# hila-chefer/Transformer-Explainability

Hardware: NVIDIA H100
Metric: explanations_per_sec (higher is better)
Workload: dtype f32

## Files before the change

### transformer_explainability_b200/csrc/te_bert.cu

```cuda
#include <string.h>

#include <algorithm>

#include "../../include/te_b200.h"
#include "te_engine_util.h"
#include "te_gemm_tc.h"
#include "te_kernels.h"
#include "te_rollout.h"
#include "te_zplus.h"

using namespace te_util;

namespace {

constexpr int kMaxDepth = 64;

struct Dims {
    int B, N, NP, D, H, dh, F, C, L, V, P, T;
    long long M;
    float eps;
};

static bool make_dims(const te_bert_config* c, int B, int S, Dims& d) {
    if (!c || c->layers <= 0 || c->layers > kMaxDepth || c->heads <= 0 || c->hidden % c->heads != 0 || c->hidden % 8 != 0 ||
// ... 187 lines not shown
    TE_TRY(check_ws(cfg, batch, seq, workspace, workspace_bytes, d, ws));
    if (!weights || !input_ids || !attention_mask) { te_set_last_error("te_bert_forward: null pointer"); return TE_ERR_ARG; }
    Select sel;
    TE_TRY(decode_flags(sel, "te_bert_forward", flags, derived, 0, false));
    cudaStream_t st = reinterpret_cast<cudaStream_t>(stream);
    const F16Forward f16 = f16_forward(sel, d.M, d.D, d.F, ws.tD[1], ws.tD[2], ws.tF[1], ws.tD[3]);
    auto layernorm = [&](const float* x, const float* g, const float* b, float* y, float* mean, float* rstd) {
        return f16.on ? te_launch_layernorm_split(x, g, b, y, mean, rstd, d.M, d.D, d.eps, f16.qkv.split, f16.qkv.scale, st)
                      : te_launch_layernorm(x, g, b, y, mean, rstd, d.M, d.D, d.eps, st);
    };
    Weights w;
    bind_weights(cfg, weights, w);
    const float scale = 1.0f / sqrtf((float)d.dh);

    TE_TRY(te_launch_bert_embed(input_ids, w.word, w.pos, w.type, ws.tD[0], d.B, d.N, d.D, d.V, st));
    TE_TRY(layernorm(ws.tD[0], w.elnw, w.elnb, ws.layer[0].h, nullptr, nullptr));
    TE_TRY(te_launch_bert_mask(attention_mask, ws.maskadd, (long long)d.B * d.N, st));

    for (int l = 0; l < d.L; ++l) {
        LayerAct& a = ws.layer[l];
        const LayerW& lw = w.layer[l];
        float* h_next = (l + 1 < d.L) ? ws.layer[l + 1].h : ws.h_last;
        const DerivedW tw = bind_derived(d, sel.lbase, l);
        TE_TRY(linear_fwd_tc(tw.qkv, a.h, d.D, lw.qkvw, lw.qkvb, a.qkv, nullptr, nullptr, d.M, d.D, 3 * d.D, TE_EPI_BIAS, st,
                             &f16.qkv));
        TE_TRY(attn_nn(sel.atc, d.B, d.H, d.N, d.NP, d.dh, a.qkv, 3 * d.D, a.qkv + d.D, 3 * d.D, a.P, nullptr, scale,
                       TE_EPI_STORE, st));
        TE_TRY(te_launch_softmax_masked(a.P, (long long)d.B * d.H * d.N, d.N, d.NP, ws.maskadd, (long long)d.H * d.N, st));
        TE_TRY(attn_nk(sel.atc, d.B, d.H, d.N, d.NP, d.dh, a.P, 0, a.qkv + 2 * d.D, 3 * d.D, a.ctx, d.D, nullptr, 1.f,
                       TE_EPI_STORE, st));
        TE_TRY(linear_fwd_tc(tw.o, a.ctx, d.D, lw.ow, lw.ob, a.d1, a.s1, a.h, d.M, d.D, d.D, TE_EPI_BIAS_ADD, st, &f16.proj));
        TE_TRY(layernorm(a.s1, lw.ln1w, lw.ln1b, a.ao, a.mean1, a.rstd1));
        TE_TRY(linear_fwd_tc(tw.w1, a.ao, d.D, lw.w1, lw.b1, a.hpre, a.g, nullptr, d.M, d.D, d.F, TE_EPI_BIAS_GELU, st,
                             &f16.fc1));
        TE_TRY(linear_fwd_tc(tw.w2, a.g, d.F, lw.w2, lw.b2, a.d2, a.s2, a.ao, d.M, d.F, d.D, TE_EPI_BIAS_ADD, st, &f16.fc2));
        TE_TRY(layernorm(a.s2, lw.ln2w, lw.ln2b, h_next, a.mean2, a.rstd2));
    }
    TE_TRY(linear_fwd(ws.h_last, d.N * d.D, w.poolw, w.poolb, ws.pd, nullptr, nullptr, d.B, d.D, d.D, TE_EPI_BIAS, st));
    TE_TRY(te_launch_tanh(ws.pd, ws.pooled, (long long)d.B * d.D, st));
    TE_TRY(linear_fwd(ws.pooled, d.D, w.clsw, w.clsb, ws.logits, nullptr, nullptr, d.B, d.D, d.C, TE_EPI_BIAS, st));
    if (logits && cudaMemcpyAsync(logits, ws.logits, sizeof(float) * d.B * d.C, cudaMemcpyDeviceToDevice, st) != cudaSuccess) {
        te_set_last_error("te_bert_forward: logits copy failed");
        return TE_ERR_CUDA;
    }
    return TE_OK;
}

extern "C" int te_bert_attribute(const te_bert_config* cfg, const float* weights, const float* derived, int batch, int seq,
                                 int* index, int start_layer, float alpha, unsigned flags, float* maps, void* workspace,
                                 long long workspace_bytes, void* stream) {
    Dims d; Workspace ws;
    TE_TRY(check_ws(cfg, batch, seq, workspace, workspace_bytes, d, ws));
    if (!isfinite(alpha)) { te_set_last_error("te_bert_attribute: alpha must be finite"); return TE_ERR_ARG; }
    TE_TRY(te_util::check_grad_rollout("te_bert_attribute", flags, alpha));
    const bool grad_rollout = (flags & TE_FLAG_ATTN_GRAD_ROLLOUT) != 0;
    if (!weights || !index || (!maps && !(flags & TE_FLAG_GRADIENTS_ONLY))) { te_set_last_error("te_bert_attribute: null pointer"); return TE_ERR_ARG; }
    if (start_layer < 0 || start_layer >= d.L) { te_set_last_error("te_bert_attribute: start_layer out of range"); return TE_ERR_ARG; }
    Select sel;
    TE_TRY(decode_flags(sel, "te_bert_attribute", flags, derived, start_layer, !grad_rollout, {ws.tF[1], ws.nF[1]},
                        {ws.t3D[1], d.M * 3LL * d.D}, d.M, std::max(3 * d.D, d.F)));
    cudaStream_t st = reinterpret_cast<cudaStream_t>(stream);
    Weights w;
    bind_weights(cfg, weights, w);
    const float scale = 1.0f / sqrtf((float)d.dh);
    const long long MD = d.M * d.D, DD = (long long)d.D * d.D;

    TE_TRY(te_launch_argmax(ws.logits, index, d.B, d.C, 1, st));
    TE_TRY(te_launch_onehot(index, ws.seed, d.B, d.C, 1.0f, st));

    float* dxa = ws.tD[0]; float* dsx = ws.tD[1]; float* dctx = ws.tD[2]; float* dxn = ws.tD[3];
    float* dF = ws.tF[0]; float* dqkv = ws.t3D[0]; float* dS = ws.tA[0];
    TE_TRY(linear_bwd(ws.seed, w.clsw, ws.dpool, nullptr, d.B, d.D, d.C, TE_EPI_STORE, st));
    TE_TRY(te_launch_tanh_bwd(ws.dpool, ws.pooled, ws.dpd, (long long)d.B * d.D, st));
    TE_TRY(linear_bwd(ws.dpd, w.poolw, ws.dfirst, nullptr, d.B, d.D, d.D, TE_EPI_STORE, st));
    TE_TRY(te_launch_fill(dxa, 0.f, MD, st));
    if (cudaMemcpy2DAsync(dxa, sizeof(float) * d.N * d.D, ws.dfirst, sizeof(float) * d.D, sizeof(float) * d.D, d.B,
                          cudaMemcpyDeviceToDevice, st) != cudaSuccess) {
        te_set_last_error("te_bert_attribute: scatter of the pooled-token gradient failed");
        return TE_ERR_CUDA;
    }
    for (int l = d.L - 1; l >= start_layer; --l) {
        LayerAct& a = ws.layer[l];
        const LayerW& lw = w.layer[l];
        TE_TRY(te_launch_layernorm_bwd(dxa, a.s2, lw.ln2w, a.mean2, a.rstd2, nullptr, dsx, d.M, d.D, st));
        const DerivedW tw = bind_derived(d, sel.lbase, l);
        TE_TRY(linear_bwd_tc(tw.w2, dsx, lw.w2, dF, a.hpre, d.M, d.F, d.D, TE_EPI_GELU_BWD, st, sel.btf, &sel.bfs));
        TE_TRY(linear_bwd_tc(tw.w1, dF, lw.w1, dxn, nullptr, d.M, d.D, d.F, TE_EPI_STORE, st, sel.btf, &sel.bfs));
        TE_TRY(te_launch_add2(dxn, dsx, dxn, MD, st));
        TE_TRY(te_launch_layernorm_bwd(dxn, a.s1, lw.ln1w, a.mean1, a.rstd1, nullptr, dsx, d.M, d.D, st));
        TE_TRY(linear_bwd_tc(tw.o, dsx, lw.ow, dctx, nullptr, d.M, d.D, d.D, TE_EPI_STORE, st, sel.btf, &sel.bfs));
        const bool last = (l == start_layer);
        TE_TRY(attn_block_bwd(sel, d.B, d.H, d.N, d.NP, d.dh, a.qkv, a.P, dctx, a.G, dS, dqkv, scale, last, st));
        if (last) break;
        TE_TRY(linear_bwd_tc(tw.qkv, dqkv, lw.qkvw, dxn, nullptr, d.M, d.D, 3 * d.D, TE_EPI_STORE, st, sel.btf, &sel.bfs));
        TE_TRY(te_launch_add2(dxn, dsx, dxa, MD, st));
    }

    if (flags & TE_FLAG_GRADIENTS_ONLY) return TE_OK;
    const long long layer_stride = d.L > 1 ? (long long)(ws.layer[1].G - ws.layer[0].G) : 0;
    if (grad_rollout) {
        TE_TRY(te_rollout_layers(ws.layer[0].G, ws.layer[0].P, layer_stride, d.L, d.B, d.H, d.N, d.NP, d.NP, start_layer,
                                 0, flags, ws.mats, ws.joint[0], ws.joint[1], nullptr, maps, 0,
                                 0, st));
        if (cudaMemset2DAsync(maps, sizeof(float) * d.N, 0, sizeof(float), d.B, st) != cudaSuccess) {
            te_set_last_error("te_bert_attribute: clearing element 0 of the maps failed");
            return TE_ERR_CUDA;
        }
        return TE_OK;
    }

    float* R = ws.tD[0]; float* R1 = ws.tD[1]; float* R2 = ws.tD[2]; float* R3 = ws.tD[3];
    float* RF = ws.tF[0]; float* SF = ws.tF[1]; float* S = ws.t3D[0]; float* Rqkv = ws.t3D[1];
    double* addp = sel.lrp ? nullptr : ws.addpart;
    TE_TRY(te_linear_rule_relprop(sel.lrp, ws.pooled, d.D, w.clsw, nullptr, ws.seed, d.C, ws.rpool, ws.shead, d.B, d.D, d.C, st,
                                  nullptr, 0, nullptr, sel.zv, 0, nullptr, alpha));
    TE_TRY(te_linear_rule_relprop(sel.lrp, ws.h_last, (long long)d.N * d.D, w.poolw, nullptr, ws.rpool, d.D, ws.rfirst, ws.shead,
                                  d.B, d.D, d.D, st, nullptr, 0, nullptr, sel.zv, 0, nullptr, alpha));
    TE_TRY(te_launch_index_select_relprop(ws.h_last, ws.rfirst, nullptr, R, d.B, d.N, d.D, st));

    for (int l = d.L - 1; l >= sel.low; --l) {
        LayerAct& a = ws.layer[l];
        const LayerW& lw = w.layer[l];
        const DerivedW dw = bind_derived(d, sel.dbase, l);
        const bool top = (l == d.L - 1) && te_engine_cls_rows();
        const long long zr = top ? d.B : d.M;
        const long long sD = top ? (long long)d.N * d.D : d.D, sF = top ? (long long)d.N * d.F : d.F;
        TE_TRY(te_launch_add_relprop(a.d2, a.ao, R, R1, R2, addp, d.B, (long long)d.N * d.D, st));
        TE_TRY(te_linear_rule_relprop(sel.lrp, a.g, sF, lw.w2, dw.w2, R1, sD, RF, S, zr, d.F, d.D, st, a.d2, sD, lw.b2, sel.zv, sF,
                                      SF, alpha));
        TE_TRY(te_linear_rule_relprop(sel.lrp, a.ao, sD, lw.w1, dw.w1, RF, sF, R1, SF, zr, d.D, d.F, st, a.hpre, sF, lw.b1, sel.zv,
                                      sD, S, alpha));
        TE_TRY(te_launch_clone_relprop(a.ao, R1, R2, nullptr, R, MD, st));
        TE_TRY(te_launch_add_relprop(a.d1, a.h, R, R1, R2, addp, d.B, (long long)d.N * d.D, st));
        if (top) TE_TRY(te_launch_fill(R3, 0.f, MD, st));
        TE_TRY(te_linear_rule_relprop(sel.lrp, a.ctx, sD, lw.ow, dw.o, R1, sD, R3, S, zr, d.D, d.D, st, a.d1, sD, lw.ob, sel.zv, sD,
                                      S + MD, alpha));
        const bool last = (l == sel.low && !(flags & TE_FLAG_RELPROP_TO_INPUT));
        TE_TRY(attn_relprop_pv(sel, d.B, d.H, d.N, d.NP, d.dh, a.qkv, a.P, R3, a.ctx, S, a.cam, Rqkv, last, st));
        if (last) break;
        TE_TRY(attn_nn(sel.atc, d.B, d.H, d.N, d.NP, d.dh, a.qkv, 3 * d.D, a.qkv + d.D, 3 * d.D, ws.tA[0], nullptr, scale,
                       TE_EPI_STORE, st));
        TE_TRY(te_launch_add_relprop_keymask(ws.tA[0], ws.maskadd, a.cam, ws.tA[1], addp, d.B, d.H, d.N, d.NP, st));
        TE_TRY(attn_relprop_qk(sel, d.B, d.H, d.N, d.NP, d.dh, a.qkv, ws.tA[1], ws.tA[0], Rqkv, st));
        TE_TRY(te_linear_rule_relprop(sel.lrp, a.h, d.D, lw.qkvw, dw.q, Rqkv, 3 * d.D, R, S, d.M, d.D, d.D, st, a.qkv, 3 * d.D,
                                      lw.qkvb, sel.zv, 0, S + MD, alpha));
        TE_TRY(te_linear_rule_relprop(sel.lrp, a.h, d.D, lw.qkvw + DD, dw.k, Rqkv + d.D, 3 * d.D, R1, S, d.M, d.D, d.D, st,
                                      a.qkv + d.D, 3 * d.D, lw.qkvb + d.D, sel.zv, 0, S + MD, alpha));
        TE_TRY(te_linear_rule_relprop(sel.lrp, a.h, d.D, lw.qkvw + 2 * DD, dw.v, Rqkv + 2 * d.D, 3 * d.D, R3, S, d.M, d.D, d.D, st,
                                      a.qkv + 2 * d.D, 3 * d.D, lw.qkvb + 2 * d.D, sel.zv, 0, S + MD, alpha));
        TE_TRY(te_launch_clone_relprop(a.h, R, R1, R3, SF, MD, st));
        TE_TRY(te_launch_clone_relprop(a.h, SF, R2, nullptr, R, MD, st));
    }

    TE_TRY(te_rollout_layers(ws.layer[0].G, ws.layer[0].cam, layer_stride, d.L, d.B, d.H, d.N, d.NP, d.NP, start_layer,
                             1, flags, ws.mats, ws.joint[0], ws.joint[1], nullptr, maps, 0,
                             1, st));
    return TE_OK;
}

extern "C" int te_bert_explain(const te_bert_config* cfg, const float* weights, const float* derived,
                               const long long* input_ids, const long long* attention_mask, int batch, int seq,
                               int* index, int start_layer, unsigned flags, float* maps, float* logits, void* workspace,
                               long long workspace_bytes, void* stream) {
    TE_TRY(te_bert_forward(cfg, weights, derived, input_ids, attention_mask, batch, seq, flags, logits, workspace,
                           workspace_bytes, stream));
    return te_bert_attribute(cfg, weights, derived, batch, seq, index, start_layer, 1.f, flags, maps, workspace, workspace_bytes,
                             stream);
}

extern "C" int te_bert_tensor(const te_bert_config* cfg, int batch, int seq, void* workspace, const char* name, int layer,
                              float** ptr, long long dims[4], long long strides[4]) {
    Dims d; Workspace ws;
    if (!workspace || !name || !ptr) return TE_ERR_ARG;
    if (batch <= 0 || !make_dims(cfg, batch, seq, d)) return TE_ERR_ARG;
    carve(d, reinterpret_cast<char*>(workspace), ws);
    const std::string n(name);
    const View set{ptr, dims, strides};
    if (n == "logits") return set(ws.logits, d.B, d.C, 1, 1, d.C, 1, 1, 1);
    if (n == "relevance_in") return set(ws.tD[0], d.B, d.N, d.D, 1, (long long)d.N * d.D, d.D, 1, 1);
    if (n.rfind("tmp_d", 0) == 0 && n.size() == 6 && n[5] >= '0' && n[5] <= '3')
        return set(ws.tD[n[5] - '0'], d.B, d.N, d.D, 1, (long long)d.N * d.D, d.D, 1, 1);
    if (n.rfind("tmp_f", 0) == 0 && n.size() == 6 && n[5] >= '0' && n[5] <= '1')
        return set(ws.tF[n[5] - '0'], d.B, d.N, d.F, 1, (long long)d.N * d.F, d.F, 1, 1);
    if (n.rfind("tmp_3d", 0) == 0 && n.size() == 7 && n[6] >= '0' && n[6] <= '1')
        return set(ws.t3D[n[6] - '0'], d.B, d.N, 3LL * d.D, 1, (long long)d.N * 3 * d.D, 3LL * d.D, 1, 1);
    const long long ND = (long long)d.N * d.D, NF = (long long)d.N * d.F;
    if (n == "h_last") return set(ws.h_last, d.B, d.N, d.D, 1, ND, d.D, 1, 1);
    if (n == "pooled") return set(ws.pooled, d.B, d.D, 1, 1, d.D, 1, 1, 1);
    if (layer < 0 || layer >= d.L) { te_set_last_error("te_bert_tensor: layer out of range"); return TE_ERR_ARG; }
    LayerAct& a = ws.layer[layer];
    const long long hs = (long long)d.N * d.NP, bs = hs * d.H;
    if (n == "attn") return set(a.P, d.B, d.H, d.N, d.N, bs, hs, d.NP, 1);
    if (n == "attn_grad") return set(a.G, d.B, d.H, d.N, d.N, bs, hs, d.NP, 1);
    if (n == "attn_cam") return set(a.cam, d.B, d.H, d.N, d.N, bs, hs, d.NP, 1);
    if (n == "hidden") return set(a.h, d.B, d.N, d.D, 1, (long long)d.N * d.D, d.D, 1, 1);
    if (n == "qkv") return set(a.qkv, d.B, d.N, 3LL * d.D, 1, 3 * ND, 3LL * d.D, 1, 1);
    float* rowD = n == "ctx" ? a.ctx : n == "d1" ? a.d1 : n == "s1" ? a.s1 : n == "ao" ? a.ao : n == "d2" ? a.d2
                : n == "s2" ? a.s2 : nullptr;
    if (rowD) return set(rowD, d.B, d.N, d.D, 1, ND, d.D, 1, 1);
    float* rowF = n == "hpre" ? a.hpre : n == "g" ? a.g : nullptr;
    if (rowF) return set(rowF, d.B, d.N, d.F, 1, NF, d.F, 1, 1);
    float* row1 = n == "mean1" ? a.mean1 : n == "rstd1" ? a.rstd1 : n == "mean2" ? a.mean2 : n == "rstd2" ? a.rstd2 : nullptr;
    if (row1) return set(row1, d.B, d.N, 1, 1, d.N, 1, 1, 1);
    te_set_last_error("te_bert_tensor: unknown tensor name");
    return TE_ERR_ARG;
}
```

### transformer_explainability_b200/csrc/te_elementwise.cu

```cuda
#include "te_kernels.h"

namespace {

constexpr int kThreads = 256;

__global__ void im2col_kernel(const float* __restrict__ img, float* __restrict__ patches, int B, int C, int H,
                              int W, int P) {
    const int gw = W / P, gh = H / P, pq = P / 4;
    const long long total = (long long)B * gh * gw * C * P * pq;
    for (long long t = blockIdx.x * (long long)blockDim.x + threadIdx.x; t < total;
         t += (long long)gridDim.x * blockDim.x) {
        long long r = t;
        const int q = (int)(r % pq); r /= pq;
        const int iy = (int)(r % P); r /= P;
        const int c = (int)(r % C); r /= C;
        const int px = (int)(r % gw); r /= gw;
        const int py = (int)(r % gh); r /= gh;
        const int b = (int)r;
        const float4 v = *reinterpret_cast<const float4*>(
            img + (((long long)b * C + c) * H + (py * P + iy)) * W + px * P + q * 4);
        const long long row = ((long long)b * gh + py) * gw + px;
        *reinterpret_cast<float4*>(patches + row * ((long long)C * P * P) + (c * P + iy) * P + q * 4) = v;
    }
}
// ... 37 lines not shown
    const float var = te_warp_sum(q) / (float)D;
    rstd = 1.0f / sqrtf(var + eps);
}

template <bool SPLIT>
__global__ void layernorm_kernel(const float* __restrict__ x, const float* __restrict__ w,
                                 const float* __restrict__ b, float* __restrict__ y, float* __restrict__ mean_o,
                                 float* __restrict__ rstd_o, long long rows, int D, float eps, __half* __restrict__ hi,
                                 __half* __restrict__ lo, float* __restrict__ scale) {
    const int lane = threadIdx.x & 31;
    const long long row = blockIdx.x * (long long)(blockDim.x >> 5) + (threadIdx.x >> 5);
    if (row >= rows) return;
    const float* xr = x + row * D;
    float mean, rstd;
    row_stats(xr, D, lane, eps, mean, rstd);
    float* yr = y + row * D;
    const int nblk = (D + 127) / 128;
    for (int base = 0; base < D; base += 128) {
        const int i = base + lane * 4;
        float4 o = make_float4(0.f, 0.f, 0.f, 0.f);
        if (i < D) {
            const float4 v = *reinterpret_cast<const float4*>(xr + i);
            const float4 ww = *reinterpret_cast<const float4*>(w + i);
            const float4 bb = *reinterpret_cast<const float4*>(b + i);
            o.x = (v.x - mean) * rstd * ww.x + bb.x;
            o.y = (v.y - mean) * rstd * ww.y + bb.y;
            o.z = (v.z - mean) * rstd * ww.z + bb.z;
            o.w = (v.w - mean) * rstd * ww.w + bb.w;
            *reinterpret_cast<float4*>(yr + i) = o;
        }
        if (SPLIT) {
            float s, si;
            te_f16_block_scale(te_warp_max(te_absmax4(o)), s, si);
            if (i < D) {
                uint2 h, l;
                te_f16_split4(o, s, h, l);
                *reinterpret_cast<uint2*>(hi + row * D + i) = h;
                *reinterpret_cast<uint2*>(lo + row * D + i) = l;
            }
            if (lane == 0) scale[row * nblk + base / 128] = si;
        }
    }
    if (lane == 0) {
        if (mean_o) mean_o[row] = mean;
        if (rstd_o) rstd_o[row] = rstd;
    }
}

__device__ __forceinline__ void ln_bwd_row(const float* __restrict__ dyr, const float* __restrict__ xr,
                                           const float* __restrict__ w, const float* __restrict__ dresr,
                                           float* __restrict__ dxr, int D, int lane, float mean, float rstd) {
    float s1 = 0.f, s2 = 0.f;
    for (int i = lane * 4; i < D; i += 128) {
        const float4 dy = *reinterpret_cast<const float4*>(dyr + i);
        const float4 xv = *reinterpret_cast<const float4*>(xr + i);
        const float4 ww = *reinterpret_cast<const float4*>(w + i);
        const float g0 = dy.x * ww.x, g1 = dy.y * ww.y, g2 = dy.z * ww.z, g3 = dy.w * ww.w;
        s1 += (g0 + g1) + (g2 + g3);
        s2 += (g0 * ((xv.x - mean) * rstd) + g1 * ((xv.y - mean) * rstd)) +
              (g2 * ((xv.z - mean) * rstd) + g3 * ((xv.w - mean) * rstd));
    }
    const float c1 = te_warp_sum(s1) / (float)D;
    const float c2 = te_warp_sum(s2) / (float)D;
    for (int i = lane * 4; i < D; i += 128) {
        const float4 dy = *reinterpret_cast<const float4*>(dyr + i);
        const float4 xv = *reinterpret_cast<const float4*>(xr + i);
        const float4 ww = *reinterpret_cast<const float4*>(w + i);
        float4 o;
        o.x = rstd * (dy.x * ww.x - c1 - (xv.x - mean) * rstd * c2);
        o.y = rstd * (dy.y * ww.y - c1 - (xv.y - mean) * rstd * c2);
        o.z = rstd * (dy.z * ww.z - c1 - (xv.z - mean) * rstd * c2);
        o.w = rstd * (dy.w * ww.w - c1 - (xv.w - mean) * rstd * c2);
        if (dresr) {
            const float4 r = *reinterpret_cast<const float4*>(dresr + i);
            o.x += r.x; o.y += r.y; o.z += r.z; o.w += r.w;
        }
        *reinterpret_cast<float4*>(dxr + i) = o;
    }
}

__global__ void layernorm_bwd_kernel(const float* __restrict__ dy, const float* __restrict__ x,
                                     const float* __restrict__ w, const float* __restrict__ mean,
                                     const float* __restrict__ rstd, const float* __restrict__ dres,
                                     float* __restrict__ dx, long long rows, int D) {
    const int lane = threadIdx.x & 31;
    const long long row = blockIdx.x * (long long)(blockDim.x >> 5) + (threadIdx.x >> 5);
    if (row >= rows) return;
    ln_bwd_row(dy + row * D, x + row * D, w, dres ? dres + row * D : nullptr, dx + row * D, D, lane, mean[row],
               rstd[row]);
}

__global__ void layernorm_bwd_strided_kernel(const float* __restrict__ dy, long long dy_stride,
                                             const float* __restrict__ x, long long x_stride,
                                             const float* __restrict__ w, float eps, float* __restrict__ dx,
                                             long long dx_stride, int rows, int D) {
    const int lane = threadIdx.x & 31;
    const int row = blockIdx.x * (blockDim.x >> 5) + (threadIdx.x >> 5);
    if (row >= rows) return;
    const float* xr = x + row * x_stride;
    float mean, rstd;
    row_stats(xr, D, lane, eps, mean, rstd);
    ln_bwd_row(dy + row * dy_stride, xr, w, nullptr, dx + row * dx_stride, D, lane, mean, rstd);
}

__global__ void softmax_kernel(float* __restrict__ s, long long rows, int N, int ld,
                               const float* __restrict__ keymask, long long rows_per_batch) {
    const int lane = threadIdx.x & 31;
    const long long row = blockIdx.x * (long long)(blockDim.x >> 5) + (threadIdx.x >> 5);
    if (row >= rows) return;
    float* r = s + row * ld;
    if (keymask) {
        const float* mk = keymask + (row / rows_per_batch) * N;
        for (int j = lane; j < N; j += 32) r[j] = r[j] + mk[j];
    }
    float m = -INFINITY;
    for (int j = lane; j < N; j += 32) m = fmaxf(m, r[j]);
    m = te_warp_max(m);
    float sum = 0.f;
    for (int j = lane; j < N; j += 32) {
        const float e = expf(r[j] - m);
        r[j] = e;
        sum += e;
    }
    sum = te_warp_sum(sum);
    for (int j = lane; j < ld; j += 32) r[j] = (j < N) ? r[j] / sum : 0.f;
}

__global__ void softmax_bwd_kernel(const float* __restrict__ p, const float* __restrict__ dp,
                                   float* __restrict__ ds, long long rows, int N, int ld, float scale) {
    const int lane = threadIdx.x & 31;
    const long long row = blockIdx.x * (long long)(blockDim.x >> 5) + (threadIdx.x >> 5);
    if (row >= rows) return;
    const float* pr = p + row * ld;
    const float* gr = dp + row * ld;
    float dot = 0.f;
    for (int j = lane; j < N; j += 32) dot = fmaf(pr[j], gr[j], dot);
    dot = te_warp_sum(dot);
    float* o = ds + row * ld;
    for (int j = lane; j < ld; j += 32) o[j] = (j < N) ? pr[j] * (gr[j] - dot) * scale : 0.f;
}

__global__ void argmax_kernel(const float* __restrict__ logits, int* __restrict__ index, int B, int C,
                              int only_negative) {
    const int lane = threadIdx.x & 31;
    const int b = blockIdx.x * (blockDim.x >> 5) + (threadIdx.x >> 5);
    if (b >= B) return;
    const float* r = logits + (long long)b * C;
    float best = -INFINITY;
    int bi = 0x7fffffff;
    for (int j = lane; j < C; j += 32) {
        const float v = r[j];
        if (v > best || (v == best && j < bi)) { best = v; bi = j; }
    }
#pragma unroll
    for (int o = 16; o > 0; o >>= 1) {
        const float ov = __shfl_xor_sync(0xffffffffu, best, o);
        const int oi = __shfl_xor_sync(0xffffffffu, bi, o);
        if (ov > best || (ov == best && oi < bi)) { best = ov; bi = oi; }
    }
    if (lane == 0 && (!only_negative || index[b] < 0)) index[b] = (bi == 0x7fffffff) ? 0 : bi;
}

__global__ void onehot_kernel(const int* __restrict__ index, float* __restrict__ seed, int B, int C, float value) {
    const long long total = (long long)B * C;
    for (long long t = blockIdx.x * (long long)blockDim.x + threadIdx.x; t < total;
         t += (long long)gridDim.x * blockDim.x) {
        const int b = (int)(t / C), c = (int)(t % C);
        seed[t] = (index[b] == c) ? value : 0.f;
    }
}

__global__ void sd_kernel(const float* a, const float* b, float* out,
                          long long n4) {
    for (long long t = blockIdx.x * (long long)blockDim.x + threadIdx.x; t < n4;
         t += (long long)gridDim.x * blockDim.x) {
        const float4 va = reinterpret_cast<const float4*>(a)[t];
        const float4 vb = reinterpret_cast<const float4*>(b)[t];
        reinterpret_cast<float4*>(out)[t] =
            make_float4(te_sd(va.x, vb.x), te_sd(va.y, vb.y), te_sd(va.z, vb.z), te_sd(va.w, vb.w));
    }
}

__global__ void clone_relprop_kernel(const float* __restrict__ x, const float* __restrict__ r1,
                                     const float* __restrict__ r2, const float* __restrict__ r3,
                                     float* __restrict__ out, long long n4) {
    for (long long t = blockIdx.x * (long long)blockDim.x + threadIdx.x; t < n4;
         t += (long long)gridDim.x * blockDim.x) {
        const float4 xv = reinterpret_cast<const float4*>(x)[t];
        const float4 a = reinterpret_cast<const float4*>(r1)[t];
        const float4 b = reinterpret_cast<const float4*>(r2)[t];
        float4 c = make_float4(te_sd(a.x, xv.x) + te_sd(b.x, xv.x), te_sd(a.y, xv.y) + te_sd(b.y, xv.y),
                               te_sd(a.z, xv.z) + te_sd(b.z, xv.z), te_sd(a.w, xv.w) + te_sd(b.w, xv.w));
        if (r3) {
            const float4 d = reinterpret_cast<const float4*>(r3)[t];
            c.x += te_sd(d.x, xv.x); c.y += te_sd(d.y, xv.y); c.z += te_sd(d.z, xv.z); c.w += te_sd(d.w, xv.w);
        }
        reinterpret_cast<float4*>(out)[t] = make_float4(xv.x * c.x, xv.y * c.y, xv.z * c.z, xv.w * c.w);
    }
}

__global__ void add_reduce_kernel(const float* __restrict__ x1, const float* __restrict__ x2,
                                  const float* __restrict__ r, double* __restrict__ partial, long long per4,
                                  long long x2s4) {
    const int b = blockIdx.y, sp = blockIdx.x;
    const long long chunk = (per4 + TE_ADD_SPLIT - 1) / TE_ADD_SPLIT;
    const long long lo = sp * chunk, hi = min(per4, lo + chunk);
    const float4* p1 = reinterpret_cast<const float4*>(x1) + b * per4;
    const float4* p2 = reinterpret_cast<const float4*>(x2) + b * x2s4;
    const float4* pr = reinterpret_cast<const float4*>(r) + b * per4;
    double sa = 0.0, sb = 0.0, sr = 0.0;
    for (long long t = lo + threadIdx.x; t < hi; t += blockDim.x) {
        const float4 a = p1[t], c = p2[t], rr = pr[t];
        const float s0 = te_sd(rr.x, a.x + c.x), s1 = te_sd(rr.y, a.y + c.y);
        const float s2 = te_sd(rr.z, a.z + c.z), s3 = te_sd(rr.w, a.w + c.w);
        sa += ((double)(a.x * s0) + (double)(a.y * s1)) + ((double)(a.z * s2) + (double)(a.w * s3));
        sb += ((double)(c.x * s0) + (double)(c.y * s1)) + ((double)(c.z * s2) + (double)(c.w * s3));
        sr += ((double)rr.x + (double)rr.y) + ((double)rr.z + (double)rr.w);
    }
    __shared__ double red[3][kThreads / 32];
    sa = te_warp_sum(sa); sb = te_warp_sum(sb); sr = te_warp_sum(sr);
    const int lane = threadIdx.x & 31, wid = threadIdx.x >> 5;
    if (lane == 0) { red[0][wid] = sa; red[1][wid] = sb; red[2][wid] = sr; }
    __syncthreads();
    if (threadIdx.x == 0) {
        double ta = 0, tb = 0, tr = 0;
        for (int i = 0; i < kThreads / 32; ++i) { ta += red[0][i]; tb += red[1][i]; tr += red[2][i]; }
        double* o = partial + ((long long)b * TE_ADD_SPLIT + sp) * 3;
        o[0] = ta; o[1] = tb; o[2] = tr;
    }
}

__global__ void add_scale_kernel(const float* __restrict__ x1, const float* __restrict__ x2,
                                 const float* __restrict__ r, float* __restrict__ r1, float* __restrict__ r2,
                                 const double* __restrict__ partial, long long per4, long long x2s4) {
    const int b = blockIdx.y;
    __shared__ float fa_s, fb_s;
    if (threadIdx.x == 0 && partial == nullptr) { fa_s = 1.f; fb_s = 1.f; }
    if (threadIdx.x == 0 && partial != nullptr) {
        double A = 0, Bs = 0, rho = 0;
        const double* q = partial + (long long)b * TE_ADD_SPLIT * 3;
        for (int i = 0; i < TE_ADD_SPLIT; ++i) { A += q[i * 3]; Bs += q[i * 3 + 1]; rho += q[i * 3 + 2]; }
        const double den = fabs(A) + fabs(Bs);
        const double a_fact = te_sd(fabs(A), den) * rho;
        const double b_fact = te_sd(fabs(Bs), den) * rho;
        fa_s = (float)te_sd(a_fact, A);
        fb_s = (float)te_sd(b_fact, Bs);
    }
    __syncthreads();
    const float fa = fa_s, fb = fb_s;
    const float4* p1 = reinterpret_cast<const float4*>(x1) + b * per4;
    const float4* p2 = reinterpret_cast<const float4*>(x2) + b * x2s4;
    const float4* pr = reinterpret_cast<const float4*>(r) + b * per4;
    float4* o1 = reinterpret_cast<float4*>(r1) + b * per4;
    float4* o2 = r2 ? reinterpret_cast<float4*>(r2) + b * per4 : nullptr;
    for (long long t = blockIdx.x * (long long)blockDim.x + threadIdx.x; t < per4;
         t += (long long)gridDim.x * blockDim.x) {
        const float4 a = p1[t], c = p2[t], rr = pr[t];
        const float s0 = te_sd(rr.x, a.x + c.x), s1 = te_sd(rr.y, a.y + c.y);
        const float s2 = te_sd(rr.z, a.z + c.z), s3 = te_sd(rr.w, a.w + c.w);
        o1[t] = make_float4(a.x * s0 * fa, a.y * s1 * fa, a.z * s2 * fa, a.w * s3 * fa);
        if (o2) o2[t] = make_float4(c.x * s0 * fb, c.y * s1 * fb, c.z * s2 * fb, c.w * s3 * fb);
    }
}

__global__ void index_select_relprop_kernel(const float* __restrict__ x, const float* __restrict__ r0,
                                            const float* __restrict__ r1, float* __restrict__ out, int B, int N,
                                            int D) {
    const long long total = (long long)B * N * D;
    for (long long t = blockIdx.x * (long long)blockDim.x + threadIdx.x; t < total;
         t += (long long)gridDim.x * blockDim.x) {
        const int d = (int)(t % D);
        const long long rt = t / D;
        const int tok = (int)(rt % N);
        const int b = (int)(rt / N);
        float v = 0.f;
        if (tok == 0) v = x[t] * te_sd(r0[(long long)b * D + d], x[t]);
        else if (tok == 1 && r1 != nullptr) v = x[t] * te_sd(r1[(long long)b * D + d], x[t]);
        out[t] = v;
    }
}

__global__ void aggregate_kernel(const float* __restrict__ G, const float* __restrict__ cam,
                                 float* __restrict__ M, int B, int H, int N, int ld_in, int ld, int add_eye,
                                 int normalize, float* __restrict__ diag) {
    const int lane = threadIdx.x & 31;
    const long long row = blockIdx.x * (long long)(blockDim.x >> 5) + (threadIdx.x >> 5);
    if (row >= (long long)B * N) return;
    const int b = (int)(row / N), i = (int)(row % N);
    float* out = M + row * ld;
    float rs = 0.f;
    for (int j = lane; j < ld; j += 32) {
        float v = 0.f;
        if (j < N) {
            float s = 0.f;
            for (int h = 0; h < H; ++h) {
                const long long o = (((long long)b * H + h) * N + i) * ld_in + j;
                s += fmaxf(G[o] * cam[o], 0.f);
            }
            v = s / (float)H;
            if (add_eye && j == i) v += 1.0f;
        }
        out[j] = v;
        rs += v;
    }
    if (normalize) {
        rs = te_warp_sum(rs);
        if (diag != nullptr) rs += 1.0f;
        __syncwarp();
        for (int j = lane; j < N; j += 32) out[j] = out[j] / rs;
        if (diag != nullptr && lane == 0) diag[row] = 1.0f / rs;
    }
}

__global__ void aggregate_vec_kernel(const float* __restrict__ G, const float* __restrict__ cam, float* __restrict__ M,
                                     int B, int H, int N, int ld_in, int ld, int add_eye, int normalize,
                                     float* __restrict__ diag) {
    const int lane = threadIdx.x & 31;
    const long long row = blockIdx.x * (long long)(blockDim.x >> 5) + (threadIdx.x >> 5);
    if (row >= (long long)B * N) return;
    const int b = (int)(row / N), i = (int)(row % N);
    float* out = M + row * ld;
    float rs = 0.f;
    for (int j4 = lane; j4 * 4 < ld; j4 += 32) {
        const int j = j4 * 4;
        float4 s = make_float4(0.f, 0.f, 0.f, 0.f);
        if (j < N && j < ld_in) {
#pragma unroll 4
            for (int h = 0; h < H; ++h) {
                const long long o = (((long long)b * H + h) * N + i) * ld_in + j;
                const float4 g = __ldcs(reinterpret_cast<const float4*>(G + o));
                const float4 c = __ldcs(reinterpret_cast<const float4*>(cam + o));
                s.x += fmaxf(g.x * c.x, 0.f); s.y += fmaxf(g.y * c.y, 0.f);
                s.z += fmaxf(g.z * c.z, 0.f); s.w += fmaxf(g.w * c.w, 0.f);
            }
        }
        float v[4] = {s.x / (float)H, s.y / (float)H, s.z / (float)H, s.w / (float)H};
#pragma unroll
        for (int u = 0; u < 4; ++u) {
// ... 133 lines not shown
    }
}

__global__ void prep_mats_kernel(const float* __restrict__ in, float* __restrict__ out, long long rows, int N,
                                 int ld_in, int ld_out, int normalize) {
    const int lane = threadIdx.x & 31;
    const long long row = blockIdx.x * (long long)(blockDim.x >> 5) + (threadIdx.x >> 5);
    if (row >= rows) return;
    const int i = (int)(row % N);
    const float* r = in + row * ld_in;
    float* o = out + row * ld_out;
    float rs = 0.f;
    for (int j = lane; j < ld_out; j += 32) {
        float v = 0.f;
        if (j < N) v = r[j] + ((j == i) ? 1.0f : 0.0f);
        o[j] = v;
        rs += v;
    }
    if (normalize) {
        rs = te_warp_sum(rs);
        __syncwarp();
        for (int j = lane; j < N; j += 32) o[j] = o[j] / rs;
    }
}

__global__ void extract_row_kernel(const float* __restrict__ joint, float* __restrict__ out, int B, int N, int ld,
                                   int first, int bert_fix) {
    const int lane = threadIdx.x & 31;
    const int b = blockIdx.x * (blockDim.x >> 5) + (threadIdx.x >> 5);
    if (b >= B) return;
    const float* r = joint + (long long)b * N * ld;
    float mn = INFINITY;
    if (bert_fix) {
        for (int j = lane; j < N; j += 32) mn = fminf(mn, r[j]);
#pragma unroll
        for (int o = 16; o > 0; o >>= 1) mn = fminf(mn, __shfl_xor_sync(0xffffffffu, mn, o));
    }
    float* o = out + (long long)b * (N - first);
    for (int j = first + lane; j < N; j += 32) o[j - first] = (bert_fix && j == 0) ? mn : r[j];
}

__global__ void average2_kernel(const float* __restrict__ a, const float* __restrict__ b, float* __restrict__ out,
                                long long n) {
    for (long long t = blockIdx.x * (long long)blockDim.x + threadIdx.x; t < n;
         t += (long long)gridDim.x * blockDim.x) out[t] = (a[t] + b[t]) / 2.0f;
}

__global__ void bert_embed_kernel(const long long* __restrict__ ids, const float* __restrict__ word,
                                  const float* __restrict__ pos, const float* __restrict__ type0,
                                  float* __restrict__ out, int B, int S, int D, int vocab) {
    const int d4 = D / 4;
    const long long total = (long long)B * S * d4;
    for (long long t = blockIdx.x * (long long)blockDim.x + threadIdx.x; t < total;
         t += (long long)gridDim.x * blockDim.x) {
        const int q = (int)(t % d4);
        const long long rt = t / d4;
        const int s = (int)(rt % S);
        const long long id = ids[rt];
        if (id < 0 || id >= vocab) {
            const float qn = __int_as_float(0x7fc00000);
            *reinterpret_cast<float4*>(out + rt * D + q * 4) = make_float4(qn, qn, qn, qn);
            continue;
        }
        const float4 w = *reinterpret_cast<const float4*>(word + id * D + q * 4);
        const float4 p = *reinterpret_cast<const float4*>(pos + (long long)s * D + q * 4);
        const float4 ty = *reinterpret_cast<const float4*>(type0 + q * 4);
        *reinterpret_cast<float4*>(out + rt * D + q * 4) =
            make_float4((ty.x + p.x) + w.x, (ty.y + p.y) + w.y, (ty.z + p.z) + w.z, (ty.w + p.w) + w.w);
    }
}
__global__ void bert_mask_kernel(const long long* __restrict__ mask, float* __restrict__ out, long long n) {
    for (long long t = blockIdx.x * (long long)blockDim.x + threadIdx.x; t < n; t += (long long)gridDim.x * blockDim.x)
        out[t] = (1.0f - (float)mask[t]) * -10000.0f;
}
__global__ void tanh_kernel(const float* __restrict__ x, float* __restrict__ y, long long n) {
    for (long long t = blockIdx.x * (long long)blockDim.x + threadIdx.x; t < n; t += (long long)gridDim.x * blockDim.x)
        y[t] = tanhf(x[t]);
}
__global__ void tanh_bwd_kernel(const float* __restrict__ dy, const float* __restrict__ y, float* __restrict__ dx,
                                long long n) {
    for (long long t = blockIdx.x * (long long)blockDim.x + threadIdx.x; t < n; t += (long long)gridDim.x * blockDim.x)
        dx[t] = dy[t] * (1.0f - y[t] * y[t]);
}
__global__ void add2_kernel(const float* a, const float* b, float* out, long long n4) {
    for (long long t = blockIdx.x * (long long)blockDim.x + threadIdx.x; t < n4;
         t += (long long)gridDim.x * blockDim.x) {
        const float4 u = reinterpret_cast<const float4*>(a)[t], v = reinterpret_cast<const float4*>(b)[t];
        reinterpret_cast<float4*>(out)[t] = make_float4(u.x + v.x, u.y + v.y, u.z + v.z, u.w + v.w);
    }
}

__global__ void add_keymask_reduce_kernel(const float* __restrict__ x1, const float* __restrict__ mk,
                                          const float* __restrict__ r, double* __restrict__ partial, int HN, int N,
                                          int ld) {
    const int b = blockIdx.y, sp = blockIdx.x;
    const int lane = threadIdx.x & 31, wid = threadIdx.x >> 5, nw = blockDim.x >> 5;
    const float* m = mk + (long long)b * N;
    double sa = 0.0, sb = 0.0, sr = 0.0;
    for (int row = sp * nw + wid; row < HN; row += TE_ADD_SPLIT * nw) {
        const float* xr = x1 + ((long long)b * HN + row) * ld;
        const float* rr = r + ((long long)b * HN + row) * ld;
        for (int j = lane; j < N; j += 32) {
            const float a = xr[j], c = m[j], rv = rr[j];
            const float s = te_sd(rv, a + c);
            sa += (double)(a * s); sb += (double)(c * s); sr += (double)rv;
        }
    }
    __shared__ double red[3][kThreads / 32];
    sa = te_warp_sum(sa); sb = te_warp_sum(sb); sr = te_warp_sum(sr);
    if (lane == 0) { red[0][wid] = sa; red[1][wid] = sb; red[2][wid] = sr; }
    __syncthreads();
    if (threadIdx.x == 0) {
        double ta = 0, tb = 0, tr = 0;
        for (int i = 0; i < nw; ++i) { ta += red[0][i]; tb += red[1][i]; tr += red[2][i]; }
        double* o = partial + ((long long)b * TE_ADD_SPLIT + sp) * 3;
        o[0] = ta; o[1] = tb; o[2] = tr;
    }
}
__global__ void add_keymask_scale_kernel(const float* __restrict__ x1, const float* __restrict__ mk,
                                         const float* __restrict__ r, float* __restrict__ r1,
                                         const double* __restrict__ partial, int HN, int N, int ld) {
    const int b = blockIdx.y;
    __shared__ float fa_s;
    if (threadIdx.x == 0 && partial == nullptr) fa_s = 1.f;
    else if (threadIdx.x == 0) {
        double A = 0, Bs = 0, rho = 0;
        const double* q = partial + (long long)b * TE_ADD_SPLIT * 3;
        for (int i = 0; i < TE_ADD_SPLIT; ++i) { A += q[i * 3]; Bs += q[i * 3 + 1]; rho += q[i * 3 + 2]; }
        const double den = fabs(A) + fabs(Bs);
        fa_s = (float)te_sd(te_sd(fabs(A), den) * rho, A);
    }
    __syncthreads();
    const float fa = fa_s;
    const int lane = threadIdx.x & 31, wid = threadIdx.x >> 5, nw = blockDim.x >> 5;
    const float* m = mk + (long long)b * N;
    for (int row = blockIdx.x * nw + wid; row < HN; row += gridDim.x * nw) {
        const float* xr = x1 + ((long long)b * HN + row) * ld;
        const float* rr = r + ((long long)b * HN + row) * ld;
        float* o = r1 + ((long long)b * HN + row) * ld;
        for (int j = lane; j < ld; j += 32) {
            float v = 0.f;
            if (j < N) { const float a = xr[j]; v = a * te_sd(rr[j], a + m[j]) * fa; }
            o[j] = v;
        }
    }
}

__global__ void fill_kernel(float* __restrict__ p, float v, long long n) {
    for (long long t = blockIdx.x * (long long)blockDim.x + threadIdx.x; t < n;
         t += (long long)gridDim.x * blockDim.x) p[t] = v;
}

inline int flat_grid(long long work) {
    long long g = (work + kThreads - 1) / kThreads;
    const long long cap = 132LL * 16;
    return (int)(g < 1 ? 1 : (g > cap ? cap : g));
}
inline int warp_rows_grid(long long rows) { return (int)((rows + (kThreads / 32) - 1) / (kThreads / 32)); }

}

#define TE_REQ(c, msg) do { if (!(c)) { te_set_last_error(msg); return TE_ERR_ARG; } } while (0)

int te_launch_im2col(const float* img, float* patches, int B, int C, int H, int W, int P, cudaStream_t st) {
    TE_REQ(P % 4 == 0 && W % P == 0 && H % P == 0, "im2col: patch must divide the image and be a multiple of 4");
    const long long total = (long long)B * (H / P) * (W / P) * C * P * (P / 4);
    im2col_kernel<<<flat_grid(total), kThreads, 0, st>>>(img, patches, B, C, H, W, P);
    TE_CUDA_CHECK_LAUNCH();
    return TE_OK;
}
int te_launch_assemble_tokens(const float* patch_out, const float* cls, const float* dist, const float* pos,
                              float* x, int B, int N, int D, int n_prefix, cudaStream_t st) {
    TE_REQ(D % 4 == 0, "assemble: D % 4 != 0");
    assemble_tokens_kernel<<<flat_grid((long long)B * N * (D / 4)), kThreads, 0, st>>>(patch_out, cls, dist, pos, x,
                                                                                     B, N, D, n_prefix);
    TE_CUDA_CHECK_LAUNCH();
    return TE_OK;
}
int te_launch_layernorm(const float* x, const float* w, const float* b, float* y, float* mean, float* rstd,
                        long long rows, int D, float eps, cudaStream_t st) {
    TE_REQ(D % 4 == 0, "layernorm: D % 4 != 0");
    if (rows <= 0) return TE_OK;
    layernorm_kernel<false><<<warp_rows_grid(rows), kThreads, 0, st>>>(x, w, b, y, mean, rstd, rows, D, eps, nullptr, nullptr,
                                                                       nullptr);
    TE_CUDA_CHECK_LAUNCH();
    return TE_OK;
}
int te_launch_layernorm_split(const float* x, const float* w, const float* b, float* y, float* mean, float* rstd,
                              long long rows, int D, float eps, float* split, float* scale, cudaStream_t st) {
    TE_REQ(D % 4 == 0, "layernorm: D % 4 != 0");
    TE_REQ(split && scale, "layernorm_split: null split buffers");
    if (rows <= 0) return TE_OK;
    __half* hi = reinterpret_cast<__half*>(split);
    layernorm_kernel<true><<<warp_rows_grid(rows), kThreads, 0, st>>>(x, w, b, y, mean, rstd, rows, D, eps, hi, hi + rows * D, scale);
    TE_CUDA_CHECK_LAUNCH();
    return TE_OK;
}
int te_launch_layernorm_bwd(const float* dy, const float* x, const float* w, const float* mean, const float* rstd,
                            const float* dres, float* dx, long long rows, int D, cudaStream_t st) {
    TE_REQ(D % 4 == 0, "layernorm_bwd: D % 4 != 0");
    if (rows <= 0) return TE_OK;
    layernorm_bwd_kernel<<<warp_rows_grid(rows), kThreads, 0, st>>>(dy, x, w, mean, rstd, dres, dx, rows, D);
    TE_CUDA_CHECK_LAUNCH();
    return TE_OK;
}
int te_launch_layernorm_bwd_strided(const float* dy, long long dy_stride, const float* x, long long x_stride,
                                    const float* w, float eps, float* dx, long long dx_stride, int rows, int D,
                                    cudaStream_t st) {
    TE_REQ(D % 4 == 0 && dy_stride % 4 == 0 && x_stride % 4 == 0 && dx_stride % 4 == 0, "layernorm_bwd_strided: align");
    if (rows <= 0) return TE_OK;
    layernorm_bwd_strided_kernel<<<warp_rows_grid(rows), kThreads, 0, st>>>(dy, dy_stride, x, x_stride, w, eps, dx,
                                                                          dx_stride, rows, D);
    TE_CUDA_CHECK_LAUNCH();
    return TE_OK;
}
int te_launch_softmax(float* s, long long rows, int N, int ld, cudaStream_t st) {
    return te_launch_softmax_masked(s, rows, N, ld, nullptr, 1, st);
}
int te_launch_softmax_masked(float* s, long long rows, int N, int ld, const float* keymask, long long rows_per_batch,
                             cudaStream_t st) {
    if (rows <= 0) return TE_OK;
    softmax_kernel<<<warp_rows_grid(rows), kThreads, 0, st>>>(s, rows, N, ld, keymask, rows_per_batch);
    TE_CUDA_CHECK_LAUNCH();
    return TE_OK;
}
int te_launch_softmax_bwd(const float* p, const float* dp, float* ds, long long rows, int N, int ld, float scale,
                          cudaStream_t st) {
    if (rows <= 0) return TE_OK;
    softmax_bwd_kernel<<<warp_rows_grid(rows), kThreads, 0, st>>>(p, dp, ds, rows, N, ld, scale);
    TE_CUDA_CHECK_LAUNCH();
    return TE_OK;
}
int te_launch_argmax(const float* logits, int* index, int B, int C, int only_negative, cudaStream_t st) {
    argmax_kernel<<<warp_rows_grid(B), kThreads, 0, st>>>(logits, index, B, C, only_negative);
    TE_CUDA_CHECK_LAUNCH();
    return TE_OK;
}
int te_launch_onehot(const int* index, float* seed, int B, int C, float value, cudaStream_t st) {
    onehot_kernel<<<flat_grid((long long)B * C), kThreads, 0, st>>>(index, seed, B, C, value);
    TE_CUDA_CHECK_LAUNCH();
    return TE_OK;
}
int te_launch_sd(const float* a, const float* b, float* out, long long n, cudaStream_t st) {
    TE_REQ(n % 4 == 0, "sd: n % 4 != 0");
    sd_kernel<<<flat_grid(n / 4), kThreads, 0, st>>>(a, b, out, n / 4);
    TE_CUDA_CHECK_LAUNCH();
    return TE_OK;
}
int te_launch_clone_relprop(const float* x, const float* r1, const float* r2, const float* r3, float* out,
                            long long n, cudaStream_t st) {
    TE_REQ(n % 4 == 0, "clone_relprop: n % 4 != 0");
    clone_relprop_kernel<<<flat_grid(n / 4), kThreads, 0, st>>>(x, r1, r2, r3, out, n / 4);
    TE_CUDA_CHECK_LAUNCH();
    return TE_OK;
}
int te_launch_add_relprop_strided(const float* x1, const float* x2, long long x2_sample_stride, const float* r, float* r1,
                                  float* r2, double* partial, int B, long long per_sample, cudaStream_t st) {
    TE_REQ(per_sample % 4 == 0 && x2_sample_stride % 4 == 0, "add_relprop: per-sample size % 4 != 0");
    TE_REQ(B <= 65535, "add_relprop: batch too large for one launch");
    const long long per4 = per_sample / 4, x2s4 = x2_sample_stride / 4;
    if (partial) {
        add_reduce_kernel<<<dim3(TE_ADD_SPLIT, B), kThreads, 0, st>>>(x1, x2, r, partial, per4, x2s4);
        TE_CUDA_CHECK_LAUNCH();
    }
    int gx = (int)((per4 + kThreads - 1) / kThreads);
    gx = gx > 64 ? 64 : (gx < 1 ? 1 : gx);
    add_scale_kernel<<<dim3(gx, B), kThreads, 0, st>>>(x1, x2, r, r1, r2, partial, per4, x2s4);
    TE_CUDA_CHECK_LAUNCH();
    return TE_OK;
}
int te_launch_add_relprop(const float* x1, const float* x2, const float* r, float* r1, float* r2, double* partial,
                          int B, long long per_sample, cudaStream_t st) {
    return te_launch_add_relprop_strided(x1, x2, per_sample, r, r1, r2, partial, B, per_sample, st);
}
int te_launch_index_select_relprop(const float* x, const float* r_tok0, const float* r_tok1, float* out, int B,
                                   int N, int D, cudaStream_t st) {
    index_select_relprop_kernel<<<flat_grid((long long)B * N * D), kThreads, 0, st>>>(x, r_tok0, r_tok1, out, B, N, D);
    TE_CUDA_CHECK_LAUNCH();
    return TE_OK;
}
int te_launch_aggregate(const float* G, const float* cam, float* M, int B, int H, int N, int ld_in, int ld_out,
                        int add_eye, int normalize, cudaStream_t st, float* diag) {
    const bool vec = ld_in % 4 == 0 && ld_out % 4 == 0 && ld_in >= ((N + 3) & ~3) &&
                     ((reinterpret_cast<uintptr_t>(G) | reinterpret_cast<uintptr_t>(cam) | reinterpret_cast<uintptr_t>(M)) & 15u) == 0;
    if (vec)
        aggregate_vec_kernel<<<warp_rows_grid((long long)B * N), kThreads, 0, st>>>(G, cam, M, B, H, N, ld_in, ld_out,
                                                                                  add_eye, normalize, diag);
    else
        aggregate_kernel<<<warp_rows_grid((long long)B * N), kThreads, 0, st>>>(G, cam, M, B, H, N, ld_in, ld_out, add_eye,
                                                                              normalize, diag);
    TE_CUDA_CHECK_LAUNCH();
    return TE_OK;
}
int te_launch_aggregate_layers(const float* G0, const float* cam0, long long in_layer_stride, float* M0, long long m_layer_stride,
                               int B, int H, int N, int ld_in, int ld_out, int first_layer, int num_layers, int normalize,
                               cudaStream_t st, float* diag0) {
    const bool vec = ld_in % 4 == 0 && ld_out % 4 == 0 && ld_in >= ((N + 3) & ~3) && in_layer_stride % 4 == 0 &&
                     m_layer_stride % 4 == 0 &&
                     ((reinterpret_cast<uintptr_t>(G0) | reinterpret_cast<uintptr_t>(cam0) | reinterpret_cast<uintptr_t>(M0)) & 15u) == 0;
    TE_REQ(vec && num_layers >= 1 && num_layers <= 65535, "aggregate_layers: unsupported layout");
    dim3 grid(warp_rows_grid((long long)B * N), num_layers);
    aggregate_layers_vec_kernel<<<grid, kThreads, 0, st>>>(G0, cam0, in_layer_stride, M0, m_layer_stride, B, H, N, ld_in, ld_out,
                                                          first_layer, normalize, diag0);
    TE_CUDA_CHECK_LAUNCH();
    return TE_OK;
}
int te_launch_relevance_heatmap(const float* maps, float* out, int B, int g, int scale, cudaStream_t st) {
    TE_REQ(B > 0 && g > 0 && scale > 0, "relevance_heatmap: bad shape");
    relevance_heatmap_kernel<<<B, kThreads, 0, st>>>(maps, out, g, scale);
    TE_CUDA_CHECK_LAUNCH();
    return TE_OK;
}
int te_launch_head_reduce(const float* a, const float* g, const float* hw, float* out, int B, int H, int N, int ld,
                          int mode, cudaStream_t st) {
    head_reduce_kernel<<<warp_rows_grid((long long)B * N), kThreads, 0, st>>>(a, g, hw, out, B, H, N, ld, mode);
    TE_CUDA_CHECK_LAUNCH();
    return TE_OK;
}
int te_launch_head_region_mean(const float* g, float* out, int BH, int N, int ld, int r0, int r1, int c0, int c1,
                               cudaStream_t st) {
    TE_REQ(BH > 0 && r0 >= 0 && r1 > r0 && r1 <= N && c0 >= 0 && c1 > c0 && c1 <= N, "head_region_mean: bad region");
    head_region_mean_kernel<<<BH, kThreads, 0, st>>>(g, out, N, ld, r0, r1, c0, c1);
    TE_CUDA_CHECK_LAUNCH();
    return TE_OK;
}
int te_launch_prep_mats(const float* in, float* out, long long rows, int N, int ld_in, int ld_out, int normalize,
                        cudaStream_t st) {
    if (rows <= 0) return TE_OK;
    prep_mats_kernel<<<warp_rows_grid(rows), kThreads, 0, st>>>(in, out, rows, N, ld_in, ld_out, normalize);
    TE_CUDA_CHECK_LAUNCH();
    return TE_OK;
}
int te_launch_extract_row(const float* joint, float* out, int B, int N, int ld, int first, int bert_fix,
                          cudaStream_t st) {
    extract_row_kernel<<<warp_rows_grid(B), kThreads, 0, st>>>(joint, out, B, N, ld, first, bert_fix);
    TE_CUDA_CHECK_LAUNCH();
    return TE_OK;
}
int te_launch_average2(const float* a, const float* b, float* out, long long n, cudaStream_t st) {
    average2_kernel<<<flat_grid(n), kThreads, 0, st>>>(a, b, out, n);
    TE_CUDA_CHECK_LAUNCH();
    return TE_OK;
}
int te_launch_bert_embed(const long long* ids, const float* word, const float* pos, const float* type0, float* out,
                         int B, int S, int D, int vocab, cudaStream_t st) {
    TE_REQ(D % 4 == 0, "bert_embed: D % 4 != 0");
    bert_embed_kernel<<<flat_grid((long long)B * S * (D / 4)), kThreads, 0, st>>>(ids, word, pos, type0, out, B, S, D, vocab);
    TE_CUDA_CHECK_LAUNCH();
    return TE_OK;
}
int te_launch_bert_mask(const long long* mask, float* out, long long n, cudaStream_t st) {
    bert_mask_kernel<<<flat_grid(n), kThreads, 0, st>>>(mask, out, n);
    TE_CUDA_CHECK_LAUNCH();
    return TE_OK;
}
int te_launch_tanh(const float* x, float* y, long long n, cudaStream_t st) {
    tanh_kernel<<<flat_grid(n), kThreads, 0, st>>>(x, y, n);
    TE_CUDA_CHECK_LAUNCH();
    return TE_OK;
}
int te_launch_tanh_bwd(const float* dy, const float* y, float* dx, long long n, cudaStream_t st) {
    tanh_bwd_kernel<<<flat_grid(n), kThreads, 0, st>>>(dy, y, dx, n);
    TE_CUDA_CHECK_LAUNCH();
    return TE_OK;
}
int te_launch_add2(const float* a, const float* b, float* out, long long n, cudaStream_t st) {
    TE_REQ(n % 4 == 0, "add2: n % 4 != 0");
    add2_kernel<<<flat_grid(n / 4), kThreads, 0, st>>>(a, b, out, n / 4);
    TE_CUDA_CHECK_LAUNCH();
    return TE_OK;
}
int te_launch_add_relprop_keymask(const float* x1, const float* keymask, const float* r, float* r1, double* partial,
                                  int B, int H, int N, int ld, cudaStream_t st) {
    TE_REQ(B <= 65535, "add_relprop_keymask: batch too large for one launch");
    if (partial) {
        add_keymask_reduce_kernel<<<dim3(TE_ADD_SPLIT, B), kThreads, 0, st>>>(x1, keymask, r, partial, H * N, N, ld);
        TE_CUDA_CHECK_LAUNCH();
    }
    int gx = (H * N + 7) / 8;
    gx = gx > 64 ? 64 : gx;
    add_keymask_scale_kernel<<<dim3(gx, B), kThreads, 0, st>>>(x1, keymask, r, r1, partial, H * N, N, ld);
    TE_CUDA_CHECK_LAUNCH();
    return TE_OK;
}
int te_launch_fill(float* p, float v, long long n, cudaStream_t st) {
    if (n <= 0) return TE_OK;
    fill_kernel<<<flat_grid(n), kThreads, 0, st>>>(p, v, n);
    TE_CUDA_CHECK_LAUNCH();
    return TE_OK;
}
```

### transformer_explainability_b200/csrc/te_engine_util.h

```cpp
#pragma once
#include <string.h>
#include <string>
#include <vector>

#include "../../include/te_b200.h"
#include "te_gemm.cuh"
#include "te_gemm_tc.h"
#include "te_kernels.h"
#include "te_zplus.h"

bool te_engine_cls_rows();
void te_engine_set_cls_rows(int on);
bool te_engine_gelu_split();
void te_engine_set_gelu_split(int on);

namespace te_util {

static inline TeGemm gemm0() {
    TeGemm p;
    memset(&p, 0, sizeof(p));
    p.nb1 = 1; p.nb2 = 1; p.alpha = 1.f;
    return p;
}

static inline int linear_fwd(const float* x, int lda, const float* w, const float* bias, float* y, float* y2,
                             const float* e0, long long M, int in, int out, int epi, cudaStream_t st) {
    TeGemm p = gemm0();
    p.A = x; p.lda = lda; p.B = w; p.ldb = in; p.C = y; p.ldc = out; p.C2 = y2; p.ldc2 = out; p.E0 = e0; p.lde0 = out;
    p.bias = bias; p.M = (int)M; p.N = out; p.K = in;
    return te_gemm_launch(p, TE_L_K, TE_L_K, TE_XF_NONE, epi, st);
}
static inline int linear_bwd(const float* dy, const float* w, float* dx, const float* e0, long long M, int in, int out,
                             int epi, cudaStream_t st) {
    TeGemm p = gemm0();
    p.A = dy; p.lda = out; p.B = w; p.ldb = in; p.C = dx; p.ldc = in; p.E0 = e0; p.lde0 = in;
    p.M = (int)M; p.N = in; p.K = out;
    return te_gemm_launch(p, TE_L_K, TE_L_MN, TE_XF_NONE, epi, st);
}

static inline int no_fallback(const char* msg) {
    te_set_last_error(msg);
    return TE_ERR_UNSUPPORTED;
}

struct F16Split { float* split; float* scale; bool ready; float* split_out; float* scale_out; };
static inline int linear_fwd_tc(const float* dw, const float* x, int lda, const float* w, const float* bias, float* y,
                                float* y2, const float* e0, long long M, int in, int out, int epi, cudaStream_t st,
                                const F16Split* fs = nullptr) {
    const bool f16 = dw && fs && fs->split;
    if (f16 && epi != TE_EPI_GELU_BWD && te_tc_fwd16_supported(M, in, out, lda))
        return te_tc_linear_fwd16(fs->ready ? nullptr : x, lda, fs->split, fs->scale, dw, in, out, bias, y, y2, e0, M, epi, st,
                                  epi == TE_EPI_BIAS_GELU ? fs->split_out : nullptr, epi == TE_EPI_BIAS_GELU ? fs->scale_out : nullptr);
    if (dw && te_tc_gemm3x_supported(M, in, out, lda))
        return te_tc_linear_fwd(x, lda, dw, in, out, bias, y, y2, e0, M, epi, st);
    return linear_fwd(x, lda, w, bias, y, y2, e0, M, in, out, epi, st);
}
static inline int linear_bwd_tc(const float* dw, const float* dy, const float* w, float* dx, const float* e0, long long M,
                                int in, int out, int epi, cudaStream_t st, bool tf32 = false, const F16Split* fs = nullptr) {
    const bool f16 = dw && fs && fs->split, single_epi = epi == TE_EPI_STORE || epi == TE_EPI_GELU_BWD;
    if (f16 && single_epi && te_tc_fwd16_supported(M, out, in, out))
        return te_tc_linear_bwd16(fs->ready ? nullptr : dy, out, fs->split, fs->scale, dw, in, out, dx, e0, M, epi, st);
    if (dw && tf32 && single_epi && te_tc_gemm3x_supported(M, out, in, out))
        return te_tc_linear_bwd_tf32(dy, out, dw, in, out, dx, e0, M, epi, st);
    if (dw && te_tc_gemm3x_supported(M, out, in, out))
        return te_tc_linear_bwd(dy, dw, in, out, dx, e0, M, epi, st);
    return linear_bwd(dy, w, dx, e0, M, in, out, epi, st);
}

struct HeadOp { const float* ptr; int ld; long long s1, s2; };
static inline HeadOp head_rows(const float* base, int ld, int N, int dh) {
    return {base, ld, (long long)N * ld, (long long)dh};
}
static inline HeadOp attn_map(const float* base, int H, int N, int NP) {
    return {base, NP, (long long)H * N * NP, (long long)N * NP};
}
static inline int head_gemm(int B, int H, HeadOp A, int alay, HeadOp Bm, int blay, HeadOp C, HeadOp E, int M, int N,
                            int K, float alpha, int epi, cudaStream_t st) {
    TeGemm p = gemm0();
    p.A = A.ptr; p.lda = A.ld; p.sA1 = A.s1; p.sA2 = A.s2;
    p.B = Bm.ptr; p.ldb = Bm.ld; p.sB1 = Bm.s1; p.sB2 = Bm.s2;
    p.C = const_cast<float*>(C.ptr); p.ldc = C.ld; p.sC1 = C.s1; p.sC2 = C.s2;
    p.E0 = E.ptr; p.lde0 = E.ld; p.sE1 = E.s1; p.sE2 = E.s2;
    p.M = M; p.N = N; p.K = K; p.nb1 = B; p.nb2 = H; p.alpha = alpha;
    return te_gemm_launch(p, alay, blay, TE_XF_NONE, epi, st);
}

static inline int attn_nn(bool tc, int B, int H, int N, int NP, int dh, const float* A, int lda, const float* Bm, int ldb,
                          float* out, const float* E, float alpha, int epi, cudaStream_t st, bool tf32 = false) {
    if (tc && te_tc_attn_supported(N, dh, lda, ldb, NP)) {
        const int e = (epi == TE_EPI_STORE) ? TE_TC_ATTN_STORE : (epi == TE_EPI_MUL) ? TE_TC_ATTN_MUL : TE_TC_ATTN_SD;
        return te_tc_attn_nn(A, lda, Bm, ldb, B, H, N, dh, out, NP, E, alpha, e, st, tf32 && N <= 256 && epi != TE_EPI_SD);
    }
    const HeadOp none = {nullptr, 0, 0, 0};
    return head_gemm(B, H, head_rows(A, lda, N, dh), TE_L_K, head_rows(Bm, ldb, N, dh), TE_L_K, attn_map(out, H, N, NP),
                     E ? attn_map(E, H, N, NP) : none, N, N, dh, alpha, epi, st);
}

static inline int attn_probs(bool tc, int B, int H, int N, int NP, int dh, const float* Q, int ldq, const float* K, int ldk,
                             float* P, float alpha, cudaStream_t st) {
    if (tc && N <= 256 && te_tc_attn_supported(N, dh, ldq, ldk, NP))
        return te_tc_attn_nn(Q, ldq, K, ldk, B, H, N, dh, P, NP, nullptr, alpha, TE_TC_ATTN_SOFTMAX, st);
    TE_TRY(attn_nn(tc, B, H, N, NP, dh, Q, ldq, K, ldk, P, nullptr, alpha, TE_EPI_STORE, st));
    return te_launch_softmax(P, (long long)B * H * N, N, NP, st);
}

static inline int attn_nk(bool tc, int B, int H, int N, int NP, int dh, const float* map, int amn, const float* X, int ldx,
                          float* out, int ld_out, const float* E, float alpha, int epi, cudaStream_t st, bool tf32 = false) {
    if (tc && te_tc_attn_nk_supported(N, dh, NP, ldx, ld_out)) {
        const int e = (epi == TE_EPI_STORE) ? TE_TC_ATTN_STORE : TE_TC_ATTN_MUL;
        if (epi == TE_EPI_STORE || epi == TE_EPI_MUL)
            return te_tc_attn_nk(map, NP, amn, X, ldx, B, H, N, out, ld_out, E, alpha, e, st, tf32);
    }
    const HeadOp none = {nullptr, 0, 0, 0};
    return head_gemm(B, H, attn_map(map, H, N, NP), amn ? TE_L_MN : TE_L_K, head_rows(X, ldx, N, dh), TE_L_MN,
                     head_rows(out, ld_out, N, dh), E ? head_rows(E, ld_out, N, dh) : none, N, dh, N, alpha, epi, st);
}

struct Select {
    const float* lbase;
    const float* dbase;
    bool atc;
    bool btf;
    bool rtf;
    bool f16;
    F16Split bfs;
    bool lrp;
    ZplusVariant zv;
    int low;
};
struct Lent { float* ptr; long long floats; };
static inline long long bwd_split_floats(long long rows, int out) { return rows * out / 2; }
static inline long long bwd_scale_floats(long long rows, int out) { return rows * ((out + 127) / 128); }

static inline int decode_flags(Select& s, const char* fn, unsigned flags, const float* derived, int start_layer, bool zplus,
                               Lent bwd_split = {nullptr, 0}, Lent bwd_scale = {nullptr, 0}, long long rows = 0,
                               int widest_out = 0) {
    const bool lrp = (flags & TE_FLAG_RULES_LRP) != 0;
    const unsigned rule_tc = lrp ? (flags & TE_FLAG_RULES_LRP_TC) : (flags & TE_FLAG_ZPLUS_TENSOR_CORES);
    if (((flags & (TE_FLAG_LINEAR_TENSOR_CORES | (zplus ? TE_FLAG_ZPLUS_TENSOR_CORES : 0u))) || (zplus && rule_tc)) && !derived) {
        te_set_last_error((std::string(fn) + ": tensor-core flags need the derived weight buffer").c_str());
        return TE_ERR_ARG;
    }
    s.lbase = (flags & TE_FLAG_LINEAR_TENSOR_CORES) ? derived : nullptr;
    s.dbase = rule_tc ? derived : nullptr;
    s.atc = (flags & TE_FLAG_ATTN_TENSOR_CORES) != 0;
    s.btf = (flags & TE_FLAG_BACKWARD_TF32) != 0;
    s.rtf = (flags & TE_FLAG_RELPROP_TF32) != 0;
    s.f16 = s.lbase && (flags & TE_FLAG_LINEAR_F16_SPLIT);
    const bool bf16 = s.lbase && (flags & TE_FLAG_BACKWARD_F16) && bwd_split.ptr;
    if (bf16 && (bwd_split.floats < bwd_split_floats(rows, widest_out) || bwd_scale.floats < bwd_scale_floats(rows, widest_out))) {
        te_set_last_error((std::string(fn) + ": the region lent for the fp16 split of the backward gradients is too small").c_str());
        return TE_ERR_WORKSPACE;
    }
    s.bfs = {bf16 ? bwd_split.ptr : nullptr, bwd_scale.ptr, false, nullptr, nullptr};
    s.lrp = lrp;
    s.zv = te_zplus_from_flags(flags);
    s.low = (flags & (TE_FLAG_KEEP_ALL_CAMS | TE_FLAG_RELPROP_TO_INPUT)) ? 0 : start_layer;
    return TE_OK;
}

static inline int check_grad_rollout(const char* fn, unsigned flags, float alpha) {
    if (!(flags & TE_FLAG_ATTN_GRAD_ROLLOUT)) return TE_OK;
    const char* clash = (flags & TE_FLAG_GRADIENTS_ONLY) ? "TE_FLAG_GRADIENTS_ONLY"
                      : (flags & TE_FLAG_KEEP_ALL_CAMS) ? "TE_FLAG_KEEP_ALL_CAMS"
                      : (flags & TE_FLAG_RELPROP_TO_INPUT) ? "TE_FLAG_RELPROP_TO_INPUT" : nullptr;
    if (clash) {
        te_set_last_error((std::string(fn) + ": TE_FLAG_ATTN_GRAD_ROLLOUT does not combine with " + clash).c_str());
        return TE_ERR_ARG;
    }
    if (alpha != 1.f) {
        te_set_last_error((std::string(fn) + ": TE_FLAG_ATTN_GRAD_ROLLOUT runs no relprop, alpha must be 1").c_str());
        return TE_ERR_ARG;
    }
    return TE_OK;
}

struct F16Forward { bool on; F16Split qkv, proj, fc1, fc2; };
static inline F16Forward f16_forward(const Select& s, long long M, int D, int F, float* a, float* a_scale, float* b,
                                     float* b_scale) {
    F16Forward f = {};
    f.on = s.f16 && F >= D && te_tc_fwd16_supported(M, D, 3 * D, D) && te_tc_fwd16_supported(M, D, D, D) &&
           te_tc_fwd16_supported(M, D, F, D) && te_tc_fwd16_supported(M, F, D, F);
    if (!f.on) return f;
    const bool gsf = te_engine_gelu_split();
    f.qkv = {a, a_scale, true, nullptr, nullptr};
    f.proj = {a, a_scale, false, nullptr, nullptr};
    f.fc1 = {a, a_scale, true, gsf ? b : nullptr, gsf ? b_scale : nullptr};
    f.fc2 = {b, b_scale, gsf, nullptr, nullptr};
    return f;
}

static inline int attn_block_bwd(const Select& s, int B, int H, int N, int NP, int dh, const float* qkv, const float* P,
                                 const float* dctx, float* G, float* dS, float* dqkv, float scale, bool g_only, cudaStream_t st) {
    const int D = H * dh;
    TE_TRY(attn_nn(s.atc, B, H, N, NP, dh, dctx, D, qkv + 2 * D, 3 * D, G, nullptr, 1.f, TE_EPI_STORE, st, s.btf));
    if (g_only) return TE_OK;
    TE_TRY(attn_nk(s.atc, B, H, N, NP, dh, P, 1, dctx, D, dqkv + 2 * D, 3 * D, nullptr, 1.f, TE_EPI_STORE, st, s.btf));
    TE_TRY(te_launch_softmax_bwd(P, G, dS, (long long)B * H * N, N, NP, scale, st));
    TE_TRY(attn_nk(s.atc, B, H, N, NP, dh, dS, 0, qkv + D, 3 * D, dqkv, 3 * D, nullptr, 1.f, TE_EPI_STORE, st, s.btf));
    return attn_nk(s.atc, B, H, N, NP, dh, dS, 1, qkv, 3 * D, dqkv + D, 3 * D, nullptr, 1.f, TE_EPI_STORE, st, s.btf);
}

static inline int attn_relprop_pv(const Select& s, int B, int H, int N, int NP, int dh, const float* qkv, const float* P,
                                  const float* Rctx, const float* ctx, float* S, float* cam, float* Rqkv, bool cam_only,
                                  cudaStream_t st) {
    const int D = H * dh;
    TE_TRY(te_launch_sd(Rctx, ctx, S, (long long)B * N * D, st));
    TE_TRY(attn_nn(s.atc, B, H, N, NP, dh, S, D, qkv + 2 * D, 3 * D, cam, P, 0.5f, TE_EPI_MUL, st, s.rtf));
    if (cam_only) return TE_OK;
    return attn_nk(s.atc, B, H, N, NP, dh, P, 1, S, D, Rqkv + 2 * D, 3 * D, qkv + 2 * D, 0.5f, TE_EPI_MUL, st, s.rtf);
}
static inline int attn_relprop_qk(const Select& s, int B, int H, int N, int NP, int dh, const float* qkv, const float* E,
                                  float* S1, float* Rqkv, cudaStream_t st) {
    const int D = H * dh;
    TE_TRY(attn_nn(s.atc, B, H, N, NP, dh, qkv, 3 * D, qkv + D, 3 * D, S1, E, 1.f, TE_EPI_SD, st));
    TE_TRY(attn_nk(s.atc, B, H, N, NP, dh, S1, 0, qkv + D, 3 * D, Rqkv, 3 * D, qkv, 0.5f, TE_EPI_MUL, st, s.rtf));
    return attn_nk(s.atc, B, H, N, NP, dh, S1, 1, qkv, 3 * D, Rqkv + D, 3 * D, qkv + D, 0.5f, TE_EPI_MUL, st, s.rtf);
}

struct Bump {
    char* base;
    long long off = 0;
    float* operator()(long long nfloat) {
        float* p = base ? reinterpret_cast<float*>(base + off) : nullptr;
        off += ((nfloat * 4 + 255) / 256) * 256;
        return p;
    }
};

template <class MakeDims, class Carve>
static inline int check_ws(const char* eng, int batch, void* workspace, long long bytes, MakeDims make_dims, Carve carve) {
    const std::string e(eng);
    if (batch <= 0 || !workspace) { te_set_last_error((e + ": batch <= 0 or null workspace").c_str()); return TE_ERR_ARG; }
    if (!make_dims()) return TE_ERR_ARG;
    if (((uintptr_t)workspace & 255u) != 0) { te_set_last_error((e + ": workspace must be 256-byte aligned").c_str()); return TE_ERR_ARG; }
    if (carve() > bytes) { te_set_last_error((e + ": workspace too small").c_str()); return TE_ERR_WORKSPACE; }
    return TE_OK;
}

struct View {
    float** ptr; long long* dims; long long* strides;
    int operator()(float* p, long long d0, long long d1, long long d2, long long d3, long long s0, long long s1, long long s2,
                   long long s3) const {
        *ptr = p; dims[0] = d0; dims[1] = d1; dims[2] = d2; dims[3] = d3;
        strides[0] = s0; strides[1] = s1; strides[2] = s2; strides[3] = s3;
        return TE_OK;
    }
};

struct WEntry { std::string name; long long numel; long long offset; };
using WTable = std::vector<WEntry>;
static inline int wt_count(const WTable& t) { return t.empty() ? TE_ERR_ARG : (int)t.size() - 1; }
static inline bool wt_has(const WTable& t, int i) { return i >= 0 && i + 1 < (int)t.size(); }
static inline const char* wt_name(const WTable& t, int i) {
    static thread_local std::string s;
    if (!wt_has(t, i)) return nullptr;
    s = t[i].name;
    return s.c_str();
}
static inline long long wt_numel(const WTable& t, int i) { return wt_has(t, i) ? t[i].numel : TE_ERR_ARG; }
static inline long long wt_offset(const WTable& t, int i) { return wt_has(t, i) ? t[i].offset : TE_ERR_ARG; }
static inline long long wt_total(const WTable& t) { return t.empty() ? TE_ERR_ARG : t.back().offset; }

}
```

### transformer_explainability_b200/csrc/te_gemm_tc.h

```cpp
#pragma once
#include <cuda_bf16.h>
#include <type_traits>

#include "te_common.cuh"
#include "te_zplus.h"

bool te_tc_zplus_supported(long long rows, int in_features, int out_features, long long ldx);

template <class F>
struct TeDerived {
    template <class T> using P = std::conditional_t<std::is_const<F>::value, const T*, T*>;
    F *wp, *wn, *wpt, *wnt;
    F *wh, *wl, *wth, *wtl;
    F* wabs;
    P<__nv_bfloat16> bf_wpt, bf_wnt;
    F* gap;
    P<__nv_bfloat16> bf_wabs;
    P<__half> h_w, l_w;
    F* s_w;
    P<__half> h_wt;
    F* s_wt;
    P<__half> h_wpt, h_wnt;
    F *s_wpt, *s_wnt;
    static constexpr long long floats(int in_features, int out_features) { return 16LL * in_features * out_features; }
    __host__ __device__ TeDerived(F* d, int in_features, int out_features) {
        const long long n = (long long)in_features * out_features;
        wp = d; wn = d + n; wpt = d + 2 * n; wnt = d + 3 * n;
        wh = d + 4 * n; wl = d + 5 * n; wth = d + 6 * n; wtl = d + 7 * n;
        wabs = d + 8 * n;
        bf_wpt = reinterpret_cast<P<__nv_bfloat16>>(d + 9 * n); bf_wnt = bf_wpt + n;
        gap = d + 10 * n;
        bf_wabs = reinterpret_cast<P<__nv_bfloat16>>(d + 11 * n);
        h_w = reinterpret_cast<P<__half>>(d + 11 * n + n / 2); l_w = reinterpret_cast<P<__half>>(d + 12 * n); s_w = d + 12 * n + n / 2;
        h_wt = reinterpret_cast<P<__half>>(d + 13 * n); s_wt = d + 13 * n + n / 2;
        h_wpt = reinterpret_cast<P<__half>>(d + 14 * n); h_wnt = reinterpret_cast<P<__half>>(d + 14 * n + n / 2);
        s_wpt = d + 15 * n; s_wnt = d + 15 * n + in_features;
    }
};
long long te_tc_derived_floats(int in_features, int out_features);
int te_tc_prepare_weights(const float* w, float* derived, int in_features, int out_features, cudaStream_t st);
int te_tc_zplus_linear_relprop(const float* x, long long ldx, const float* derived, const float* r, long long ldr,
                               float* out, float* s_scratch, long long rows, int in_features, int out_features, cudaStream_t st,
                               const float* y, long long ldy, const float* bias, ZplusVariant zv, long long ld_out,
                               float* xabs, float alpha = 1.f);
int te_tc_lrp_linear_relprop(const float* x, long long ldx, const float* derived, const float* r, long long ldr, float* out,
                             long long ld_out, float* s_scratch, long long rows, int in_features, int out_features,
                             cudaStream_t st, float alpha = 1.f);

enum { TE_TC_EPI_STORE = 0, TE_TC_EPI_BIAS = 1, TE_TC_EPI_BIAS_GELU = 2, TE_TC_EPI_BIAS_ADD = 3, TE_TC_EPI_GELU_BWD = 4 };
bool te_tc_gemm3x_supported(long long rows, int K, int N, long long lda);
int te_tc_linear_fwd(const float* x, long long ldx, const float* derived, int in_features, int out_features,
                     const float* bias, float* y, float* y2, const float* e0, long long rows, int epi, cudaStream_t st);
int te_tc_linear_bwd(const float* dy, const float* derived, int in_features, int out_features, float* dx, const float* e0,
                     long long rows, int epi, cudaStream_t st);

bool te_tc_fwd16_supported(long long rows, int K, int N, long long lda);
int te_tc_rowsplit_f16(const float* x, long long ldx, long long rows, int cols, void* hi, void* lo, float* scale_inv,
                       cudaStream_t st);
int te_tc_blocksplit_f16(const float* x, long long ldx, long long rows, int cols, float* split, float* scale_inv, cudaStream_t st,
                         bool hi_only = false);
int te_tc_linear_fwd16(const float* x, long long ldx, float* split, float* scale, const float* derived, int in_features,
                       int out_features, const float* bias, float* y, float* y2, const float* e0, long long rows, int epi,
                       cudaStream_t st, float* split_out = nullptr, float* scale_out = nullptr);
int te_tc_linear_bwd16(const float* dy, long long lddy, float* split, float* scale, const float* derived, int in_features,
                       int out_features, float* dx, const float* e0, long long rows, int epi, cudaStream_t st);
int te_tc_zplus_r16(const float* s, float* split, float* scale, const float* derived, const float* x, long long ldx, float* out,
                    long long ld_out, long long rows, int in_features, int out_features, cudaStream_t st, bool inh = false);

enum { TE_TC_ATTN_STORE = 0, TE_TC_ATTN_MUL = 1, TE_TC_ATTN_SD = 2, TE_TC_ATTN_SOFTMAX = 3 };
bool te_tc_attn_supported(int N, int dh, long long lda, long long ldb, int ld_out);
int te_tc_attn_nn(const float* A, long long lda, const float* B, long long ldb, int batch, int H, int N, int dh,
                  float* out, int ld_out, const float* E, float alpha, int epi, cudaStream_t st, bool single_pass = false);

bool te_tc_attn_nk_supported(int N, int dh, int NP, long long ldx, long long ld_out);
int te_tc_attn_nk(const float* map, int NP, int amn, const float* X, long long ldx, int batch, int H, int N, float* out,
                  int ld_out, const float* E, float alpha, int epi, cudaStream_t st, bool single_pass = false);

bool te_tc_bmm_nk_supported(int N, int ld);
int te_tc_bmm_nk_resid(const float* A, const float* J, const float* rowscale, float* out, int batch, int N, int ld,
                       cudaStream_t st);

int te_tc_zplus_s1(const float* x, long long ldx, float* xabs, const float* derived, const float* r, long long ldr,
                   const float* y, long long ldy, const float* bias, float* s_out, long long rows, int in_features,
                   int out_features, cudaStream_t st, bool bf16 = false, float* s16 = nullptr, float* s16_scale = nullptr,
                   float s_scale = 1.f, bool inh = false);
int te_tc_zplus_r(const float* s, const float* derived, const float* x, long long ldx, float* out, long long ld_out,
                  long long rows, int in_features, int out_features, cudaStream_t st, bool inh = false);
int te_tc_linear_bwd_tf32(const float* dy, long long lddy, const float* derived, int in_features, int out_features, float* dx,
                          const float* e0, long long rows, int epi, cudaStream_t st);
```

### transformer_explainability_b200/csrc/te_kernels.h

```cpp
#pragma once
#include "te_common.cuh"
#include "te_gemm.cuh"

int te_launch_im2col(const float* img, float* patches, int B, int C, int H, int W, int P, cudaStream_t st);
int te_launch_assemble_tokens(const float* patch_out, const float* cls, const float* dist, const float* pos,
                              float* x, int B, int N, int D, int n_prefix, cudaStream_t st);
int te_launch_layernorm(const float* x, const float* w, const float* b, float* y, float* mean, float* rstd,
                        long long rows, int D, float eps, cudaStream_t st);
int te_launch_layernorm_split(const float* x, const float* w, const float* b, float* y, float* mean, float* rstd,
                              long long rows, int D, float eps, float* split, float* scale, cudaStream_t st);
int te_launch_layernorm_bwd(const float* dy, const float* x, const float* w, const float* mean, const float* rstd,
                            const float* dres, float* dx, long long rows, int D, cudaStream_t st);
int te_launch_layernorm_bwd_strided(const float* dy, long long dy_stride, const float* x, long long x_stride,
                                    const float* w, float eps, float* dx, long long dx_stride, int rows, int D,
                                    cudaStream_t st);
int te_launch_softmax(float* s, long long rows, int N, int ld, cudaStream_t st);
int te_launch_softmax_bwd(const float* p, const float* dp, float* ds, long long rows, int N, int ld, float scale,
                          cudaStream_t st);
int te_launch_argmax(const float* logits, int* index, int B, int C, int only_negative, cudaStream_t st);
int te_launch_average2(const float* a, const float* b, float* out, long long n, cudaStream_t st);
int te_launch_onehot(const int* index, float* seed, int B, int C, float value, cudaStream_t st);
int te_launch_sd(const float* a, const float* b, float* out, long long n, cudaStream_t st);
int te_launch_clone_relprop(const float* x, const float* r1, const float* r2, const float* r3, float* out,
                            long long n, cudaStream_t st);
#define TE_ADD_SPLIT 16
int te_launch_add_relprop(const float* x1, const float* x2, const float* r, float* r1, float* r2, double* partial,
                          int B, long long per_sample, cudaStream_t st);
int te_launch_add_relprop_strided(const float* x1, const float* x2, long long x2_sample_stride, const float* r, float* r1,
                                  float* r2, double* partial, int B, long long per_sample, cudaStream_t st);
long long te_patch_relprop_scratch_floats(int B, int C, int img, int P, int D);
int te_patch_relprop_run(const float* images, const float* weight, const float* r, long long r_sample_stride, int B,
                         int C, int img, int P, int D, float* scratch, float* r_pixels, float* r_sum, cudaStream_t st);
int te_launch_index_select_relprop(const float* x, const float* r_tok0, const float* r_tok1, float* out, int B,
                                   int N, int D, cudaStream_t st);
int te_launch_aggregate(const float* G, const float* cam, float* M, int B, int H, int N, int ld_in, int ld_out,
                        int add_eye, int normalize, cudaStream_t st, float* diag = nullptr);
int te_launch_aggregate_layers(const float* G0, const float* cam0, long long in_layer_stride, float* M0, long long m_layer_stride,
                               int B, int H, int N, int ld_in, int ld_out, int first_layer, int num_layers, int normalize,
                               cudaStream_t st, float* diag0 = nullptr);
int te_launch_relevance_heatmap(const float* maps, float* out, int B, int g, int scale, cudaStream_t st);
int te_launch_head_reduce(const float* a, const float* g, const float* hw, float* out, int B, int H, int N, int ld,
                          int mode, cudaStream_t st);
int te_launch_head_region_mean(const float* g, float* out, int BH, int N, int ld, int r0, int r1, int c0, int c1,
                               cudaStream_t st);
int te_launch_prep_mats(const float* in, float* out, long long rows, int N, int ld_in, int ld_out, int normalize,
                        cudaStream_t st);
int te_launch_extract_row(const float* joint, float* out, int B, int N, int ld, int first, int bert_fix,
                          cudaStream_t st);
int te_launch_fill(float* p, float v, long long n, cudaStream_t st);
int te_launch_softmax_masked(float* s, long long rows, int N, int ld, const float* keymask, long long rows_per_batch,
                             cudaStream_t st);
int te_launch_bert_embed(const long long* ids, const float* word, const float* pos, const float* type0, float* out,
                         int B, int S, int D, int vocab, cudaStream_t st);
int te_launch_bert_mask(const long long* mask, float* out, long long n, cudaStream_t st);
int te_launch_tanh(const float* x, float* y, long long n, cudaStream_t st);
int te_launch_tanh_bwd(const float* dy, const float* y, float* dx, long long n, cudaStream_t st);
int te_launch_add2(const float* a, const float* b, float* out, long long n, cudaStream_t st);
int te_launch_add_relprop_keymask(const float* x1, const float* keymask, const float* r, float* r1, double* partial,
                                  int B, int H, int N, int ld, cudaStream_t st);
```

### transformer_explainability_b200/csrc/te_rollout_fused.cu

```cuda
#include <cooperative_groups.h>

#include "te_rollout_fused.h"

namespace cg = cooperative_groups;

namespace {

constexpr int kThreads = 256;
constexpr int kWarps = kThreads / 32;
constexpr int kHeadGroup = 6;

template <int NCHUNK>
__global__ void __launch_bounds__(kThreads, 2)
rollout_row_kernel(const float* __restrict__ G0, const float* __restrict__ cam0, long long layer_stride, int L, int H,
                   int N, int ld, int start, int normalize, int first, int bert_fix, float* __restrict__ out) {
    constexpr int NPAD = NCHUNK * 128;
    cg::cluster_group cluster = cg::this_cluster();
    const int K = (int)cluster.num_blocks();
    const int crank = (int)cluster.block_rank();
    const int b = blockIdx.x / K;
    const int warp = threadIdx.x >> 5, lane = threadIdx.x & 31;

    __shared__ __align__(16) float r[NPAD];
    __shared__ __align__(16) float part[NPAD];
    __shared__ __align__(16) float wacc[kWarps][NPAD];

    for (int j = threadIdx.x; j < NPAD; j += kThreads) r[j] = (j == 0) ? 1.f : 0.f;
    __syncthreads();

    const float invH = 1.0f / (float)H;
    for (int l = L - 1; l >= start; --l) {
        const float* Gl = G0 + l * layer_stride + (long long)b * H * N * ld;
        const float* Cl = cam0 + l * layer_stride + (long long)b * H * N * ld;
        float acc[NCHUNK][4];
#pragma unroll
        for (int c = 0; c < NCHUNK; ++c) { acc[c][0] = acc[c][1] = acc[c][2] = acc[c][3] = 0.f; }

        for (int i = crank + K * warp; i < N; i += K * kWarps) {
            float m[NCHUNK][4];
#pragma unroll
            for (int c = 0; c < NCHUNK; ++c) { m[c][0] = m[c][1] = m[c][2] = m[c][3] = 0.f; }
            for (int h0 = 0; h0 < H; h0 += kHeadGroup) {
#pragma unroll
                for (int c = 0; c < NCHUNK; ++c) {
                    const int col = c * 128 + lane * 4;
                    float4 g[kHeadGroup], q[kHeadGroup];
#pragma unroll
                    for (int hh = 0; hh < kHeadGroup; ++hh) {
                        g[hh] = make_float4(0.f, 0.f, 0.f, 0.f);
                        q[hh] = g[hh];
                        if (h0 + hh < H && col < ld) {
                            const long long o = ((long long)(h0 + hh) * N + i) * ld + col;
                            g[hh] = __ldcs(reinterpret_cast<const float4*>(Gl + o));
                            q[hh] = __ldcs(reinterpret_cast<const float4*>(Cl + o));
                        }
                    }
#pragma unroll
                    for (int hh = 0; hh < kHeadGroup; ++hh) {
                        m[c][0] += fmaxf(g[hh].x * q[hh].x, 0.f);
                        m[c][1] += fmaxf(g[hh].y * q[hh].y, 0.f);
                        m[c][2] += fmaxf(g[hh].z * q[hh].z, 0.f);
                        m[c][3] += fmaxf(g[hh].w * q[hh].w, 0.f);
                    }
                }
            }
            float rs = 0.f;
#pragma unroll
            for (int c = 0; c < NCHUNK; ++c)
#pragma unroll
                for (int e = 0; e < 4; ++e) {
                    const int col = c * 128 + lane * 4 + e;
                    m[c][e] = (col < N) ? m[c][e] * invH : 0.f;
                    rs += m[c][e];
                }
            float wgt = r[i];
            if (normalize) {
                rs = te_warp_sum(rs) + 1.0f;
                wgt = wgt / rs;
            }
#pragma unroll
            for (int c = 0; c < NCHUNK; ++c)
#pragma unroll
                for (int e = 0; e < 4; ++e) {
                    const int col = c * 128 + lane * 4 + e;
                    acc[c][e] = fmaf(wgt, m[c][e] + ((col == i) ? 1.0f : 0.0f), acc[c][e]);
                }
        }
#pragma unroll
        for (int c = 0; c < NCHUNK; ++c)
            *reinterpret_cast<float4*>(&wacc[warp][c * 128 + lane * 4]) = make_float4(acc[c][0], acc[c][1], acc[c][2], acc[c][3]);
        __syncthreads();
        for (int j = threadIdx.x; j < NPAD; j += kThreads) {
            float s = 0.f;
#pragma unroll
            for (int w = 0; w < kWarps; ++w) s += wacc[w][j];
            part[j] = s;
        }
        cluster.sync();
        for (int j = threadIdx.x; j < NPAD; j += kThreads) {
            float s = 0.f;
            for (int k = 0; k < K; ++k) s += cluster.map_shared_rank(part, k)[j];
            r[j] = s;
        }
        cluster.sync();
    }
    if (crank == 0) {
        __shared__ float mn_s;
        if (bert_fix) {
            if (warp == 0) {
                float mn = INFINITY;
                for (int j = lane; j < N; j += 32) mn = fminf(mn, r[j]);
#pragma unroll
                for (int o = 16; o > 0; o >>= 1) mn = fminf(mn, __shfl_xor_sync(0xffffffffu, mn, o));
                if (lane == 0) mn_s = mn;
            }
            __syncthreads();
        }
        float* o = out + (long long)b * (N - first);
        for (int j = first + threadIdx.x; j < N; j += kThreads) o[j - first] = (bert_fix && j == 0) ? mn_s : r[j];
    }
}
// ... 44 lines not shown
```

### transformer_explainability_b200/csrc/te_tc_wgmma.cu

```cuda
#include <cuda.h>
#include <cuda_bf16.h>
#include <cuda_fp16.h>
#include <cuda_runtime.h>
#include <string.h>
#include <algorithm>
#include <string>
#include <type_traits>
#include <utility>

#include "te_gemm_tc.h"
#include "te_wgmma.cuh"

namespace {

constexpr int BM = 128, NTHREADS = 256;

__device__ __forceinline__ uint32_t smem_u32(const void* p) { return (uint32_t)__cvta_generic_to_shared(p); }
__device__ __forceinline__ void fence_proxy_async() { asm volatile("fence.proxy.async.shared::cta;" ::: "memory"); }
__device__ __forceinline__ void wg_fence() { asm volatile("wgmma.fence.sync.aligned;" ::: "memory"); }
__device__ __forceinline__ void wg_commit() { asm volatile("wgmma.commit_group.sync.aligned;" ::: "memory"); }
__device__ __forceinline__ void wg_wait0() { asm volatile("wgmma.wait_group.sync.aligned 0;" ::: "memory"); }
__device__ __forceinline__ void wg_wait1() { asm volatile("wgmma.wait_group.sync.aligned 1;" ::: "memory"); }

__device__ __forceinline__ void mbar_init(uint32_t bar, uint32_t count) {
// ... 721 lines not shown
        return i == 0 ? TmaTile{a, (long long)batch * N, H * dh, lda, BM} : TmaTile{b, (long long)batch * N, H * dh, ldb, BN};
    }
    __device__ void produce(const TmaArgs& ta, uint32_t st, uint32_t bar, int kb, int m0, int n0, int bh) const {
        const int s = bh / H, k = (bh % H) * dh + kb * 32;
        mbar_expect_tx(bar, TILE128 + BN * 128);
        tma_load(st + L::a(0), &ta.map[0], k, s * N + m0, bar);
        tma_load(st + L::b(0), &ta.map[1], k, s * N + n0, bar);
    }
    __device__ void fix(uint8_t* st, int wg, int tid) const {
        fix_tf32<SP>(st + L::a(0), st + L::a(1), 64 * wg, 64, tid & 127, 128);
        fix_tf32<SP>(st + L::b(0), st + L::b(1), 0, BN, tid, 256);
    }
    __device__ void epilogue(float (&acc)[1][BN / 2], int m0, int n0, int bh, int tid, const uint8_t*) const {
        const int ncols = (N + 3) & ~3;
        if constexpr (EPI == AT_SOFTMAX) {
            float mx[2] = {-INFINITY, -INFINITY};
#pragma unroll
            for (int j = 0; j < BN / 2; ++j)
                if (n0 + frag_col(tid, j) < N) mx[(j >> 1) & 1] = fmaxf(mx[(j >> 1) & 1], alpha * acc[0][j]);
            float sum[2] = {0.f, 0.f}, m2[2];
#pragma unroll
            for (int h = 0; h < 2; ++h) {
                mx[h] = fmaxf(mx[h], __shfl_xor_sync(0xffffffffu, mx[h], 1));
                mx[h] = fmaxf(mx[h], __shfl_xor_sync(0xffffffffu, mx[h], 2));
                m2[h] = -mx[h] * 1.4426950408889634f;
            }
            const float a2 = alpha * 1.4426950408889634f;
#pragma unroll
            for (int j = 0; j < BN / 2; ++j) {
                const float e = (n0 + frag_col(tid, j) < N) ? ex2_approx(fmaf(a2, acc[0][j], m2[(j >> 1) & 1])) : 0.f;
                acc[0][j] = e;
                sum[(j >> 1) & 1] += e;
            }
#pragma unroll
            for (int h = 0; h < 2; ++h) {
                sum[h] += __shfl_xor_sync(0xffffffffu, sum[h], 1);
                sum[h] += __shfl_xor_sync(0xffffffffu, sum[h], 2);
                sum[h] = 1.0f / sum[h];
            }
#pragma unroll
            for (int j = 0; j < BN / 2; j += 2) {
                const int r = m0 + frag_row(tid, j), col = n0 + frag_col(tid, j);
                if (r >= N || col >= ncols) continue;
                const float inv = sum[(j >> 1) & 1];
                *reinterpret_cast<float2*>(out + ((long long)bh * N + r) * ld_out + col) = make_float2(acc[0][j] * inv, acc[0][j + 1] * inv);
            }
        } else {
        float2 ef[BN / 4];
#pragma unroll
        for (int j = 0; j < BN / 2; j += 2) {
            const int r = m0 + frag_row(tid, j), col = n0 + frag_col(tid, j);
            ef[j / 2] = (EPI != AT_STORE && r < N && col < ncols)
                            ? *reinterpret_cast<const float2*>(E + ((long long)bh * N + r) * ld_out + col) : make_float2(0.f, 0.f);
        }
#pragma unroll
        for (int j = 0; j < BN / 2; j += 2) {
            const int r = m0 + frag_row(tid, j), col = n0 + frag_col(tid, j);
            if (r >= N || col >= ncols) continue;
            const long long off = ((long long)bh * N + r) * ld_out + col;
            const float2 e = ef[j / 2];
            float v[2] = {alpha * acc[0][j], alpha * acc[0][j + 1]};
            const float ee[2] = {e.x, e.y};
#pragma unroll
            for (int u = 0; u < 2; ++u) {
                if (EPI == AT_MUL) v[u] *= ee[u];
                else if (EPI == AT_SD) v[u] = te_sd_fast(ee[u], v[u]);
                if (col + u >= N) v[u] = 0.f;
            }
            *reinterpret_cast<float2*>(out + off) = make_float2(v[0], v[1]);
        }
        }
    }
};

template <int AMN, int EPI, bool SP, int BN_>
struct NkProb : NoScale {
    static constexpr int BN = BN_, CHUNK = SP ? 0 : 4, FMT = OP_TF32;
    using PRODS = std::conditional_t<SP, One, Split3>;
    static constexpr int LAND_A = AMN ? BM * 128 : 0, LAND_X = BN * 128;
    using L = Stage<PRODS, BN, LAND_A + LAND_X>;
    static constexpr bool TMA = true;
    static constexpr int FIX = FIX_AB, EPI_MAPS = 0;
    int N, H, NP, ld_out, n_out, n_pad, a_shared, batch;
    const float* map; const float* X; long long ldx;
    const float* rowscale; const float* E; float* out; float alpha;
    __device__ int kblocks() const { return (N + 31) / 32; }
    static constexpr int NMAPS = 2;
    TmaTile tile(int i) const {
        if (i == 0) return TmaTile{map, N, N, NP, AMN ? 32 : BM, (long long)batch * (a_shared ? 1 : H), (long long)N * NP};
        return TmaTile{X, N, n_pad, ldx, 32, batch, (long long)N * ldx};
    }
    __device__ void produce(const TmaArgs& ta, uint32_t st, uint32_t bar, int kb, int m0, int, int bh) const {
        const int s = bh / H, h = bh % H, za = a_shared ? s : bh;
        mbar_expect_tx(bar, (AMN ? LAND_A : TILE128) + LAND_X);
        if (AMN == 0) tma_load3(st + L::a(0), &ta.map[0], kb * 32, m0, za, bar);
#pragma unroll
        for (int j = 0; j < LAND_A / 4096; ++j) tma_load3(st + L::land() + j * 4096, &ta.map[0], m0 + 32 * j, kb * 32, za, bar);
#pragma unroll
        for (int j = 0; j < LAND_X / 4096; ++j)
            tma_load3(st + L::land() + LAND_A + j * 4096, &ta.map[1], h * BN + 32 * j, kb * 32, s, bar);
    }
    __device__ void fix(uint8_t* st, int wg, int tid) const {
        if (AMN) transpose_rows(st + L::land(), 64 * wg, 64, tid & 127, 128, put_tf32<SP>(st + L::a(0), st + L::a(1)));
        else fix_tf32<SP>(st + L::a(0), st + L::a(1), 64 * wg, 64, tid & 127, 128);
        transpose_rows(st + L::land() + LAND_A, 0, BN, tid, 256, put_tf32<SP>(st + L::b(0), st + L::b(1)));
    }
    __device__ void epilogue(float (&acc)[1][BN / 2], int m0, int, int bh, int tid, const uint8_t*) const {
        const int s = bh / H, h = bh % H;
        float2 ef[BN / 4];
#pragma unroll
        for (int j = 0; j < BN / 2; j += 2) {
            const int m = m0 + frag_row(tid, j), gcol = h * BN + frag_col(tid, j);
            ef[j / 2] = (EPI != AT_STORE && m < N && gcol < n_pad)
                            ? *reinterpret_cast<const float2*>(E + ((long long)s * N + m) * ld_out + gcol) : make_float2(0.f, 0.f);
        }
#pragma unroll
        for (int j = 0; j < BN / 2; j += 2) {
            const int m = m0 + frag_row(tid, j), gcol = h * BN + frag_col(tid, j);
            if (m >= N || gcol >= n_pad) continue;
            const long long off = ((long long)s * N + m) * ld_out + gcol;
            float v[2] = {alpha * acc[0][j], alpha * acc[0][j + 1]};
            const float2 e = ef[j / 2];
            if (EPI == AT_MUL) {
                v[0] *= e.x; v[1] *= e.y;
            } else if (EPI == AT_RESID) {
                const float rsc = rowscale ? rowscale[(long long)s * N + m] : 1.f;
                v[0] += rsc * e.x; v[1] += rsc * e.y;
            }
            if (gcol >= n_out) v[0] = 0.f;
            if (gcol + 1 >= n_out) v[1] = 0.f;
            *reinterpret_cast<float2*>(out + off) = make_float2(v[0], v[1]);
        }
    }
};

inline bool a16(const void* p) { return ((uintptr_t)p & 15u) == 0; }

int sm_count() {
    static int sms[64];
    int dev = 0;
    cudaGetDevice(&dev);
    int& n = sms[dev & 63];
    if (n == 0 && cudaDeviceGetAttribute(&n, cudaDevAttrMultiProcessorCount, dev) != cudaSuccess) n = 1;
    return n;
}

using EncodeTiled = CUresult (*)(CUtensorMap*, CUtensorMapDataType, cuuint32_t, void*, const cuuint64_t*, const cuuint64_t*,
                                 const cuuint32_t*, const cuuint32_t*, CUtensorMapInterleave, CUtensorMapSwizzle,
                                 CUtensorMapL2promotion, CUtensorMapFloatOOBfill);
EncodeTiled encode_tiled() {
    static const EncodeTiled fn = [] {
        void* f = nullptr;
        cudaDriverEntryPointQueryResult q;
        if (cudaGetDriverEntryPoint("cuTensorMapEncodeTiled", &f, cudaEnableDefault, &q) != cudaSuccess ||
            q != cudaDriverEntryPointSuccess)
            return (EncodeTiled) nullptr;
        return (EncodeTiled)f;
    }();
    return fn;
}
bool encode_tile(CUtensorMap* map, const TmaTile& t, int esize) {
    const EncodeTiled fn = encode_tiled();
    const int rank = t.count > 0 ? 3 : 2;
    if (!fn || ((uintptr_t)t.base & 15u) || (t.ld * esize) % 16 != 0 || (t.cstride * esize) % 16 != 0 || t.rows < 1 || t.cols < 1)
        return false;
    const cuuint64_t dims[3] = {(cuuint64_t)t.cols, (cuuint64_t)t.rows, (cuuint64_t)t.count};
    const cuuint64_t strides[2] = {(cuuint64_t)(t.ld * esize), (cuuint64_t)(t.cstride * esize)};
    const cuuint32_t box[3] = {(cuuint32_t)(128 / esize), (cuuint32_t)t.box_rows, 1}, estr[3] = {1, 1, 1};
    return fn(map, esize == 4 ? CU_TENSOR_MAP_DATA_TYPE_FLOAT32 : CU_TENSOR_MAP_DATA_TYPE_UINT16, rank, const_cast<void*>(t.base),
// ... 79 lines not shown
        }
    }
}

__global__ void __launch_bounds__(256) blocksplit_f16_kernel(const float* __restrict__ x, long long ldx, long long rows, int cols,
                                                             __half* __restrict__ hi, __half* __restrict__ lo,
                                                             float* __restrict__ inv) {
    const int lane = threadIdx.x & 31;
    const long long wpb = blockDim.x >> 5;
    const int nblk = (cols + 127) / 128;
    for (long long row = blockIdx.x * wpb + (threadIdx.x >> 5); row < rows; row += (long long)gridDim.x * wpb) {
        const float* xr = x + row * ldx;
#pragma unroll 2
        for (int base = 0; base < cols; base += 128) {
            const int i = base + lane * 4;
            float4 v = make_float4(0.f, 0.f, 0.f, 0.f);
            if (i < cols) v = *reinterpret_cast<const float4*>(xr + i);
            float s, si;
            te_f16_block_scale(te_warp_max(te_absmax4(v)), s, si);
            if (i < cols) {
                uint2 h, l;
                te_f16_split4(v, s, h, l);
                *reinterpret_cast<uint2*>(hi + row * cols + i) = h;
                if (lo) *reinterpret_cast<uint2*>(lo + row * cols + i) = l;
            }
            if (lane == 0) inv[row * nblk + base / 128] = si;
        }
    }
}
__global__ void __launch_bounds__(256) rowsplit_f16_kernel(const float* __restrict__ x, long long ldx, long long rows, int cols4,
                                                           __half* __restrict__ hi, __half* __restrict__ lo,
                                                           float* __restrict__ inv) {
    const int lane = threadIdx.x & 31;
    const long long wpb = blockDim.x >> 5;
    for (long long row = blockIdx.x * wpb + (threadIdx.x >> 5); row < rows; row += (long long)gridDim.x * wpb) {
        const float4* xr = reinterpret_cast<const float4*>(x + row * ldx);
        float m = 0.f;
#pragma unroll 4
        for (int c = lane; c < cols4; c += 32) m = fmaxf(m, te_absmax4(xr[c]));
        float s, si;
        te_f16_block_scale(te_warp_max(m), s, si);
        uint2* hr = reinterpret_cast<uint2*>(hi + row * (long long)cols4 * 4);
        uint2* lr = reinterpret_cast<uint2*>(lo + row * (long long)cols4 * 4);
#pragma unroll 4
        for (int c = lane; c < cols4; c += 32) {
            uint2 h, l;
            te_f16_split4(xr[c], s, h, l);
            hr[c] = h;
            if (lo) lr[c] = l;
        }
        if (lane == 0) inv[row] = si;
    }
}
__global__ void abs_bf16_kernel(const float* __restrict__ x, long long ldx, __nv_bfloat16* __restrict__ out, long long rows, int cols4) {
    const long long total = rows * cols4;
    for (long long t = blockIdx.x * (long long)blockDim.x + threadIdx.x; t < total; t += (long long)gridDim.x * blockDim.x) {
        const long long r = t / cols4;
        const int c = (int)(t - r * cols4);
        const float4 v = *reinterpret_cast<const float4*>(x + r * ldx + 4 * c);
        const __nv_bfloat162 a = __floats2bfloat162_rn(fabsf(v.x), fabsf(v.y)), b = __floats2bfloat162_rn(fabsf(v.z), fabsf(v.w));
        uint2 pk;
        pk.x = *reinterpret_cast<const uint32_t*>(&a);
        pk.y = *reinterpret_cast<const uint32_t*>(&b);
        *reinterpret_cast<uint2*>(out + t * 4) = pk;
    }
}
unsigned stride_blocks(long long work, int per_block) {
    long long b = (work + per_block - 1) / per_block;
    const long long cap = (long long)sm_count() * 16;
    if (b > cap) b = cap;
    return (unsigned)(b < 1 ? 1 : b);
}

template <int EPI, int FORM>
int lin_launch(const LinArgs& args, cudaStream_t st) {
    using P = LinProb<EPI, FORM>;
    P p;
    static_cast<LinArgs&>(p) = args;
    return launch(p, dim3(mtiles(args.o.M), (args.o.N + P::BN - 1) / P::BN), st);
}
template <int FORM, bool FWD>
int linear(int K, const void* a, const void* a_lo, long long lda, const void* b, const void* b_lo, const float* rs,
           const float* cs, long long rows, int N, const float* bias, const float* e0, float* y, float* y2, int epi,
           const char* who, cudaStream_t st) {
    LinArgs g;
    g.K = K; g.a = a; g.a_lo = a_lo; g.lda = lda; g.b = b; g.b_lo = b_lo; g.rs = rs; g.rs_ld = (K + 127) / 128; g.cs = cs;
    g.o.M = (int)rows; g.o.N = N; g.o.bias = bias; g.o.E = e0; g.o.lde = N; g.o.C = y; g.o.ldc = N; g.o.C2 = y2; g.o.ldc2 = N;
    switch (epi) {
        case TE_TC_EPI_STORE: return lin_launch<TE_TC_EPI_STORE, FORM>(g, st);
        case TE_TC_EPI_BIAS: if constexpr (FWD) return lin_launch<TE_TC_EPI_BIAS, FORM>(g, st); break;
        case TE_TC_EPI_BIAS_GELU: if constexpr (FWD) return lin_launch<TE_TC_EPI_BIAS_GELU, FORM>(g, st); break;
        case TE_TC_EPI_BIAS_ADD: if constexpr (FWD) return lin_launch<TE_TC_EPI_BIAS_ADD, FORM>(g, st); break;
        case TE_TC_EPI_GELU_BWD: if constexpr (!FWD) return lin_launch<TE_TC_EPI_GELU_BWD, FORM>(g, st); break;
    }
    te_set_last_error((std::string(who) + ": unsupported epilogue").c_str());
    return TE_ERR_UNSUPPORTED;
}

template <bool SINGLE, bool BF, int OUT>
int zs(const float* x, long long ldx, const void* xabs, const void* wa, const void* wb, const float* r, long long ldr,
       const float* y, long long ldy, const float* bias, void* out, float* hs, long long rows, int in_features, int out_features,
       cudaStream_t st, float s_scale, bool inh) {
    ZsProb<SINGLE, BF, OUT> p;
    p.M = (int)rows; p.N = out_features; p.K = in_features;
    p.x = x; p.ldx = ldx; p.xabs = xabs; p.wa = wa; p.wb = wb;
    p.r = r; p.ldr = ldr; p.y = y; p.ldy = ldy; p.bias = bias;
    p.out = out; p.ldo = out_features; p.hs = hs;
    p.sscale = s_scale; p.zsign = inh ? -1.f : 1.f;
    return launch(p, dim3(mtiles(p.M), p.N / 128), st);
}

}

long long te_tc_derived_floats(int in_features, int out_features) { return TeDerived<float>::floats(in_features, out_features); }

int te_tc_prepare_weights(const float* w, float* derived, int in_features, int out_features, cudaStream_t st) {
    dim3 grid((in_features + 31) / 32, (out_features + 31) / 32), block(32, 8);
    prepare_weights_kernel<<<grid, block, 0, st>>>(w, derived, out_features, in_features);
    TE_CUDA_CHECK_LAUNCH();
    const TeDerived<float> dv(derived, in_features, out_features);
    if (in_features % 8 == 0 && in_features >= 8 && a16(w))
        TE_TRY(te_tc_rowsplit_f16(w, in_features, out_features, in_features, dv.h_w, dv.l_w, dv.s_w, st));
    if (out_features % 8 == 0 && in_features >= 2) {
        TE_TRY(te_tc_rowsplit_f16(dv.wth, out_features, in_features, out_features, dv.h_wt, nullptr, dv.s_wt, st));
        TE_TRY(te_tc_rowsplit_f16(dv.wpt, out_features, in_features, out_features, dv.h_wpt, nullptr, dv.s_wpt, st));
        TE_TRY(te_tc_rowsplit_f16(dv.wnt, out_features, in_features, out_features, dv.h_wnt, nullptr, dv.s_wnt, st));
    }
    return TE_OK;
}

int te_tc_rowsplit_f16(const float* x, long long ldx, long long rows, int cols, void* hi, void* lo, float* scale_inv,
                       cudaStream_t st) {
    if (cols % 4 != 0 || ldx % 4 != 0 || !a16(x) || ((uintptr_t)hi & 7u) || (lo && ((uintptr_t)lo & 7u))) {
        te_set_last_error("te_tc_rowsplit_f16: alignment");
        return TE_ERR_ARG;
    }
    rowsplit_f16_kernel<<<stride_blocks(rows, 8), 256, 0, st>>>(x, ldx, rows, cols / 4, reinterpret_cast<__half*>(hi),
                                                                reinterpret_cast<__half*>(lo), scale_inv);
    TE_CUDA_CHECK_LAUNCH();
    return TE_OK;
}

int te_tc_blocksplit_f16(const float* x, long long ldx, long long rows, int cols, float* split, float* scale_inv, cudaStream_t st,
                         bool hi_only) {
    if (cols % 4 != 0 || ldx % 4 != 0 || !a16(x) || !a16(split) || !scale_inv) {
        te_set_last_error("te_tc_blocksplit_f16: alignment");
        return TE_ERR_ARG;
    }
    __half* hi = reinterpret_cast<__half*>(split);
    blocksplit_f16_kernel<<<stride_blocks(rows, 8), 256, 0, st>>>(x, ldx, rows, cols, hi, hi_only ? nullptr : hi + rows * cols,
                                                                  scale_inv);
    TE_CUDA_CHECK_LAUNCH();
    return TE_OK;
}

bool te_tc_zplus_supported(long long rows, int in_features, int out_features, long long ldx) {
    return rows > 0 && rows < (1LL << 31) && in_features % 128 == 0 && out_features % 128 == 0 && ldx % 4 == 0;
}
int te_tc_zplus_s1(const float* x, long long ldx, float* xabs, const float* derived, const float* r, long long ldr,
                   const float* y, long long ldy, const float* bias, float* s_out, long long rows, int in_features,
                   int out_features, cudaStream_t st, bool bf16, float* s16, float* s16_scale, float s_scale, bool inh) {
    const TeDerived<const float> dv(derived, in_features, out_features);
    if (ldx % 4 != 0 || !a16(x) || !a16(r) || !a16(y) || ldr % 4 != 0 || ldy % 4 != 0) {
        te_set_last_error("te_tc_zplus_s1: alignment");
        return TE_ERR_ARG;
    }
    void* o = s16 ? (void*)s16 : (void*)s_out;
    auto run = [&](auto zs_fn, const void* wa) {
        return zs_fn(x, ldx, xabs, wa, nullptr, r, ldr, y, ldy, bias, o, s16_scale, rows, in_features, out_features, st, s_scale,
                     inh);
// ... 58 lines not shown
        return single ? zs_fn(x, ldx, nullptr, dv.wabs, nullptr, r, ldr, y, ldy, bias, s_scratch, nullptr, rows,
                              in_features, out_features, st, s_scale, inh)
                      : zs_fn(x, ldx, nullptr, inh ? dv.wn : dv.wp, inh ? dv.wp : dv.wn, r, ldr, nullptr, 0, nullptr, s_scratch,
                              nullptr, rows, in_features, out_features, st, s_scale, inh);
    };
    if (single) TE_TRY(rb ? run(zs<true, false, ZO_BF16>) : run(zs<true, false, ZO_F32>));
    else TE_TRY(rb ? run(zs<false, false, ZO_BF16>) : run(zs<false, false, ZO_F32>));
    if (rb) {
        ZrProb<1> p;
        memset(&p, 0, sizeof(p));
        p.M = (int)rows; p.N = in_features; p.K = out_features;
        p.s = s_scratch; p.wp = inh ? dv.bf_wnt : dv.bf_wpt; p.wn = inh ? dv.bf_wpt : dv.bf_wnt;
        p.x = x; p.ldx = ldx; p.out = out; p.ldo = ld_out; p.accum = inh;
        return launch(p, dim3(mtiles(rows), in_features / 128), st);
    }
    return te_tc_zplus_r(s_scratch, derived, x, ldx, out, ld_out, rows, in_features, out_features, st, inh);
}
}

int te_tc_zplus_linear_relprop(const float* x, long long ldx, const float* derived, const float* r, long long ldr,
                               float* out, float* s_scratch, long long rows, int in_features, int out_features, cudaStream_t st,
                               const float* y, long long ldy, const float* bias, ZplusVariant zv, long long ld_out, float* xabs,
                               float alpha) {
    if (ld_out == 0) ld_out = in_features;
    if (!a16(x) || !a16(derived) || !a16(r) || !a16(out) || !a16(s_scratch)) {
        te_set_last_error("te_gemm_tc: operands must be 16-byte aligned");
        return TE_ERR_ARG;
    }
    const float beta = alpha - 1.f;
    TE_TRY(zplus_half(x, ldx, derived, r, ldr, out, s_scratch, rows, in_features, out_features, st, y, ldy, bias, zv, ld_out, xabs,
                      alpha, false));
    if (beta == 0.f) return TE_OK;
    return zplus_half(x, ldx, derived, r, ldr, out, s_scratch, rows, in_features, out_features, st, y, ldy, bias, zv, ld_out, xabs,
                      -beta, true);
}

namespace {
template <bool NEG>
int lrp_half(const float* x, long long ldx, const float* w, const float* wt, const float* r, long long ldr, float* out,
             long long ld_out, float* s, long long rows, int in_features, int out_features, cudaStream_t st, float s_scale,
             bool accum) {
    LrpSProb<NEG> ps;
    ps.M = (int)rows; ps.N = out_features; ps.K = in_features;
    ps.x = x; ps.ldx = ldx; ps.w = w; ps.r = r; ps.ldr = ldr; ps.out = s; ps.sscale = s_scale;
    TE_TRY(launch(ps, dim3(mtiles(rows), out_features / 128), st));
    LrpRProb<NEG> pr;
    pr.M = (int)rows; pr.N = in_features; pr.K = out_features;
    pr.s = s; pr.wt = wt; pr.x = x; pr.ldx = ldx; pr.out = out; pr.ldo = ld_out; pr.accum = accum;
    return launch(pr, dim3(mtiles(rows), in_features / 128), st);
}
}

int te_tc_lrp_linear_relprop(const float* x, long long ldx, const float* derived, const float* r, long long ldr, float* out,
                             long long ld_out, float* s_scratch, long long rows, int in_features, int out_features,
                             cudaStream_t st, float alpha) {
    if (!a16(x) || !a16(derived) || !a16(r) || !a16(out) || !a16(s_scratch) || ldx % 4 != 0 || ldr % 4 != 0 || ld_out % 4 != 0) {
        te_set_last_error("te_tc_lrp_linear_relprop: operands must be 16-byte aligned");
        return TE_ERR_ARG;
    }
    const TeDerived<const float> dv(derived, in_features, out_features);
    const float beta = alpha - 1.f;
    TE_TRY(lrp_half<false>(x, ldx, dv.wp, dv.wpt, r, ldr, out, ld_out, s_scratch, rows, in_features, out_features, st, alpha, false));
    TE_TRY(lrp_half<true>(x, ldx, dv.wn, dv.wnt, r, ldr, out, ld_out, s_scratch, rows, in_features, out_features, st, alpha, true));
    if (beta == 0.f) return TE_OK;
    TE_TRY(lrp_half<false>(x, ldx, dv.wn, dv.wnt, r, ldr, out, ld_out, s_scratch, rows, in_features, out_features, st, -beta, true));
    return lrp_half<true>(x, ldx, dv.wp, dv.wpt, r, ldr, out, ld_out, s_scratch, rows, in_features, out_features, st, -beta, true);
}

bool te_tc_gemm3x_supported(long long rows, int K, int N, long long lda) {
    return rows > 0 && rows < (1LL << 31) && K % 32 == 0 && N % 128 == 0 && lda % 4 == 0;
}

int te_tc_linear_fwd(const float* x, long long ldx, const float* derived, int in_features, int out_features, const float* bias,
                     float* y, float* y2, const float* e0, long long rows, int epi, cudaStream_t st) {
    if (!a16(x) || !a16(derived) || !a16(y) || (y2 && !a16(y2)) || (e0 && !a16(e0)) || (bias && !a16(bias))) {
        te_set_last_error("te_tc_linear_fwd: operands must be 16-byte aligned");
        return TE_ERR_ARG;
    }
    const TeDerived<const float> dv(derived, in_features, out_features);
    return linear<LIN_3XTF32, true>(in_features, x, nullptr, ldx, dv.wh, dv.wl, nullptr, nullptr, rows, out_features, bias, e0, y,
                                    y2, epi, "te_tc_linear_fwd", st);
}

int te_tc_linear_bwd(const float* dy, const float* derived, int in_features, int out_features, float* dx, const float* e0,
                     long long rows, int epi, cudaStream_t st) {
    if (!a16(dy) || !a16(derived) || !a16(dx) || (e0 && !a16(e0))) {
        te_set_last_error("te_tc_linear_bwd: operands must be 16-byte aligned");
        return TE_ERR_ARG;
    }
    const TeDerived<const float> dv(derived, in_features, out_features);
    return linear<LIN_3XTF32, false>(out_features, dy, nullptr, out_features, dv.wth, dv.wtl, nullptr, nullptr, rows, in_features,
                                     nullptr, e0, dx, nullptr, epi, "te_tc_linear_bwd", st);
}

int te_tc_linear_bwd_tf32(const float* dy, long long lddy, const float* derived, int in_features, int out_features, float* dx,
                          const float* e0, long long rows, int epi, cudaStream_t st) {
    if (!a16(dy) || lddy % 4 != 0 || !a16(derived) || !a16(dx) || (e0 && !a16(e0))) {
        te_set_last_error("te_tc_linear_bwd_tf32: operands must be 16-byte aligned");
        return TE_ERR_ARG;
    }
    const TeDerived<const float> dv(derived, in_features, out_features);
    return linear<LIN_TF32, false>(out_features, dy, nullptr, lddy, dv.wth, nullptr, nullptr, nullptr, rows, in_features, nullptr,
                                   e0, dx, nullptr, epi, "te_tc_linear_bwd_tf32", st);
}

bool te_tc_fwd16_supported(long long rows, int K, int N, long long lda) {
    return rows > 0 && rows < (1LL << 31) && K % 64 == 0 && N % 128 == 0 && lda % 4 == 0;
}

int te_tc_linear_fwd16(const float* x, long long ldx, float* split, float* scale, const float* derived, int in_features,
                       int out_features, const float* bias, float* y, float* y2, const float* e0, long long rows, int epi,
                       cudaStream_t st, float* split_out, float* scale_out) {
    if (!a16(split) || !scale || !a16(derived) || !a16(y) || (y2 && !a16(y2)) || (e0 && !a16(e0)) || (bias && !a16(bias)) ||
        (split_out && (!a16(split_out) || !scale_out || !y2 || epi != TE_TC_EPI_BIAS_GELU))) {
        te_set_last_error("te_tc_linear_fwd16: bad operands");
        return TE_ERR_ARG;
    }
    const __half* ah = reinterpret_cast<const __half*>(split);
    const __half* al = ah + rows * in_features;
    if (x) TE_TRY(te_tc_blocksplit_f16(x, ldx, rows, in_features, split, scale, st));
    const TeDerived<const float> dv(derived, in_features, out_features);
    TE_TRY((linear<LIN_F16X3, true>(in_features, ah, al, in_features, dv.h_w, dv.l_w, scale, dv.s_w, rows, out_features, bias, e0,
                                    y, y2, epi, "te_tc_linear_fwd16", st)));
    if (split_out) return te_tc_blocksplit_f16(y2, out_features, rows, out_features, split_out, scale_out, st);
    return TE_OK;
}

int te_tc_linear_bwd16(const float* dy, long long lddy, float* split, float* scale, const float* derived, int in_features,
                       int out_features, float* dx, const float* e0, long long rows, int epi, cudaStream_t st) {
    if (!a16(split) || !scale || !a16(derived) || !a16(dx) || (e0 && !a16(e0))) {
        te_set_last_error("te_tc_linear_bwd16: bad operands");
        return TE_ERR_ARG;
    }
    if (dy) TE_TRY(te_tc_blocksplit_f16(dy, lddy, rows, out_features, split, scale, st, true));
    const TeDerived<const float> dv(derived, in_features, out_features);
    return linear<LIN_F16, false>(out_features, split, nullptr, out_features, dv.h_wt, nullptr, scale, dv.s_wt, rows, in_features,
                                  nullptr, e0, dx, nullptr, epi, "te_tc_linear_bwd16", st);
}

bool te_tc_attn_supported(int N, int dh, long long lda, long long ldb, int ld_out) {
    return N >= 1 && (dh == 32 || dh == 64) && lda % 4 == 0 && ldb % 4 == 0 && ld_out % 4 == 0;
}
bool te_tc_attn_nk_supported(int N, int dh, int NP, long long ldx, long long ld_out) {
    return N >= 1 && dh == 64 && NP % 4 == 0 && ldx % 4 == 0 && ld_out % 4 == 0;
}
bool te_tc_bmm_nk_supported(int N, int ld) { return N >= 1 && ld % 4 == 0 && ld >= N; }

namespace {
template <int EPI, bool SP, int BN>
int nn(const float* A, long long lda, const float* B, long long ldb, int batch, int H, int N, int dh, float* out, int ld_out,
       const float* E, float alpha, cudaStream_t st) {
    NnProb<EPI, SP, BN> p;
    p.N = N; p.H = H; p.dh = dh; p.ld_out = ld_out; p.batch = batch;
    p.a = A; p.lda = lda; p.b = B; p.ldb = ldb; p.E = E; p.out = out; p.alpha = alpha;
    return launch(p, dim3(mtiles(N), (unsigned)((N + BN - 1) / BN), (unsigned)(batch * H)), st);
}
template <int AMN, int EPI, bool SP, int BN>
int nk(const float* map, int NP, const float* X, long long ldx, int batch, int H, int N, float* out, int ld_out, int n_out,
       int n_pad, int a_shared, const float* rowscale, const float* E, float alpha, cudaStream_t st) {
    NkProb<AMN, EPI, SP, BN> p;
    p.N = N; p.H = H; p.NP = NP; p.ld_out = ld_out; p.n_out = n_out; p.n_pad = n_pad; p.a_shared = a_shared; p.batch = batch;
    p.map = map; p.X = X; p.ldx = ldx; p.rowscale = rowscale; p.E = E; p.out = out; p.alpha = alpha;
    return launch(p, dim3(mtiles(N), 1, (unsigned)(batch * H)), st);
}
}

int te_tc_attn_nn(const float* A, long long lda, const float* B, long long ldb, int batch, int H, int N, int dh,
                  float* out, int ld_out, const float* E, float alpha, int epi, cudaStream_t st, bool single_pass) {
#define TE_NN(EPI, SP, BN) nn<EPI, SP, BN>(A, lda, B, ldb, batch, H, N, dh, out, ld_out, E, alpha, st)
    if (single_pass && epi == TE_TC_ATTN_STORE) return TE_NN(AT_STORE, true, 128);
    if (single_pass && epi == TE_TC_ATTN_MUL) return TE_NN(AT_MUL, true, 128);
    switch (epi) {
        case TE_TC_ATTN_STORE: return TE_NN(AT_STORE, false, 128);
        case TE_TC_ATTN_MUL: return TE_NN(AT_MUL, false, 128);
        case TE_TC_ATTN_SD: return TE_NN(AT_SD, false, 128);
        case TE_TC_ATTN_SOFTMAX:
            if (N > 256) break;
            return TE_NN(AT_SOFTMAX, false, 256);
    }
#undef TE_NN
    te_set_last_error("te_gemm_tc: unsupported attention epilogue");
    return TE_ERR_UNSUPPORTED;
}

int te_tc_attn_nk(const float* map, int NP, int amn, const float* X, long long ldx, int batch, int H, int N, float* out,
                  int ld_out, const float* E, float alpha, int epi, cudaStream_t st, bool single_pass) {
#define TE_NK(AMN, EPI, SP) nk<AMN, EPI, SP, 64>(map, NP, X, ldx, batch, H, N, out, ld_out, H * 64, H * 64, 0, nullptr, E, alpha, st)
    if (epi == TE_TC_ATTN_STORE) {
        if (single_pass) return amn ? TE_NK(1, AT_STORE, true) : TE_NK(0, AT_STORE, true);
        return amn ? TE_NK(1, AT_STORE, false) : TE_NK(0, AT_STORE, false);
    }
    if (epi == TE_TC_ATTN_MUL) {
        if (single_pass) return amn ? TE_NK(1, AT_MUL, true) : TE_NK(0, AT_MUL, true);
        return amn ? TE_NK(1, AT_MUL, false) : TE_NK(0, AT_MUL, false);
    }
#undef TE_NK
    te_set_last_error("te_gemm_tc: unsupported attention nk epilogue");
    return TE_ERR_UNSUPPORTED;
}

int te_tc_bmm_nk_resid(const float* A, const float* J, const float* rowscale, float* out, int batch, int N, int ld,
                       cudaStream_t st) {
    return nk<0, AT_RESID, false, 128>(A, ld, J, ld, batch, (ld + 127) / 128, N, out, ld, N, ld, 1, rowscale, J, 1.f, st);
}
```

### transformer_explainability_b200/csrc/te_vit.cu

```cuda
#include <string.h>

#include <algorithm>

#include "../../include/te_b200.h"
#include "te_engine_util.h"
#include "te_kernels.h"
#include "te_rollout.h"
#include "te_zplus.h"
#include "te_gemm_tc.h"

namespace {

constexpr int kMaxDepth = 64;

struct Dims {
    int B, N, NP, D, H, dh, F, C, L, P, img, Cin, npatch, prefix, KP;
    long long M;
};

static bool make_dims(const te_vit_config* c, int B, Dims& d) {
    if (!c || c->depth <= 0 || c->depth > kMaxDepth || c->heads <= 0 || c->dim % c->heads != 0 || c->dim % 4 != 0 ||
        c->mlp_dim % 4 != 0 || c->patch_size % 4 != 0 || c->img_size % c->patch_size != 0 || c->num_classes <= 0) {
        te_set_last_error("te_vit: invalid config");
        return false;
// ... 209 lines not shown
                                      TE_EPI_BIAS_GELU, st, &f16.fc1));
        TE_TRY(te_util::linear_fwd_tc(lw.fc2, a.g, d.F, bw.fc2w, bw.fc2b, a.mlp_out, x_next, a.x_mid, d.M, d.F, d.D,
                                      TE_EPI_BIAS_ADD, st, &f16.fc2));
    }
    TE_TRY(te_launch_layernorm(ws.x_last, w.normw, w.normb, ws.xf, nullptr, nullptr, d.M, d.D, cfg->eps_final, st));
    TE_TRY(linear_fwd(ws.xf, d.N * d.D, w.headw, w.headb, ws.logits, nullptr, nullptr, d.B, d.D, d.C, TE_EPI_BIAS, st));
    if (cfg->distilled) {
        TE_TRY(linear_fwd(ws.xf + d.D, d.N * d.D, w.headdw, w.headdb, ws.logits2, nullptr, nullptr, d.B, d.D, d.C,
                          TE_EPI_BIAS, st));
        TE_TRY(te_launch_average2(ws.logits, ws.logits2, ws.logits, (long long)d.B * d.C, st));
    }
    if (logits) {
        if (cudaMemcpyAsync(logits, ws.logits, sizeof(float) * d.B * d.C, cudaMemcpyDeviceToDevice, st) != cudaSuccess) {
            te_set_last_error("te_vit_forward: logits copy failed");
            return TE_ERR_CUDA;
        }
    }
    return TE_OK;
}

extern "C" long long te_vit_derived_total(const te_vit_config* cfg) {
    Dims d;
    if (!make_dims(cfg, 1, d)) return TE_ERR_ARG;
    return (long long)d.L * derived_block_floats(d);
}

extern "C" int te_vit_prepare_derived(const te_vit_config* cfg, const float* weights, float* derived, void* stream) {
    Dims d;
    if (!make_dims(cfg, 1, d)) return TE_ERR_ARG;
    if (!weights || !derived) { te_set_last_error("te_vit_prepare_derived: null pointer"); return TE_ERR_ARG; }
    cudaStream_t st = reinterpret_cast<cudaStream_t>(stream);
    Weights w;
    bind_weights(cfg, weights, w);
    for (int l = 0; l < d.L; ++l) {
        const DerivedW dw = bind_derived(d, derived, l);
        TE_TRY(te_tc_prepare_weights(w.blk[l].qkvw, const_cast<float*>(dw.qkv), d.D, 3 * d.D, st));
        TE_TRY(te_tc_prepare_weights(w.blk[l].projw, const_cast<float*>(dw.proj), d.D, d.D, st));
        TE_TRY(te_tc_prepare_weights(w.blk[l].fc1w, const_cast<float*>(dw.fc1), d.D, d.F, st));
        TE_TRY(te_tc_prepare_weights(w.blk[l].fc2w, const_cast<float*>(dw.fc2), d.F, d.D, st));
    }
    return TE_OK;
}

extern "C" int te_vit_attribute(const te_vit_config* cfg, const float* weights, const float* derived, int batch, int* index,
                                int start_layer, float alpha, unsigned flags, float* maps, void* workspace,
                                long long workspace_bytes, void* stream) {
    Dims d; Workspace ws;
    TE_TRY(check_ws(cfg, batch, workspace, workspace_bytes, d, ws));
    if (!isfinite(alpha)) { te_set_last_error("te_vit_attribute: alpha must be finite"); return TE_ERR_ARG; }
    TE_TRY(te_util::check_grad_rollout("te_vit_attribute", flags, alpha));
    const bool grad_rollout = (flags & TE_FLAG_ATTN_GRAD_ROLLOUT) != 0;
    if (!weights || !index || (!maps && !(flags & TE_FLAG_GRADIENTS_ONLY))) { te_set_last_error("te_vit_attribute: null pointer"); return TE_ERR_ARG; }
    if (start_layer < 0 || start_layer >= d.L) { te_set_last_error("te_vit_attribute: start_layer out of range"); return TE_ERR_ARG; }
    cudaStream_t st = reinterpret_cast<cudaStream_t>(stream);
    Weights w;
    bind_weights(cfg, weights, w);
    const float scale = 1.0f / sqrtf((float)d.dh);
    const long long MD = d.M * d.D, M3D = d.M * 3LL * d.D;
    te_util::Select sel;
    TE_TRY(te_util::decode_flags(sel, "te_vit_attribute", flags, derived, start_layer, !grad_rollout, {ws.tF[1], ws.nF[1]},
                                 {ws.t3D[1], M3D}, d.M, std::max(3 * d.D, d.F)));

    TE_TRY(te_launch_argmax(ws.logits, index, d.B, d.C, 1, st));
    const float seedv = cfg->distilled ? 0.5f : 1.0f;
    TE_TRY(te_launch_onehot(index, ws.seed, d.B, d.C, seedv, st));

    float* dxa = ws.tD[0]; float* dxb = ws.tD[1]; float* dctx = ws.tD[2]; float* dxn = ws.tD[3];
    float* dF = ws.tF[0]; float* dqkv = ws.t3D[0]; float* dS = ws.tA;
    TE_TRY(te_launch_fill(dxa, 0.f, MD, st));
    {
        TE_TRY(linear_bwd(ws.seed, w.headw, ws.dpool, nullptr, d.B, d.D, d.C, TE_EPI_STORE, st));
        TE_TRY(te_launch_layernorm_bwd_strided(ws.dpool, d.D, ws.x_last, (long long)d.N * d.D, w.normw, cfg->eps_final,
                                               dxa, (long long)d.N * d.D, d.B, d.D, st));
        if (cfg->distilled) {
            TE_TRY(linear_bwd(ws.seed, w.headdw, ws.dpool, nullptr, d.B, d.D, d.C, TE_EPI_STORE, st));
            TE_TRY(te_launch_layernorm_bwd_strided(ws.dpool, d.D, ws.x_last + d.D, (long long)d.N * d.D, w.normw,
                                                   cfg->eps_final, dxa + d.D, (long long)d.N * d.D, d.B, d.D, st));
        }
    }
    for (int l = d.L - 1; l >= start_layer; --l) {
        LayerAct& a = ws.layer[l];
        const BlockW& bw = w.blk[l];
        const DerivedW lw = bind_derived(d, sel.lbase, l);
        TE_TRY(te_util::linear_bwd_tc(lw.fc2, dxa, bw.fc2w, dF, a.h, d.M, d.F, d.D, TE_EPI_GELU_BWD, st, sel.btf, &sel.bfs));
        TE_TRY(te_util::linear_bwd_tc(lw.fc1, dF, bw.fc1w, dxn, nullptr, d.M, d.D, d.F, TE_EPI_STORE, st, sel.btf, &sel.bfs));
        TE_TRY(te_launch_layernorm_bwd(dxn, a.x_mid, bw.n2w, a.mean2, a.rstd2, dxa, dxb, d.M, d.D, st));
        TE_TRY(te_util::linear_bwd_tc(lw.proj, dxb, bw.projw, dctx, nullptr, d.M, d.D, d.D, TE_EPI_STORE, st, sel.btf, &sel.bfs));
        const bool last = (l == start_layer);
        TE_TRY(te_util::attn_block_bwd(sel, d.B, d.H, d.N, d.NP, d.dh, a.qkv, a.P, dctx, a.G, dS, dqkv, scale, last, st));
        if (last) break;
        TE_TRY(te_util::linear_bwd_tc(lw.qkv, dqkv, bw.qkvw, dxn, nullptr, d.M, d.D, 3 * d.D, TE_EPI_STORE, st, sel.btf, &sel.bfs));
        TE_TRY(te_launch_layernorm_bwd(dxn, a.x_in, bw.n1w, a.mean1, a.rstd1, dxb, dxa, d.M, d.D, st));
    }

    if (flags & TE_FLAG_GRADIENTS_ONLY) return TE_OK;
    const long long layer_stride = d.L > 1 ? (long long)(ws.layer[1].G - ws.layer[0].G) : 0;
    if (grad_rollout)
        return te_rollout_layers(ws.layer[0].G, ws.layer[0].P, layer_stride, d.L, d.B, d.H, d.N, d.NP, d.NP, start_layer,
                                 0, flags, ws.mats, ws.joint[0], ws.joint[1], nullptr, maps, d.prefix,
                                 0, st);

    float* R = ws.tD[0]; float* R1 = ws.tD[1]; float* R2 = ws.tD[2]; float* R3 = ws.tD[3];
    float* RF = ws.tF[0]; float* SF = ws.tF[1]; float* S = ws.t3D[0]; float* Rqkv = ws.t3D[1]; float* S1 = ws.tA;
    auto addrule = [&](const float* x1, const float* x2, const float* r, float* r1, float* r2) -> int {
        return te_launch_add_relprop(x1, x2, r, r1, r2, sel.lrp ? nullptr : ws.addpart, d.B, (long long)d.N * d.D, st);
    };
    TE_TRY(te_linear_rule_relprop(sel.lrp, ws.xf, (long long)d.N * d.D, w.headw, nullptr, ws.seed, d.C, ws.rhead0, ws.shead, d.B,
                                  d.D, d.C, st, nullptr, 0, nullptr, sel.zv, 0, nullptr, alpha));
    if (cfg->distilled)
        TE_TRY(te_linear_rule_relprop(sel.lrp, ws.xf + d.D, (long long)d.N * d.D, w.headdw, nullptr, ws.seed, d.C, ws.rhead1,
                                      ws.shead, d.B, d.D, d.C, st, nullptr, 0, nullptr, sel.zv, 0, nullptr, alpha));
    TE_TRY(te_launch_index_select_relprop(ws.xf, ws.rhead0, cfg->distilled ? ws.rhead1 : nullptr, R, d.B, d.N, d.D, st));

    for (int l = d.L - 1; l >= sel.low; --l) {
        LayerAct& a = ws.layer[l];
        const BlockW& bw = w.blk[l];
        const DerivedW dw = bind_derived(d, sel.dbase, l);
        const bool top = (l == d.L - 1) && !cfg->distilled && !sel.lrp && te_engine_cls_rows();
        const long long zr = top ? d.B : d.M;
        const long long sD = top ? (long long)d.N * d.D : d.D, sF = top ? (long long)d.N * d.F : d.F;
        TE_TRY(addrule(a.x_mid, a.mlp_out, R, R1, R2));
        TE_TRY(te_linear_rule_relprop(sel.lrp, a.g, sF, bw.fc2w, dw.fc2, R2, sD, RF, S, zr, d.F, d.D, st, a.mlp_out, sD, bw.fc2b,
                                      sel.zv, sF, SF, alpha));
        TE_TRY(te_linear_rule_relprop(sel.lrp, a.xn2, sD, bw.fc1w, dw.fc1, RF, sF, R2, SF, zr, d.D, d.F, st, a.h, sF, bw.fc1b,
                                      sel.zv, sD, S, alpha));
        TE_TRY(te_launch_clone_relprop(a.x_mid, R1, R2, nullptr, R, MD, st));
        TE_TRY(addrule(a.x_in, a.attn_out, R, R1, R2));
        if (top) TE_TRY(te_launch_fill(R3, 0.f, MD, st));
        TE_TRY(te_linear_rule_relprop(sel.lrp, a.ctx, sD, bw.projw, dw.proj, R2, sD, R3, S, zr, d.D, d.D, st, a.attn_out, sD,
                                      bw.projb, sel.zv, sD, S + MD, alpha));
        const bool last = (l == sel.low && !(flags & TE_FLAG_RELPROP_TO_INPUT));
        TE_TRY(te_util::attn_relprop_pv(sel, d.B, d.H, d.N, d.NP, d.dh, a.qkv, a.P, R3, a.ctx, S, a.cam, Rqkv, last, st));
        if (last) break;
        TE_TRY(te_util::attn_relprop_qk(sel, d.B, d.H, d.N, d.NP, d.dh, a.qkv, a.cam, S1, Rqkv, st));
        TE_TRY(te_linear_rule_relprop(sel.lrp, a.xn1, d.D, bw.qkvw, dw.qkv, Rqkv, 3 * d.D, R2, S, d.M, d.D, 3 * d.D, st, a.qkv,
                                      3 * d.D, bw.qkvb, sel.zv, 0, RF, alpha));
        TE_TRY(te_launch_clone_relprop(a.x_in, R1, R2, nullptr, R, MD, st));
    }

    TE_TRY(te_rollout_layers(ws.layer[0].G, ws.layer[0].cam, layer_stride, d.L, d.B, d.H, d.N, d.NP, d.NP,
                             start_layer, 0, flags, ws.mats, ws.joint[0], ws.joint[1], nullptr, maps,
                             d.prefix, 0, st));
    return TE_OK;
}

extern "C" int te_vit_relprop_pixels(const te_vit_config* cfg, const float* weights, const float* images, int batch,
                                     unsigned flags, float* pixel_maps, float* pixel_relevance, void* workspace,
                                     long long workspace_bytes, void* stream) {
    Dims d; Workspace ws;
    TE_TRY(check_ws(cfg, batch, workspace, workspace_bytes, d, ws));
    if (!weights || !images || (!pixel_maps && !pixel_relevance)) { te_set_last_error("te_vit_relprop_pixels: null pointer"); return TE_ERR_ARG; }
    cudaStream_t st = reinterpret_cast<cudaStream_t>(stream);
    Weights w;
    bind_weights(cfg, weights, w);
    float* R = ws.tD[0];
    float* tokens = ws.tD[1];
    float* Rtok = ws.tD[2];
    float* patches = ws.tF[0];
    float* patch_out = ws.tD[3];
    TE_TRY(te_launch_im2col(images, patches, d.B, d.Cin, d.img, d.img, d.P, st));
    TE_TRY(linear_fwd(patches, d.KP, w.patchw, w.patchb, patch_out, nullptr, nullptr, (long long)d.B * d.npatch, d.KP,
                      d.D, TE_EPI_BIAS, st));
    TE_TRY(te_launch_assemble_tokens(patch_out, w.cls, w.dist, nullptr, tokens, d.B, d.N, d.D, d.prefix, st));
    TE_TRY(te_launch_add_relprop_strided(tokens, w.pos, 0, R, Rtok, nullptr, (flags & TE_FLAG_RULES_LRP) ? nullptr : ws.addpart,
                                         d.B, (long long)d.N * d.D, st));
    return te_patch_relprop_run(images, w.patchw, Rtok + (long long)d.prefix * d.D, (long long)d.N * d.D, d.B, d.Cin, d.img,
                                d.P, d.D, ws.pix, pixel_relevance, pixel_maps, st);
}

extern "C" int te_vit_explain(const te_vit_config* cfg, const float* weights, const float* derived, const float* images,
                              int batch, int* index, int start_layer, unsigned flags, float* maps, float* logits,
                              void* workspace, long long workspace_bytes, void* stream) {
    TE_TRY(te_vit_forward(cfg, weights, derived, images, batch, flags, logits, workspace, workspace_bytes, stream));
    return te_vit_attribute(cfg, weights, derived, batch, index, start_layer, 1.f, flags, maps, workspace, workspace_bytes,
                            stream);
}

extern "C" int te_vit_tensor(const te_vit_config* cfg, int batch, void* workspace, const char* name, int layer,
                             float** ptr, long long dims[4], long long strides[4]) {
    Dims d; Workspace ws;
    if (!workspace || !name || !ptr) return TE_ERR_ARG;
    if (batch <= 0 || !make_dims(cfg, batch, d)) return TE_ERR_ARG;
    carve(d, reinterpret_cast<char*>(workspace), ws);
    const std::string n(name);
    const te_util::View set{ptr, dims, strides};
    if (n == "logits") return set(ws.logits, d.B, d.C, 1, 1, d.C, 1, 1, 1);
    if (n == "relevance_in") return set(ws.tD[0], d.B, d.N, d.D, 1, (long long)d.N * d.D, d.D, 1, 1);
    if (n == "rollout_mats") return set(ws.mats, d.L, d.B, d.N, d.N, (long long)d.B * d.N * d.NP, (long long)d.N * d.NP, d.NP, 1);
    const long long ND = (long long)d.N * d.D, NF = (long long)d.N * d.F;
    if (n == "x_last") return set(ws.x_last, d.B, d.N, d.D, 1, ND, d.D, 1, 1);
    if (n == "x_final_norm") return set(ws.xf, d.B, d.N, d.D, 1, ND, d.D, 1, 1);
    if (n.rfind("tmp_d", 0) == 0 && n.size() == 6 && n[5] >= '0' && n[5] <= '3')
        return set(ws.tD[n[5] - '0'], d.B, d.N, d.D, 1, (long long)d.N * d.D, d.D, 1, 1);
    if (n.rfind("tmp_f", 0) == 0 && n.size() == 6 && n[5] >= '0' && n[5] <= '1')
        return set(ws.tF[n[5] - '0'], d.B, d.N, d.F, 1, (long long)d.N * d.F, d.F, 1, 1);
    if (n.rfind("tmp_3d", 0) == 0 && n.size() == 7 && n[6] >= '0' && n[6] <= '1')
        return set(ws.t3D[n[6] - '0'], d.B, d.N, 3LL * d.D, 1, (long long)d.N * 3 * d.D, 3LL * d.D, 1, 1);
    if (layer < 0 || layer >= d.L) { te_set_last_error("te_vit_tensor: layer out of range"); return TE_ERR_ARG; }
    LayerAct& a = ws.layer[layer];
    const long long hs = (long long)d.N * d.NP, bs = hs * d.H;
    if (n == "attn") return set(a.P, d.B, d.H, d.N, d.N, bs, hs, d.NP, 1);
    if (n == "attn_grad") return set(a.G, d.B, d.H, d.N, d.N, bs, hs, d.NP, 1);
    if (n == "attn_cam") return set(a.cam, d.B, d.H, d.N, d.N, bs, hs, d.NP, 1);
    if (n == "qkv") return set(a.qkv, d.B, d.N, 3LL * d.D, 1, (long long)d.N * 3 * d.D, 3LL * d.D, 1, 1);
    if (n == "x_in") return set(a.x_in, d.B, d.N, d.D, 1, (long long)d.N * d.D, d.D, 1, 1);
    if (n == "ctx") return set(a.ctx, d.B, d.N, d.D, 1, (long long)d.N * d.D, d.D, 1, 1);
    float* rowD = n == "xn1" ? a.xn1 : n == "attn_out" ? a.attn_out : n == "x_mid" ? a.x_mid : n == "xn2" ? a.xn2
                : n == "mlp_out" ? a.mlp_out : nullptr;
    if (rowD) return set(rowD, d.B, d.N, d.D, 1, ND, d.D, 1, 1);
    float* rowF = n == "h" ? a.h : n == "g" ? a.g : nullptr;
    if (rowF) return set(rowF, d.B, d.N, d.F, 1, NF, d.F, 1, 1);
    float* row1 = n == "mean1" ? a.mean1 : n == "rstd1" ? a.rstd1 : n == "mean2" ? a.mean2 : n == "rstd2" ? a.rstd2 : nullptr;
    if (row1) return set(row1, d.B, d.N, 1, 1, d.N, 1, 1, 1);
    te_set_last_error("te_vit_tensor: unknown tensor name");
    return TE_ERR_ARG;
}
```

Measured before the change: 924.9.

## Restrict top-layer backward and relprop to CLS-token rows

In the top layer, only the CLS token's gradient and relevance are nonzero, so the gradient backward (MLP, layernorm, output projection, attention) and the relprop add/clone rules now process only B rows with strided access rather than all B*N rows. Kernels gain row-stride, stat-stride and kept-prefix parameters, and the attention GEMMs can limit their m rows or k tokens. The untouched rows of the buffers are zero-filled, which adds fill launches in exchange for much smaller top-layer GEMMs. The extra bookkeeping makes it easy to get the correctness conditions wrong.

```diff
diff --git a/transformer_explainability_b200/csrc/te_bert.cu b/transformer_explainability_b200/csrc/te_bert.cu
--- a/transformer_explainability_b200/csrc/te_bert.cu
+++ b/transformer_explainability_b200/csrc/te_bert.cu
@@ -293,15 +293,21 @@
     for (int l = d.L - 1; l >= start_layer; --l) {
         LayerAct& a = ws.layer[l];
         const LayerW& lw = w.layer[l];
-        TE_TRY(te_launch_layernorm_bwd(dxa, a.s2, lw.ln2w, a.mean2, a.rstd2, nullptr, dsx, d.M, d.D, st));
+        const bool top = (l == d.L - 1) && !sel.bfs.split && te_engine_cls_rows();
+        const long long br = top ? d.B : d.M;
+        const long long bD = top ? (long long)d.N * d.D : d.D, bF = top ? (long long)d.N * d.F : d.F;
+        const long long sl = top ? d.N : 1;
+        TE_TRY(te_launch_layernorm_bwd(dxa, a.s2, lw.ln2w, a.mean2, a.rstd2, nullptr, dsx, br, d.D, st, bD, sl));
         const DerivedW tw = bind_derived(d, sel.lbase, l);
-        TE_TRY(linear_bwd_tc(tw.w2, dsx, lw.w2, dF, a.hpre, d.M, d.F, d.D, TE_EPI_GELU_BWD, st, sel.btf, &sel.bfs));
-        TE_TRY(linear_bwd_tc(tw.w1, dF, lw.w1, dxn, nullptr, d.M, d.D, d.F, TE_EPI_STORE, st, sel.btf, &sel.bfs));
-        TE_TRY(te_launch_add2(dxn, dsx, dxn, MD, st));
-        TE_TRY(te_launch_layernorm_bwd(dxn, a.s1, lw.ln1w, a.mean1, a.rstd1, nullptr, dsx, d.M, d.D, st));
-        TE_TRY(linear_bwd_tc(tw.o, dsx, lw.ow, dctx, nullptr, d.M, d.D, d.D, TE_EPI_STORE, st, sel.btf, &sel.bfs));
+        TE_TRY(linear_bwd_tc(tw.w2, dsx, lw.w2, dF, a.hpre, br, d.F, d.D, TE_EPI_GELU_BWD, st, sel.btf, &sel.bfs, bD, bF));
+        TE_TRY(linear_bwd_tc(tw.w1, dF, lw.w1, dxn, nullptr, br, d.D, d.F, TE_EPI_STORE, st, sel.btf, &sel.bfs, bF, bD));
+        TE_TRY(te_launch_add2(dxn, dsx, dxn, top ? d.D : MD, st, top ? d.B : 1, bD));
+        if (top) TE_TRY(te_launch_fill(dsx, 0.f, MD, st));
+        TE_TRY(te_launch_layernorm_bwd(dxn, a.s1, lw.ln1w, a.mean1, a.rstd1, nullptr, dsx, br, d.D, st, bD, sl));
+        if (top) TE_TRY(te_launch_fill(dctx, 0.f, MD, st));
+        TE_TRY(linear_bwd_tc(tw.o, dsx, lw.ow, dctx, nullptr, br, d.D, d.D, TE_EPI_STORE, st, sel.btf, &sel.bfs, bD, bD));
         const bool last = (l == start_layer);
-        TE_TRY(attn_block_bwd(sel, d.B, d.H, d.N, d.NP, d.dh, a.qkv, a.P, dctx, a.G, dS, dqkv, scale, last, st));
+        TE_TRY(attn_block_bwd(sel, d.B, d.H, d.N, d.NP, d.dh, a.qkv, a.P, dctx, a.G, dS, dqkv, scale, last, st, top));
         if (last) break;
         TE_TRY(linear_bwd_tc(tw.qkv, dqkv, lw.qkvw, dxn, nullptr, d.M, d.D, 3 * d.D, TE_EPI_STORE, st, sel.btf, &sel.bfs));
         TE_TRY(te_launch_add2(dxn, dsx, dxa, MD, st));
@@ -336,23 +342,25 @@
         const bool top = (l == d.L - 1) && te_engine_cls_rows();
         const long long zr = top ? d.B : d.M;
         const long long sD = top ? (long long)d.N * d.D : d.D, sF = top ? (long long)d.N * d.F : d.F;
-        TE_TRY(te_launch_add_relprop(a.d2, a.ao, R, R1, R2, addp, d.B, (long long)d.N * d.D, st));
+        const long long keep = top ? d.D : 0;
+        TE_TRY(te_launch_add_relprop(a.d2, a.ao, R, R1, R2, addp, d.B, (long long)d.N * d.D, st, keep));
         TE_TRY(te_linear_rule_relprop(sel.lrp, a.g, sF, lw.w2, dw.w2, R1, sD, RF, S, zr, d.F, d.D, st, a.d2, sD, lw.b2, sel.zv, sF,
                                       SF, alpha));
         TE_TRY(te_linear_rule_relprop(sel.lrp, a.ao, sD, lw.w1, dw.w1, RF, sF, R1, SF, zr, d.D, d.F, st, a.hpre, sF, lw.b1, sel.zv,
                                       sD, S, alpha));
-        TE_TRY(te_launch_clone_relprop(a.ao, R1, R2, nullptr, R, MD, st));
-        TE_TRY(te_launch_add_relprop(a.d1, a.h, R, R1, R2, addp, d.B, (long long)d.N * d.D, st));
+        TE_TRY(te_launch_clone_relprop(a.ao, R1, R2, nullptr, R, top ? d.D : MD, st, top ? d.B : 1, sD));
+        if (top) TE_TRY(te_launch_fill(R2, 0.f, MD, st));
+        TE_TRY(te_launch_add_relprop(a.d1, a.h, R, R1, R2, addp, d.B, (long long)d.N * d.D, st, keep));
         if (top) TE_TRY(te_launch_fill(R3, 0.f, MD, st));
         TE_TRY(te_linear_rule_relprop(sel.lrp, a.ctx, sD, lw.ow, dw.o, R1, sD, R3, S, zr, d.D, d.D, st, a.d1, sD, lw.ob, sel.zv, sD,
                                       S + MD, alpha));
         const bool last = (l == sel.low && !(flags & TE_FLAG_RELPROP_TO_INPUT));
-        TE_TRY(attn_relprop_pv(sel, d.B, d.H, d.N, d.NP, d.dh, a.qkv, a.P, R3, a.ctx, S, a.cam, Rqkv, last, st));
+        TE_TRY(attn_relprop_pv(sel, d.B, d.H, d.N, d.NP, d.dh, a.qkv, a.P, R3, a.ctx, S, a.cam, Rqkv, last, st, top));
         if (last) break;
         TE_TRY(attn_nn(sel.atc, d.B, d.H, d.N, d.NP, d.dh, a.qkv, 3 * d.D, a.qkv + d.D, 3 * d.D, ws.tA[0], nullptr, scale,
                        TE_EPI_STORE, st));
         TE_TRY(te_launch_add_relprop_keymask(ws.tA[0], ws.maskadd, a.cam, ws.tA[1], addp, d.B, d.H, d.N, d.NP, st));
-        TE_TRY(attn_relprop_qk(sel, d.B, d.H, d.N, d.NP, d.dh, a.qkv, ws.tA[1], ws.tA[0], Rqkv, st));
+        TE_TRY(attn_relprop_qk(sel, d.B, d.H, d.N, d.NP, d.dh, a.qkv, ws.tA[1], ws.tA[0], Rqkv, st, top));
         TE_TRY(te_linear_rule_relprop(sel.lrp, a.h, d.D, lw.qkvw, dw.q, Rqkv, 3 * d.D, R, S, d.M, d.D, d.D, st, a.qkv, 3 * d.D,
                                       lw.qkvb, sel.zv, 0, S + MD, alpha));
         TE_TRY(te_linear_rule_relprop(sel.lrp, a.h, d.D, lw.qkvw + DD, dw.k, Rqkv + d.D, 3 * d.D, R1, S, d.M, d.D, d.D, st,
diff --git a/transformer_explainability_b200/csrc/te_elementwise.cu b/transformer_explainability_b200/csrc/te_elementwise.cu
--- a/transformer_explainability_b200/csrc/te_elementwise.cu
+++ b/transformer_explainability_b200/csrc/te_elementwise.cu
@@ -143,12 +143,12 @@
 __global__ void layernorm_bwd_kernel(const float* __restrict__ dy, const float* __restrict__ x,
                                      const float* __restrict__ w, const float* __restrict__ mean,
                                      const float* __restrict__ rstd, const float* __restrict__ dres,
-                                     float* __restrict__ dx, long long rows, int D) {
+                                     float* __restrict__ dx, long long rows, int D, long long ld, long long sld) {
     const int lane = threadIdx.x & 31;
     const long long row = blockIdx.x * (long long)(blockDim.x >> 5) + (threadIdx.x >> 5);
     if (row >= rows) return;
-    ln_bwd_row(dy + row * D, x + row * D, w, dres ? dres + row * D : nullptr, dx + row * D, D, lane, mean[row],
-               rstd[row]);
+    const long long o = row * ld;
+    ln_bwd_row(dy + o, x + o, w, dres ? dres + o : nullptr, dx + o, D, lane, mean[row * sld], rstd[row * sld]);
 }
 
 __global__ void layernorm_bwd_strided_kernel(const float* __restrict__ dy, long long dy_stride,
@@ -188,16 +188,16 @@
 }
 
 __global__ void softmax_bwd_kernel(const float* __restrict__ p, const float* __restrict__ dp,
-                                   float* __restrict__ ds, long long rows, int N, int ld, float scale) {
+                                   float* __restrict__ ds, long long rows, int N, int ld, float scale, long long rstride) {
     const int lane = threadIdx.x & 31;
     const long long row = blockIdx.x * (long long)(blockDim.x >> 5) + (threadIdx.x >> 5);
     if (row >= rows) return;
-    const float* pr = p + row * ld;
-    const float* gr = dp + row * ld;
+    const float* pr = p + row * rstride;
+    const float* gr = dp + row * rstride;
     float dot = 0.f;
     for (int j = lane; j < N; j += 32) dot = fmaf(pr[j], gr[j], dot);
     dot = te_warp_sum(dot);
-    float* o = ds + row * ld;
+    float* o = ds + row * rstride;
     for (int j = lane; j < ld; j += 32) o[j] = (j < N) ? pr[j] * (gr[j] - dot) * scale : 0.f;
 }
 
@@ -244,7 +244,10 @@
 
 __global__ void clone_relprop_kernel(const float* __restrict__ x, const float* __restrict__ r1,
                                      const float* __restrict__ r2, const float* __restrict__ r3,
-                                     float* __restrict__ out, long long n4) {
+                                     float* __restrict__ out, long long n4, long long ld4) {
+    const long long o = blockIdx.y * ld4;
+    x += 4 * o; r1 += 4 * o; r2 += 4 * o; out += 4 * o;
+    if (r3) r3 += 4 * o;
     for (long long t = blockIdx.x * (long long)blockDim.x + threadIdx.x; t < n4;
          t += (long long)gridDim.x * blockDim.x) {
         const float4 xv = reinterpret_cast<const float4*>(x)[t];
@@ -262,10 +265,10 @@
 
 __global__ void add_reduce_kernel(const float* __restrict__ x1, const float* __restrict__ x2,
                                   const float* __restrict__ r, double* __restrict__ partial, long long per4,
-                                  long long x2s4) {
+                                  long long x2s4, long long keep4) {
     const int b = blockIdx.y, sp = blockIdx.x;
     const long long chunk = (per4 + TE_ADD_SPLIT - 1) / TE_ADD_SPLIT;
-    const long long lo = sp * chunk, hi = min(per4, lo + chunk);
+    const long long lo = sp * chunk, hi = min(keep4, lo + chunk);
     const float4* p1 = reinterpret_cast<const float4*>(x1) + b * per4;
     const float4* p2 = reinterpret_cast<const float4*>(x2) + b * x2s4;
     const float4* pr = reinterpret_cast<const float4*>(r) + b * per4;
@@ -293,7 +296,7 @@
 
 __global__ void add_scale_kernel(const float* __restrict__ x1, const float* __restrict__ x2,
                                  const float* __restrict__ r, float* __restrict__ r1, float* __restrict__ r2,
-                                 const double* __restrict__ partial, long long per4, long long x2s4) {
+                                 const double* __restrict__ partial, long long per4, long long x2s4, long long keep4) {
     const int b = blockIdx.y;
     __shared__ float fa_s, fb_s;
     if (threadIdx.x == 0 && partial == nullptr) { fa_s = 1.f; fb_s = 1.f; }
@@ -314,7 +317,7 @@
     const float4* pr = reinterpret_cast<const float4*>(r) + b * per4;
     float4* o1 = reinterpret_cast<float4*>(r1) + b * per4;
     float4* o2 = r2 ? reinterpret_cast<float4*>(r2) + b * per4 : nullptr;
-    for (long long t = blockIdx.x * (long long)blockDim.x + threadIdx.x; t < per4;
+    for (long long t = blockIdx.x * (long long)blockDim.x + threadIdx.x; t < keep4;
          t += (long long)gridDim.x * blockDim.x) {
         const float4 a = p1[t], c = p2[t], rr = pr[t];
         const float s0 = te_sd(rr.x, a.x + c.x), s1 = te_sd(rr.y, a.y + c.y);
@@ -614,7 +617,9 @@
     for (long long t = blockIdx.x * (long long)blockDim.x + threadIdx.x; t < n; t += (long long)gridDim.x * blockDim.x)
         dx[t] = dy[t] * (1.0f - y[t] * y[t]);
 }
-__global__ void add2_kernel(const float* a, const float* b, float* out, long long n4) {
+__global__ void add2_kernel(const float* a, const float* b, float* out, long long n4, long long ld4) {
+    const long long o = blockIdx.y * ld4;
+    a += 4 * o; b += 4 * o; out += 4 * o;
     for (long long t = blockIdx.x * (long long)blockDim.x + threadIdx.x; t < n4;
          t += (long long)gridDim.x * blockDim.x) {
         const float4 u = reinterpret_cast<const float4*>(a)[t], v = reinterpret_cast<const float4*>(b)[t];
@@ -729,10 +734,12 @@
     return TE_OK;
 }
 int te_launch_layernorm_bwd(const float* dy, const float* x, const float* w, const float* mean, const float* rstd,
-                            const float* dres, float* dx, long long rows, int D, cudaStream_t st) {
-    TE_REQ(D % 4 == 0, "layernorm_bwd: D % 4 != 0");
+                            const float* dres, float* dx, long long rows, int D, cudaStream_t st, long long ld,
+                            long long stat_ld) {
+    if (ld == 0) ld = D;
+    TE_REQ(D % 4 == 0 && ld % 4 == 0, "layernorm_bwd: D or the row stride % 4 != 0");
     if (rows <= 0) return TE_OK;
-    layernorm_bwd_kernel<<<warp_rows_grid(rows), kThreads, 0, st>>>(dy, x, w, mean, rstd, dres, dx, rows, D);
+    layernorm_bwd_kernel<<<warp_rows_grid(rows), kThreads, 0, st>>>(dy, x, w, mean, rstd, dres, dx, rows, D, ld, stat_ld);
     TE_CUDA_CHECK_LAUNCH();
     return TE_OK;
 }
@@ -757,9 +764,11 @@
     return TE_OK;
 }
 int te_launch_softmax_bwd(const float* p, const float* dp, float* ds, long long rows, int N, int ld, float scale,
-                          cudaStream_t st) {
+                          cudaStream_t st, long long row_stride) {
     if (rows <= 0) return TE_OK;
-    softmax_bwd_kernel<<<warp_rows_grid(rows), kThreads, 0, st>>>(p, dp, ds, rows, N, ld, scale);
+    if (row_stride == 0) row_stride = ld;
+    TE_REQ(row_stride >= ld, "softmax_bwd: overlapping rows");
+    softmax_bwd_kernel<<<warp_rows_grid(rows), kThreads, 0, st>>>(p, dp, ds, rows, N, ld, scale, row_stride);
     TE_CUDA_CHECK_LAUNCH();
     return TE_OK;
 }
@@ -780,30 +789,34 @@
     return TE_OK;
 }
 int te_launch_clone_relprop(const float* x, const float* r1, const float* r2, const float* r3, float* out,
-                            long long n, cudaStream_t st) {
-    TE_REQ(n % 4 == 0, "clone_relprop: n % 4 != 0");
-    clone_relprop_kernel<<<flat_grid(n / 4), kThreads, 0, st>>>(x, r1, r2, r3, out, n / 4);
+                            long long n, cudaStream_t st, int rows, long long ld) {
+    TE_REQ(n % 4 == 0 && ld % 4 == 0, "clone_relprop: n or the row stride % 4 != 0");
+    TE_REQ(rows >= 1 && rows <= 65535 && (rows == 1 || ld >= n), "clone_relprop: rows out of range or overlapping");
+    clone_relprop_kernel<<<dim3(flat_grid(n / 4), rows), kThreads, 0, st>>>(x, r1, r2, r3, out, n / 4, ld / 4);
     TE_CUDA_CHECK_LAUNCH();
     return TE_OK;
 }
 int te_launch_add_relprop_strided(const float* x1, const float* x2, long long x2_sample_stride, const float* r, float* r1,
-                                  float* r2, double* partial, int B, long long per_sample, cudaStream_t st) {
-    TE_REQ(per_sample % 4 == 0 && x2_sample_stride % 4 == 0, "add_relprop: per-sample size % 4 != 0");
+                                  float* r2, double* partial, int B, long long per_sample, cudaStream_t st,
+                                  long long keep) {
+    TE_REQ(per_sample % 4 == 0 && x2_sample_stride % 4 == 0 && keep % 4 == 0, "add_relprop: per-sample size % 4 != 0");
+    TE_REQ(keep >= 0 && keep <= per_sample, "add_relprop: kept prefix out of range");
     TE_REQ(B <= 65535, "add_relprop: batch too large for one launch");
     const long long per4 = per_sample / 4, x2s4 = x2_sample_stride / 4;
+    const long long keep4 = keep > 0 && keep / 4 <= (per4 + TE_ADD_SPLIT - 1) / TE_ADD_SPLIT ? keep / 4 : per4;
     if (partial) {
-        add_reduce_kernel<<<dim3(TE_ADD_SPLIT, B), kThreads, 0, st>>>(x1, x2, r, partial, per4, x2s4);
+        add_reduce_kernel<<<dim3(TE_ADD_SPLIT, B), kThreads, 0, st>>>(x1, x2, r, partial, per4, x2s4, keep4);
         TE_CUDA_CHECK_LAUNCH();
     }
-    int gx = (int)((per4 + kThreads - 1) / kThreads);
+    int gx = (int)((keep4 + kThreads - 1) / kThreads);
     gx = gx > 64 ? 64 : (gx < 1 ? 1 : gx);
-    add_scale_kernel<<<dim3(gx, B), kThreads, 0, st>>>(x1, x2, r, r1, r2, partial, per4, x2s4);
+    add_scale_kernel<<<dim3(gx, B), kThreads, 0, st>>>(x1, x2, r, r1, r2, partial, per4, x2s4, keep4);
     TE_CUDA_CHECK_LAUNCH();
     return TE_OK;
 }
 int te_launch_add_relprop(const float* x1, const float* x2, const float* r, float* r1, float* r2, double* partial,
-                          int B, long long per_sample, cudaStream_t st) {
-    return te_launch_add_relprop_strided(x1, x2, per_sample, r, r1, r2, partial, B, per_sample, st);
+                          int B, long long per_sample, cudaStream_t st, long long keep) {
+    return te_launch_add_relprop_strided(x1, x2, per_sample, r, r1, r2, partial, B, per_sample, st, keep);
 }
 int te_launch_index_select_relprop(const float* x, const float* r_tok0, const float* r_tok1, float* out, int B,
                                    int N, int D, cudaStream_t st) {
@@ -896,9 +909,10 @@
     TE_CUDA_CHECK_LAUNCH();
     return TE_OK;
 }
-int te_launch_add2(const float* a, const float* b, float* out, long long n, cudaStream_t st) {
-    TE_REQ(n % 4 == 0, "add2: n % 4 != 0");
-    add2_kernel<<<flat_grid(n / 4), kThreads, 0, st>>>(a, b, out, n / 4);
+int te_launch_add2(const float* a, const float* b, float* out, long long n, cudaStream_t st, int rows, long long ld) {
+    TE_REQ(n % 4 == 0 && ld % 4 == 0, "add2: n or the row stride % 4 != 0");
+    TE_REQ(rows >= 1 && rows <= 65535 && (rows == 1 || ld >= n), "add2: rows out of range or overlapping");
+    add2_kernel<<<dim3(flat_grid(n / 4), rows), kThreads, 0, st>>>(a, b, out, n / 4, ld / 4);
     TE_CUDA_CHECK_LAUNCH();
     return TE_OK;
 }
diff --git a/transformer_explainability_b200/csrc/te_engine_util.h b/transformer_explainability_b200/csrc/te_engine_util.h
--- a/transformer_explainability_b200/csrc/te_engine_util.h
+++ b/transformer_explainability_b200/csrc/te_engine_util.h
@@ -31,9 +31,10 @@
     return te_gemm_launch(p, TE_L_K, TE_L_K, TE_XF_NONE, epi, st);
 }
 static inline int linear_bwd(const float* dy, const float* w, float* dx, const float* e0, long long M, int in, int out,
-                             int epi, cudaStream_t st) {
+                             int epi, cudaStream_t st, long long lda = 0, long long ldc = 0) {
     TeGemm p = gemm0();
-    p.A = dy; p.lda = out; p.B = w; p.ldb = in; p.C = dx; p.ldc = in; p.E0 = e0; p.lde0 = in;
+    p.A = dy; p.lda = (int)(lda ? lda : out); p.B = w; p.ldb = in; p.C = dx; p.ldc = (int)(ldc ? ldc : in); p.E0 = e0;
+    p.lde0 = p.ldc;
     p.M = (int)M; p.N = in; p.K = out;
     return te_gemm_launch(p, TE_L_K, TE_L_MN, TE_XF_NONE, epi, st);
 }
@@ -56,15 +57,20 @@
     return linear_fwd(x, lda, w, bias, y, y2, e0, M, in, out, epi, st);
 }
 static inline int linear_bwd_tc(const float* dw, const float* dy, const float* w, float* dx, const float* e0, long long M,
-                                int in, int out, int epi, cudaStream_t st, bool tf32 = false, const F16Split* fs = nullptr) {
+                                int in, int out, int epi, cudaStream_t st, bool tf32 = false, const F16Split* fs = nullptr,
+                                long long lda = 0, long long ldc = 0) {
     const bool f16 = dw && fs && fs->split, single_epi = epi == TE_EPI_STORE || epi == TE_EPI_GELU_BWD;
-    if (f16 && single_epi && te_tc_fwd16_supported(M, out, in, out))
+    if (!lda) lda = out;
+    if (!ldc) ldc = in;
+    if (f16 && single_epi && te_tc_fwd16_supported(M, out, in, out)) {
+        if (lda != out || ldc != in) return no_fallback("linear_bwd_tc: the fp16 backward Linear takes packed rows only");
         return te_tc_linear_bwd16(fs->ready ? nullptr : dy, out, fs->split, fs->scale, dw, in, out, dx, e0, M, epi, st);
-    if (dw && tf32 && single_epi && te_tc_gemm3x_supported(M, out, in, out))
-        return te_tc_linear_bwd_tf32(dy, out, dw, in, out, dx, e0, M, epi, st);
-    if (dw && te_tc_gemm3x_supported(M, out, in, out))
-        return te_tc_linear_bwd(dy, dw, in, out, dx, e0, M, epi, st);
-    return linear_bwd(dy, w, dx, e0, M, in, out, epi, st);
+    }
+    if (dw && tf32 && single_epi && te_tc_gemm3x_supported(M, out, in, lda) && ldc % 4 == 0)
+        return te_tc_linear_bwd_tf32(dy, lda, dw, in, out, dx, ldc, e0, M, epi, st);
+    if (dw && te_tc_gemm3x_supported(M, out, in, lda) && ldc % 4 == 0)
+        return te_tc_linear_bwd(dy, lda, dw, in, out, dx, ldc, e0, M, epi, st);
+    return linear_bwd(dy, w, dx, e0, M, in, out, epi, st, lda, ldc);
 }
 
 struct HeadOp { const float* ptr; int ld; long long s1, s2; };
@@ -86,10 +92,18 @@
 }
 
 static inline int attn_nn(bool tc, int B, int H, int N, int NP, int dh, const float* A, int lda, const float* Bm, int ldb,
-                          float* out, const float* E, float alpha, int epi, cudaStream_t st, bool tf32 = false) {
+                          float* out, const float* E, float alpha, int epi, cudaStream_t st, bool tf32 = false,
+                          bool row0 = false) {
     if (tc && te_tc_attn_supported(N, dh, lda, ldb, NP)) {
         const int e = (epi == TE_EPI_STORE) ? TE_TC_ATTN_STORE : (epi == TE_EPI_MUL) ? TE_TC_ATTN_MUL : TE_TC_ATTN_SD;
-        return te_tc_attn_nn(A, lda, Bm, ldb, B, H, N, dh, out, NP, E, alpha, e, st, tf32 && N <= 256 && epi != TE_EPI_SD);
+        const int kept = row0 && N > 128 ? 128 : 0;
+        TE_TRY(te_tc_attn_nn(A, lda, Bm, ldb, B, H, N, dh, out, NP, E, alpha, e, st, tf32 && N <= 256 && epi != TE_EPI_SD, kept));
+        if (kept && cudaMemset2DAsync(out + (long long)kept * NP, sizeof(float) * N * NP, 0, sizeof(float) * (N - kept) * NP,
+                                      (size_t)B * H, st) != cudaSuccess) {
+            te_set_last_error("attn_nn: clearing the rows past the first tile failed");
+            return TE_ERR_CUDA;
+        }
+        return TE_OK;
     }
     const HeadOp none = {nullptr, 0, 0, 0};
     return head_gemm(B, H, head_rows(A, lda, N, dh), TE_L_K, head_rows(Bm, ldb, N, dh), TE_L_K, attn_map(out, H, N, NP),
@@ -105,11 +119,12 @@
 }
 
 static inline int attn_nk(bool tc, int B, int H, int N, int NP, int dh, const float* map, int amn, const float* X, int ldx,
-                          float* out, int ld_out, const float* E, float alpha, int epi, cudaStream_t st, bool tf32 = false) {
+                          float* out, int ld_out, const float* E, float alpha, int epi, cudaStream_t st, bool tf32 = false,
+                          int k_tokens = 0) {
     if (tc && te_tc_attn_nk_supported(N, dh, NP, ldx, ld_out)) {
         const int e = (epi == TE_EPI_STORE) ? TE_TC_ATTN_STORE : TE_TC_ATTN_MUL;
         if (epi == TE_EPI_STORE || epi == TE_EPI_MUL)
-            return te_tc_attn_nk(map, NP, amn, X, ldx, B, H, N, out, ld_out, E, alpha, e, st, tf32);
+            return te_tc_attn_nk(map, NP, amn, X, ldx, B, H, N, out, ld_out, E, alpha, e, st, tf32, k_tokens);
     }
     const HeadOp none = {nullptr, 0, 0, 0};
     return head_gemm(B, H, attn_map(map, H, N, NP), amn ? TE_L_MN : TE_L_K, head_rows(X, ldx, N, dh), TE_L_MN,
@@ -191,31 +206,39 @@
 }
 
 static inline int attn_block_bwd(const Select& s, int B, int H, int N, int NP, int dh, const float* qkv, const float* P,
-                                 const float* dctx, float* G, float* dS, float* dqkv, float scale, bool g_only, cudaStream_t st) {
-    const int D = H * dh;
-    TE_TRY(attn_nn(s.atc, B, H, N, NP, dh, dctx, D, qkv + 2 * D, 3 * D, G, nullptr, 1.f, TE_EPI_STORE, st, s.btf));
+                                 const float* dctx, float* G, float* dS, float* dqkv, float scale, bool g_only, cudaStream_t st,
+                                 bool pooled = false) {
+    const int D = H * dh, kt = pooled ? 1 : 0;
+    TE_TRY(attn_nn(s.atc, B, H, N, NP, dh, dctx, D, qkv + 2 * D, 3 * D, G, nullptr, 1.f, TE_EPI_STORE, st, s.btf, pooled));
     if (g_only) return TE_OK;
-    TE_TRY(attn_nk(s.atc, B, H, N, NP, dh, P, 1, dctx, D, dqkv + 2 * D, 3 * D, nullptr, 1.f, TE_EPI_STORE, st, s.btf));
-    TE_TRY(te_launch_softmax_bwd(P, G, dS, (long long)B * H * N, N, NP, scale, st));
+    TE_TRY(attn_nk(s.atc, B, H, N, NP, dh, P, 1, dctx, D, dqkv + 2 * D, 3 * D, nullptr, 1.f, TE_EPI_STORE, st, s.btf, kt));
+    if (pooled) {
+        TE_TRY(te_launch_fill(dS, 0.f, (long long)B * H * N * NP, st));
+        TE_TRY(te_launch_softmax_bwd(P, G, dS, (long long)B * H, N, NP, scale, st, (long long)N * NP));
+    } else {
+        TE_TRY(te_launch_softmax_bwd(P, G, dS, (long long)B * H * N, N, NP, scale, st));
+    }
     TE_TRY(attn_nk(s.atc, B, H, N, NP, dh, dS, 0, qkv + D, 3 * D, dqkv, 3 * D, nullptr, 1.f, TE_EPI_STORE, st, s.btf));
-    return attn_nk(s.atc, B, H, N, NP, dh, dS, 1, qkv, 3 * D, dqkv + D, 3 * D, nullptr, 1.f, TE_EPI_STORE, st, s.btf);
+    return attn_nk(s.atc, B, H, N, NP, dh, dS, 1, qkv, 3 * D, dqkv + D, 3 * D, nullptr, 1.f, TE_EPI_STORE, st, s.btf, kt);
 }
 
 static inline int attn_relprop_pv(const Select& s, int B, int H, int N, int NP, int dh, const float* qkv, const float* P,
                                   const float* Rctx, const float* ctx, float* S, float* cam, float* Rqkv, bool cam_only,
-                                  cudaStream_t st) {
+                                  cudaStream_t st, bool pooled = false) {
     const int D = H * dh;
     TE_TRY(te_launch_sd(Rctx, ctx, S, (long long)B * N * D, st));
-    TE_TRY(attn_nn(s.atc, B, H, N, NP, dh, S, D, qkv + 2 * D, 3 * D, cam, P, 0.5f, TE_EPI_MUL, st, s.rtf));
+    TE_TRY(attn_nn(s.atc, B, H, N, NP, dh, S, D, qkv + 2 * D, 3 * D, cam, P, 0.5f, TE_EPI_MUL, st, s.rtf, pooled));
     if (cam_only) return TE_OK;
-    return attn_nk(s.atc, B, H, N, NP, dh, P, 1, S, D, Rqkv + 2 * D, 3 * D, qkv + 2 * D, 0.5f, TE_EPI_MUL, st, s.rtf);
+    return attn_nk(s.atc, B, H, N, NP, dh, P, 1, S, D, Rqkv + 2 * D, 3 * D, qkv + 2 * D, 0.5f, TE_EPI_MUL, st, s.rtf,
+                   pooled ? 1 : 0);
 }
 static inline int attn_relprop_qk(const Select& s, int B, int H, int N, int NP, int dh, const float* qkv, const float* E,
-                                  float* S1, float* Rqkv, cudaStream_t st) {
+                                  float* S1, float* Rqkv, cudaStream_t st, bool pooled = false) {
     const int D = H * dh;
-    TE_TRY(attn_nn(s.atc, B, H, N, NP, dh, qkv, 3 * D, qkv + D, 3 * D, S1, E, 1.f, TE_EPI_SD, st));
+    TE_TRY(attn_nn(s.atc, B, H, N, NP, dh, qkv, 3 * D, qkv + D, 3 * D, S1, E, 1.f, TE_EPI_SD, st, false, pooled));
     TE_TRY(attn_nk(s.atc, B, H, N, NP, dh, S1, 0, qkv + D, 3 * D, Rqkv, 3 * D, qkv, 0.5f, TE_EPI_MUL, st, s.rtf));
-    return attn_nk(s.atc, B, H, N, NP, dh, S1, 1, qkv, 3 * D, Rqkv + D, 3 * D, qkv + D, 0.5f, TE_EPI_MUL, st, s.rtf);
+    return attn_nk(s.atc, B, H, N, NP, dh, S1, 1, qkv, 3 * D, Rqkv + D, 3 * D, qkv + D, 0.5f, TE_EPI_MUL, st, s.rtf,
+                   pooled ? 1 : 0);
 }
 
 struct Bump {
diff --git a/transformer_explainability_b200/csrc/te_gemm_tc.h b/transformer_explainability_b200/csrc/te_gemm_tc.h
--- a/transformer_explainability_b200/csrc/te_gemm_tc.h
+++ b/transformer_explainability_b200/csrc/te_gemm_tc.h
@@ -51,8 +51,8 @@
 bool te_tc_gemm3x_supported(long long rows, int K, int N, long long lda);
 int te_tc_linear_fwd(const float* x, long long ldx, const float* derived, int in_features, int out_features,
                      const float* bias, float* y, float* y2, const float* e0, long long rows, int epi, cudaStream_t st);
-int te_tc_linear_bwd(const float* dy, const float* derived, int in_features, int out_features, float* dx, const float* e0,
-                     long long rows, int epi, cudaStream_t st);
+int te_tc_linear_bwd(const float* dy, long long lddy, const float* derived, int in_features, int out_features, float* dx,
+                     long long lddx, const float* e0, long long rows, int epi, cudaStream_t st);
 
 bool te_tc_fwd16_supported(long long rows, int K, int N, long long lda);
 int te_tc_rowsplit_f16(const float* x, long long ldx, long long rows, int cols, void* hi, void* lo, float* scale_inv,
@@ -70,11 +70,13 @@
 enum { TE_TC_ATTN_STORE = 0, TE_TC_ATTN_MUL = 1, TE_TC_ATTN_SD = 2, TE_TC_ATTN_SOFTMAX = 3 };
 bool te_tc_attn_supported(int N, int dh, long long lda, long long ldb, int ld_out);
 int te_tc_attn_nn(const float* A, long long lda, const float* B, long long ldb, int batch, int H, int N, int dh,
-                  float* out, int ld_out, const float* E, float alpha, int epi, cudaStream_t st, bool single_pass = false);
+                  float* out, int ld_out, const float* E, float alpha, int epi, cudaStream_t st, bool single_pass = false,
+                  int m_rows = 0);
 
 bool te_tc_attn_nk_supported(int N, int dh, int NP, long long ldx, long long ld_out);
 int te_tc_attn_nk(const float* map, int NP, int amn, const float* X, long long ldx, int batch, int H, int N, float* out,
-                  int ld_out, const float* E, float alpha, int epi, cudaStream_t st, bool single_pass = false);
+                  int ld_out, const float* E, float alpha, int epi, cudaStream_t st, bool single_pass = false,
+                  int k_tokens = 0);
 
 bool te_tc_bmm_nk_supported(int N, int ld);
 int te_tc_bmm_nk_resid(const float* A, const float* J, const float* rowscale, float* out, int batch, int N, int ld,
@@ -87,4 +89,4 @@
 int te_tc_zplus_r(const float* s, const float* derived, const float* x, long long ldx, float* out, long long ld_out,
                   long long rows, int in_features, int out_features, cudaStream_t st, bool inh = false);
 int te_tc_linear_bwd_tf32(const float* dy, long long lddy, const float* derived, int in_features, int out_features, float* dx,
-                          const float* e0, long long rows, int epi, cudaStream_t st);
+                          long long lddx, const float* e0, long long rows, int epi, cudaStream_t st);
diff --git a/transformer_explainability_b200/csrc/te_kernels.h b/transformer_explainability_b200/csrc/te_kernels.h
--- a/transformer_explainability_b200/csrc/te_kernels.h
+++ b/transformer_explainability_b200/csrc/te_kernels.h
@@ -10,24 +10,26 @@
 int te_launch_layernorm_split(const float* x, const float* w, const float* b, float* y, float* mean, float* rstd,
                               long long rows, int D, float eps, float* split, float* scale, cudaStream_t st);
 int te_launch_layernorm_bwd(const float* dy, const float* x, const float* w, const float* mean, const float* rstd,
-                            const float* dres, float* dx, long long rows, int D, cudaStream_t st);
+                            const float* dres, float* dx, long long rows, int D, cudaStream_t st, long long ld = 0,
+                            long long stat_ld = 1);
 int te_launch_layernorm_bwd_strided(const float* dy, long long dy_stride, const float* x, long long x_stride,
                                     const float* w, float eps, float* dx, long long dx_stride, int rows, int D,
                                     cudaStream_t st);
 int te_launch_softmax(float* s, long long rows, int N, int ld, cudaStream_t st);
 int te_launch_softmax_bwd(const float* p, const float* dp, float* ds, long long rows, int N, int ld, float scale,
-                          cudaStream_t st);
+                          cudaStream_t st, long long row_stride = 0);
 int te_launch_argmax(const float* logits, int* index, int B, int C, int only_negative, cudaStream_t st);
 int te_launch_average2(const float* a, const float* b, float* out, long long n, cudaStream_t st);
 int te_launch_onehot(const int* index, float* seed, int B, int C, float value, cudaStream_t st);
 int te_launch_sd(const float* a, const float* b, float* out, long long n, cudaStream_t st);
 int te_launch_clone_relprop(const float* x, const float* r1, const float* r2, const float* r3, float* out,
-                            long long n, cudaStream_t st);
+                            long long n, cudaStream_t st, int rows = 1, long long ld = 0);
 #define TE_ADD_SPLIT 16
 int te_launch_add_relprop(const float* x1, const float* x2, const float* r, float* r1, float* r2, double* partial,
-                          int B, long long per_sample, cudaStream_t st);
+                          int B, long long per_sample, cudaStream_t st, long long keep = 0);
 int te_launch_add_relprop_strided(const float* x1, const float* x2, long long x2_sample_stride, const float* r, float* r1,
-                                  float* r2, double* partial, int B, long long per_sample, cudaStream_t st);
+                                  float* r2, double* partial, int B, long long per_sample, cudaStream_t st,
+                                  long long keep = 0);
 long long te_patch_relprop_scratch_floats(int B, int C, int img, int P, int D);
 int te_patch_relprop_run(const float* images, const float* weight, const float* r, long long r_sample_stride, int B,
                          int C, int img, int P, int D, float* scratch, float* r_pixels, float* r_sum, cudaStream_t st);
@@ -55,6 +57,6 @@
 int te_launch_bert_mask(const long long* mask, float* out, long long n, cudaStream_t st);
 int te_launch_tanh(const float* x, float* y, long long n, cudaStream_t st);
 int te_launch_tanh_bwd(const float* dy, const float* y, float* dx, long long n, cudaStream_t st);
-int te_launch_add2(const float* a, const float* b, float* out, long long n, cudaStream_t st);
+int te_launch_add2(const float* a, const float* b, float* out, long long n, cudaStream_t st, int rows = 1, long long ld = 0);
 int te_launch_add_relprop_keymask(const float* x1, const float* keymask, const float* r, float* r1, double* partial,
                                   int B, int H, int N, int ld, cudaStream_t st);
diff --git a/transformer_explainability_b200/csrc/te_rollout_fused.cu b/transformer_explainability_b200/csrc/te_rollout_fused.cu
--- a/transformer_explainability_b200/csrc/te_rollout_fused.cu
+++ b/transformer_explainability_b200/csrc/te_rollout_fused.cu
@@ -36,7 +36,8 @@
 #pragma unroll
         for (int c = 0; c < NCHUNK; ++c) { acc[c][0] = acc[c][1] = acc[c][2] = acc[c][3] = 0.f; }
 
-        for (int i = crank + K * warp; i < N; i += K * kWarps) {
+        const int rows = (l == L - 1) ? 1 : N;
+        for (int i = crank + K * warp; i < rows; i += K * kWarps) {
             float m[NCHUNK][4];
 #pragma unroll
             for (int c = 0; c < NCHUNK; ++c) { m[c][0] = m[c][1] = m[c][2] = m[c][3] = 0.f; }
diff --git a/transformer_explainability_b200/csrc/te_tc_wgmma.cu b/transformer_explainability_b200/csrc/te_tc_wgmma.cu
--- a/transformer_explainability_b200/csrc/te_tc_wgmma.cu
+++ b/transformer_explainability_b200/csrc/te_tc_wgmma.cu
@@ -827,9 +827,10 @@
     static constexpr bool TMA = true;
     static constexpr int FIX = FIX_AB, EPI_MAPS = 0;
     int N, H, NP, ld_out, n_out, n_pad, a_shared, batch;
+    int kn;
     const float* map; const float* X; long long ldx;
     const float* rowscale; const float* E; float* out; float alpha;
-    __device__ int kblocks() const { return (N + 31) / 32; }
+    __device__ int kblocks() const { return (kn + 31) / 32; }
     static constexpr int NMAPS = 2;
     TmaTile tile(int i) const {
         if (i == 0) return TmaTile{map, N, N, NP, AMN ? 32 : BM, (long long)batch * (a_shared ? 1 : H), (long long)N * NP};
@@ -1075,10 +1076,11 @@
 template <int FORM, bool FWD>
 int linear(int K, const void* a, const void* a_lo, long long lda, const void* b, const void* b_lo, const float* rs,
            const float* cs, long long rows, int N, const float* bias, const float* e0, float* y, float* y2, int epi,
-           const char* who, cudaStream_t st) {
+           const char* who, cudaStream_t st, long long ldc = 0) {
+    if (ldc == 0) ldc = N;
     LinArgs g;
     g.K = K; g.a = a; g.a_lo = a_lo; g.lda = lda; g.b = b; g.b_lo = b_lo; g.rs = rs; g.rs_ld = (K + 127) / 128; g.cs = cs;
-    g.o.M = (int)rows; g.o.N = N; g.o.bias = bias; g.o.E = e0; g.o.lde = N; g.o.C = y; g.o.ldc = N; g.o.C2 = y2; g.o.ldc2 = N;
+    g.o.M = (int)rows; g.o.N = N; g.o.bias = bias; g.o.E = e0; g.o.lde = ldc; g.o.C = y; g.o.ldc = ldc; g.o.C2 = y2; g.o.ldc2 = ldc;
     switch (epi) {
         case TE_TC_EPI_STORE: return lin_launch<TE_TC_EPI_STORE, FORM>(g, st);
         case TE_TC_EPI_BIAS: if constexpr (FWD) return lin_launch<TE_TC_EPI_BIAS, FORM>(g, st); break;
@@ -1303,26 +1305,26 @@
                                     y2, epi, "te_tc_linear_fwd", st);
 }
 
-int te_tc_linear_bwd(const float* dy, const float* derived, int in_features, int out_features, float* dx, const float* e0,
-                     long long rows, int epi, cudaStream_t st) {
-    if (!a16(dy) || !a16(derived) || !a16(dx) || (e0 && !a16(e0))) {
+int te_tc_linear_bwd(const float* dy, long long lddy, const float* derived, int in_features, int out_features, float* dx,
+                     long long lddx, const float* e0, long long rows, int epi, cudaStream_t st) {
+    if (!a16(dy) || lddy % 4 != 0 || !a16(derived) || !a16(dx) || lddx % 4 != 0 || (e0 && !a16(e0))) {
         te_set_last_error("te_tc_linear_bwd: operands must be 16-byte aligned");
         return TE_ERR_ARG;
     }
     const TeDerived<const float> dv(derived, in_features, out_features);
-    return linear<LIN_3XTF32, false>(out_features, dy, nullptr, out_features, dv.wth, dv.wtl, nullptr, nullptr, rows, in_features,
-                                     nullptr, e0, dx, nullptr, epi, "te_tc_linear_bwd", st);
+    return linear<LIN_3XTF32, false>(out_features, dy, nullptr, lddy, dv.wth, dv.wtl, nullptr, nullptr, rows, in_features,
+                                     nullptr, e0, dx, nullptr, epi, "te_tc_linear_bwd", st, lddx);
 }
 
 int te_tc_linear_bwd_tf32(const float* dy, long long lddy, const float* derived, int in_features, int out_features, float* dx,
-                          const float* e0, long long rows, int epi, cudaStream_t st) {
-    if (!a16(dy) || lddy % 4 != 0 || !a16(derived) || !a16(dx) || (e0 && !a16(e0))) {
+                          long long lddx, const float* e0, long long rows, int epi, cudaStream_t st) {
+    if (!a16(dy) || lddy % 4 != 0 || !a16(derived) || !a16(dx) || lddx % 4 != 0 || (e0 && !a16(e0))) {
         te_set_last_error("te_tc_linear_bwd_tf32: operands must be 16-byte aligned");
         return TE_ERR_ARG;
     }
     const TeDerived<const float> dv(derived, in_features, out_features);
     return linear<LIN_TF32, false>(out_features, dy, nullptr, lddy, dv.wth, nullptr, nullptr, nullptr, rows, in_features, nullptr,
-                                   e0, dx, nullptr, epi, "te_tc_linear_bwd_tf32", st);
+                                   e0, dx, nullptr, epi, "te_tc_linear_bwd_tf32", st, lddx);
 }
 
 bool te_tc_fwd16_supported(long long rows, int K, int N, long long lda) {
@@ -1370,25 +1372,27 @@
 namespace {
 template <int EPI, bool SP, int BN>
 int nn(const float* A, long long lda, const float* B, long long ldb, int batch, int H, int N, int dh, float* out, int ld_out,
-       const float* E, float alpha, cudaStream_t st) {
+       const float* E, float alpha, cudaStream_t st, int m_rows = 0) {
     NnProb<EPI, SP, BN> p;
     p.N = N; p.H = H; p.dh = dh; p.ld_out = ld_out; p.batch = batch;
     p.a = A; p.lda = lda; p.b = B; p.ldb = ldb; p.E = E; p.out = out; p.alpha = alpha;
-    return launch(p, dim3(mtiles(N), (unsigned)((N + BN - 1) / BN), (unsigned)(batch * H)), st);
+    const int mt = m_rows > 0 && m_rows < N ? mtiles(m_rows) : mtiles(N);
+    return launch(p, dim3(mt, (unsigned)((N + BN - 1) / BN), (unsigned)(batch * H)), st);
 }
 template <int AMN, int EPI, bool SP, int BN>
 int nk(const float* map, int NP, const float* X, long long ldx, int batch, int H, int N, float* out, int ld_out, int n_out,
-       int n_pad, int a_shared, const float* rowscale, const float* E, float alpha, cudaStream_t st) {
+       int n_pad, int a_shared, const float* rowscale, const float* E, float alpha, cudaStream_t st, int k_tokens = 0) {
     NkProb<AMN, EPI, SP, BN> p;
     p.N = N; p.H = H; p.NP = NP; p.ld_out = ld_out; p.n_out = n_out; p.n_pad = n_pad; p.a_shared = a_shared; p.batch = batch;
+    p.kn = k_tokens > 0 && k_tokens < N ? k_tokens : N;
     p.map = map; p.X = X; p.ldx = ldx; p.rowscale = rowscale; p.E = E; p.out = out; p.alpha = alpha;
     return launch(p, dim3(mtiles(N), 1, (unsigned)(batch * H)), st);
 }
 }
 
 int te_tc_attn_nn(const float* A, long long lda, const float* B, long long ldb, int batch, int H, int N, int dh,
-                  float* out, int ld_out, const float* E, float alpha, int epi, cudaStream_t st, bool single_pass) {
-#define TE_NN(EPI, SP, BN) nn<EPI, SP, BN>(A, lda, B, ldb, batch, H, N, dh, out, ld_out, E, alpha, st)
+                  float* out, int ld_out, const float* E, float alpha, int epi, cudaStream_t st, bool single_pass, int m_rows) {
+#define TE_NN(EPI, SP, BN) nn<EPI, SP, BN>(A, lda, B, ldb, batch, H, N, dh, out, ld_out, E, alpha, st, m_rows)
     if (single_pass && epi == TE_TC_ATTN_STORE) return TE_NN(AT_STORE, true, 128);
     if (single_pass && epi == TE_TC_ATTN_MUL) return TE_NN(AT_MUL, true, 128);
     switch (epi) {
@@ -1405,8 +1409,9 @@
 }
 
 int te_tc_attn_nk(const float* map, int NP, int amn, const float* X, long long ldx, int batch, int H, int N, float* out,
-                  int ld_out, const float* E, float alpha, int epi, cudaStream_t st, bool single_pass) {
-#define TE_NK(AMN, EPI, SP) nk<AMN, EPI, SP, 64>(map, NP, X, ldx, batch, H, N, out, ld_out, H * 64, H * 64, 0, nullptr, E, alpha, st)
+                  int ld_out, const float* E, float alpha, int epi, cudaStream_t st, bool single_pass, int k_tokens) {
+#define TE_NK(AMN, EPI, SP) nk<AMN, EPI, SP, 64>(map, NP, X, ldx, batch, H, N, out, ld_out, H * 64, H * 64, 0, nullptr, E, alpha, \
+                                                 st, k_tokens)
     if (epi == TE_TC_ATTN_STORE) {
         if (single_pass) return amn ? TE_NK(1, AT_STORE, true) : TE_NK(0, AT_STORE, true);
         return amn ? TE_NK(1, AT_STORE, false) : TE_NK(0, AT_STORE, false);
diff --git a/transformer_explainability_b200/csrc/te_vit.cu b/transformer_explainability_b200/csrc/te_vit.cu
--- a/transformer_explainability_b200/csrc/te_vit.cu
+++ b/transformer_explainability_b200/csrc/te_vit.cu
@@ -315,12 +315,18 @@
         LayerAct& a = ws.layer[l];
         const BlockW& bw = w.blk[l];
         const DerivedW lw = bind_derived(d, sel.lbase, l);
-        TE_TRY(te_util::linear_bwd_tc(lw.fc2, dxa, bw.fc2w, dF, a.h, d.M, d.F, d.D, TE_EPI_GELU_BWD, st, sel.btf, &sel.bfs));
-        TE_TRY(te_util::linear_bwd_tc(lw.fc1, dF, bw.fc1w, dxn, nullptr, d.M, d.D, d.F, TE_EPI_STORE, st, sel.btf, &sel.bfs));
-        TE_TRY(te_launch_layernorm_bwd(dxn, a.x_mid, bw.n2w, a.mean2, a.rstd2, dxa, dxb, d.M, d.D, st));
-        TE_TRY(te_util::linear_bwd_tc(lw.proj, dxb, bw.projw, dctx, nullptr, d.M, d.D, d.D, TE_EPI_STORE, st, sel.btf, &sel.bfs));
+        const bool top = (l == d.L - 1) && !cfg->distilled && !sel.bfs.split && te_engine_cls_rows();
+        const long long br = top ? d.B : d.M;
+        const long long bD = top ? (long long)d.N * d.D : d.D, bF = top ? (long long)d.N * d.F : d.F;
+        TE_TRY(te_util::linear_bwd_tc(lw.fc2, dxa, bw.fc2w, dF, a.h, br, d.F, d.D, TE_EPI_GELU_BWD, st, sel.btf, &sel.bfs, bD, bF));
+        TE_TRY(te_util::linear_bwd_tc(lw.fc1, dF, bw.fc1w, dxn, nullptr, br, d.D, d.F, TE_EPI_STORE, st, sel.btf, &sel.bfs, bF, bD));
+        if (top) TE_TRY(te_launch_fill(dxb, 0.f, MD, st));
+        TE_TRY(te_launch_layernorm_bwd(dxn, a.x_mid, bw.n2w, a.mean2, a.rstd2, dxa, dxb, br, d.D, st, bD, top ? d.N : 1));
+        if (top) TE_TRY(te_launch_fill(dctx, 0.f, MD, st));
+        TE_TRY(te_util::linear_bwd_tc(lw.proj, dxb, bw.projw, dctx, nullptr, br, d.D, d.D, TE_EPI_STORE, st, sel.btf, &sel.bfs, bD,
+                                      bD));
         const bool last = (l == start_layer);
-        TE_TRY(te_util::attn_block_bwd(sel, d.B, d.H, d.N, d.NP, d.dh, a.qkv, a.P, dctx, a.G, dS, dqkv, scale, last, st));
+        TE_TRY(te_util::attn_block_bwd(sel, d.B, d.H, d.N, d.NP, d.dh, a.qkv, a.P, dctx, a.G, dS, dqkv, scale, last, st, top));
         if (last) break;
         TE_TRY(te_util::linear_bwd_tc(lw.qkv, dqkv, bw.qkvw, dxn, nullptr, d.M, d.D, 3 * d.D, TE_EPI_STORE, st, sel.btf, &sel.bfs));
         TE_TRY(te_launch_layernorm_bwd(dxn, a.x_in, bw.n1w, a.mean1, a.rstd1, dxb, dxa, d.M, d.D, st));
@@ -335,8 +341,8 @@
 
     float* R = ws.tD[0]; float* R1 = ws.tD[1]; float* R2 = ws.tD[2]; float* R3 = ws.tD[3];
     float* RF = ws.tF[0]; float* SF = ws.tF[1]; float* S = ws.t3D[0]; float* Rqkv = ws.t3D[1]; float* S1 = ws.tA;
-    auto addrule = [&](const float* x1, const float* x2, const float* r, float* r1, float* r2) -> int {
-        return te_launch_add_relprop(x1, x2, r, r1, r2, sel.lrp ? nullptr : ws.addpart, d.B, (long long)d.N * d.D, st);
+    auto addrule = [&](const float* x1, const float* x2, const float* r, float* r1, float* r2, long long keep) -> int {
+        return te_launch_add_relprop(x1, x2, r, r1, r2, sel.lrp ? nullptr : ws.addpart, d.B, (long long)d.N * d.D, st, keep);
     };
     TE_TRY(te_linear_rule_relprop(sel.lrp, ws.xf, (long long)d.N * d.D, w.headw, nullptr, ws.seed, d.C, ws.rhead0, ws.shead, d.B,
                                   d.D, d.C, st, nullptr, 0, nullptr, sel.zv, 0, nullptr, alpha));
@@ -352,20 +358,22 @@
         const bool top = (l == d.L - 1) && !cfg->distilled && !sel.lrp && te_engine_cls_rows();
         const long long zr = top ? d.B : d.M;
         const long long sD = top ? (long long)d.N * d.D : d.D, sF = top ? (long long)d.N * d.F : d.F;
-        TE_TRY(addrule(a.x_mid, a.mlp_out, R, R1, R2));
+        const long long keep = top ? d.D : 0;
+        TE_TRY(addrule(a.x_mid, a.mlp_out, R, R1, R2, keep));
         TE_TRY(te_linear_rule_relprop(sel.lrp, a.g, sF, bw.fc2w, dw.fc2, R2, sD, RF, S, zr, d.F, d.D, st, a.mlp_out, sD, bw.fc2b,
                                       sel.zv, sF, SF, alpha));
         TE_TRY(te_linear_rule_relprop(sel.lrp, a.xn2, sD, bw.fc1w, dw.fc1, RF, sF, R2, SF, zr, d.D, d.F, st, a.h, sF, bw.fc1b,
                                       sel.zv, sD, S, alpha));
-        TE_TRY(te_launch_clone_relprop(a.x_mid, R1, R2, nullptr, R, MD, st));
-        TE_TRY(addrule(a.x_in, a.attn_out, R, R1, R2));
+        TE_TRY(te_launch_clone_relprop(a.x_mid, R1, R2, nullptr, R, top ? d.D : MD, st, top ? d.B : 1, sD));
+        if (top) TE_TRY(te_launch_fill(R1, 0.f, MD, st));
+        TE_TRY(addrule(a.x_in, a.attn_out, R, R1, R2, keep));
         if (top) TE_TRY(te_launch_fill(R3, 0.f, MD, st));
         TE_TRY(te_linear_rule_relprop(sel.lrp, a.ctx, sD, bw.projw, dw.proj, R2, sD, R3, S, zr, d.D, d.D, st, a.attn_out, sD,
                                       bw.projb, sel.zv, sD, S + MD, alpha));
         const bool last = (l == sel.low && !(flags & TE_FLAG_RELPROP_TO_INPUT));
-        TE_TRY(te_util::attn_relprop_pv(sel, d.B, d.H, d.N, d.NP, d.dh, a.qkv, a.P, R3, a.ctx, S, a.cam, Rqkv, last, st));
+        TE_TRY(te_util::attn_relprop_pv(sel, d.B, d.H, d.N, d.NP, d.dh, a.qkv, a.P, R3, a.ctx, S, a.cam, Rqkv, last, st, top));
         if (last) break;
-        TE_TRY(te_util::attn_relprop_qk(sel, d.B, d.H, d.N, d.NP, d.dh, a.qkv, a.cam, S1, Rqkv, st));
+        TE_TRY(te_util::attn_relprop_qk(sel, d.B, d.H, d.N, d.NP, d.dh, a.qkv, a.cam, S1, Rqkv, st, top));
         TE_TRY(te_linear_rule_relprop(sel.lrp, a.xn1, d.D, bw.qkvw, dw.qkv, Rqkv, 3 * d.D, R2, S, d.M, d.D, 3 * d.D, st, a.qkv,
                                       3 * d.D, bw.qkvb, sel.zv, 0, RF, alpha));
         TE_TRY(te_launch_clone_relprop(a.x_in, R1, R2, nullptr, R, MD, st));
```

After: 942.6, median of 6. 1.02x the previous value.
